# jstmn/cppflow

Hardware: AMD Instinct MI355X
Metric: LM-IK iterations/sec (seeds x waypoints) (higher is better)
Workload: dtype f32

## Files before the change

### cppflow_amd/build.py

```python

import os
import subprocess
import sys

_HERE = os.path.dirname(os.path.abspath(__file__))
CSRC = os.path.join(_HERE, "csrc")
SOURCES = ["cppflow_hip.hip", "fused_static.hip"]
EXTRA_FLAGS = {"fused_static.hip": ["-O2", "-mllvm", "-amdgpu-sched-strategy=max-ilp", "-mllvm", "-enable-post-misched=0"]}
HEADERS = ["lmik_device.h", "robots_gen.h", "rtc_specialize.h", "kernels_chain.h", "kernels_collision.h", "kernels_fused.h", "kernels_track.h", "kernels_quad.h", "kernels_eval.h",
           "kernels_coupled.h", "kernels_dp.h", "kernels_optloop.h", "kernels_scene.h", "kernels_motion.h", "kernels_motion_resolve.h", os.path.join("..", "..", "include", "cppflow_hip.h"),
           os.path.join("..", "..", "include", "cppflow_hip_debug.h")]
OUT = os.path.join(CSRC, "libcppflow_hip.so")

HIPCC_FLAGS = [
    "--offload-arch=gfx950",
    "-O3",
    "-std=c++17",
    "-fPIC",
    "-ffp-contract=off",
    "-fhip-fp32-correctly-rounded-divide-sqrt",
    "-fno-slp-vectorize",
    "-Wno-comment",
]


def source_hash() -> str:
    import hashlib

    h = hashlib.sha256()
    for name in SOURCES + [n for n in HEADERS if n != "rtc_specialize.h"] + ["rtc_specialize.h"]:
        with open(os.path.join(CSRC, name), "rb") as f:
            h.update(name.encode() + b"\0" + f.read() + b"\0")
    h.update(" ".join(HIPCC_FLAGS).encode())
    for name in SOURCES:
        h.update((name + " " + " ".join(EXTRA_FLAGS.get(name, []))).encode())
    h.update(" ".join(link_flags()).encode())
    return h.hexdigest()[:32]


def link_flags():
    return [f for f in HIPCC_FLAGS if f.startswith("--offload-arch=") or f == "-fPIC"] + ["-shared"]


def built_id() -> str:
    if not os.path.exists(OUT):
        return ""
    import re

    with open(OUT, "rb") as f:
        m = re.search(rb"CPPF_BUILD_ID=([0-9a-f]{32})", f.read())
    return m.group(1).decode() if m else ""


def needs_build() -> bool:
    if not os.path.exists(OUT):
        return True
    return built_id() != source_hash()


EMBEDDED = ["lmik_device.h", "kernels_chain.h", "kernels_collision.h", "kernels_fused.h", "kernels_track.h", "kernels_quad.h"]
EMBEDDED_OUT = os.path.join(CSRC, "embedded_src.inc")


def write_embedded_sources() -> bool:
    parts = ["// embedded_src.inc -- GENERATED by cppflow_amd/build.py (the device headers as strings for hipRTC); do not edit."]
    files = [(n, os.path.join(CSRC, n)) for n in EMBEDDED] + [("../../include/cppflow_hip.h", os.path.join(CSRC, "..", "..", "include", "cppflow_hip.h"))]
    parts.append(f"static const int kEmbeddedCount = {len(files)};")
    parts.append("static const char* const kEmbeddedNames[] = {" + ", ".join(f'"{n}"' for n, _ in files) + "};")
    parts.append("static const char* const kEmbeddedSources[] = {")
    for _, path in files:
        text = open(path).read()
        assert ')CPPFSRC"' not in text
        chunks = [text[i : i + 12000] for i in range(0, len(text), 12000)]
        parts.append("    " + "\n    ".join(f'R"CPPFSRC({c})CPPFSRC"' for c in chunks) + ",")
    parts.append("};")
    out = "\n".join(parts) + "\n"
    if os.path.exists(EMBEDDED_OUT) and open(EMBEDDED_OUT).read() == out:
        return False
    with open(EMBEDDED_OUT, "w") as f:
        f.write(out)
    return True


def build(force: bool = False, verbose: bool = False) -> str:
    from cppflow_amd import gen_robots

    if gen_robots.write() and verbose:
        print("regenerated", gen_robots.OUT)
    if write_embedded_sources() and verbose:
        print("regenerated", EMBEDDED_OUT)
    if not force and not needs_build():
        return OUT
    hipcc = os.environ.get("HIPCC", "hipcc")
    objdir = os.path.join(CSRC, "obj")
    os.makedirs(objdir, exist_ok=True)
    procs, objs = [], []
    for src in SOURCES:
        obj = os.path.join(objdir, os.path.splitext(src)[0] + ".o")
        cmd = [hipcc] + HIPCC_FLAGS + EXTRA_FLAGS.get(src, []) + [f'-DCPPF_BUILD_ID="{source_hash()}"', "-c", "-o", obj, os.path.join(CSRC, src)]
        if verbose:
            print(" ".join(cmd))
        procs.append((cmd, subprocess.Popen(cmd, cwd=CSRC)))
        objs.append(obj)
    failed = None
    for cmd, p in procs:
        if p.wait() != 0 and failed is None:
            failed = (p.returncode, cmd)
            for _, other in procs:
                if other.poll() is None:
                    other.kill()
    if failed is not None:
        raise subprocess.CalledProcessError(*failed)
    cmd = [hipcc] + link_flags() + ["-o", OUT] + objs
    if verbose:
        print(" ".join(cmd))
    subprocess.run(cmd, check=True, cwd=CSRC)
    return OUT


TEST_SRC = os.path.join(_HERE, "..", "tests", "native", "rcp_sweep.hip")
TEST_OUT = os.path.join(_HERE, "..", "tests", "native", "libcppf_testkernels.so")


def build_test_kernels(force: bool = False, verbose: bool = False) -> str:
    deps = [TEST_SRC, os.path.join(CSRC, "lmik_device.h"), os.path.abspath(__file__)]
    if not force and os.path.exists(TEST_OUT) and all(os.path.getmtime(TEST_OUT) >= os.path.getmtime(d) for d in deps):
        return TEST_OUT
    cmd = [os.environ.get("HIPCC", "hipcc")] + HIPCC_FLAGS + ["-shared", "-o", TEST_OUT, TEST_SRC]
    if verbose:
        print(" ".join(cmd))
    subprocess.run(cmd, check=True)
    return TEST_OUT


if __name__ == "__main__":
    print(build(force="--force" in sys.argv, verbose=True))
    print(build_test_kernels(force="--force" in sys.argv, verbose=True))
```

### cppflow_amd/csrc/cppflow_hip.hip

```cpp
#include <hip/hip_runtime.h>

#include <dlfcn.h>

#include <atomic>
#include <cmath>
#include <cstdio>
#include <cstring>
#include <mutex>
#include <new>
#include <string>
#include <type_traits>
#include <utility>
#include <vector>

#include "../../include/cppflow_hip_debug.h"
#include "lmik_device.h"
#include "robots_gen.h"

using namespace cppf;

namespace cppf {
bool launch_fused_static(int static_id, int coll, unsigned grid, size_t lds, hipStream_t st, const FusedArgs& args);
int fused_static_block();
}

namespace {

#ifndef CPPF_BLOCK
#define CPPF_BLOCK 256
#endif
constexpr int kBlock = CPPF_BLOCK;

#ifndef CPPF_WAVES_LM
#define CPPF_WAVES_LM 2
#endif
#ifndef CPPF_WAVES_COLL
#define CPPF_WAVES_COLL 2
#endif

#include "kernels_chain.h"
#include "kernels_collision.h"
#include "kernels_fused.h"
#include "kernels_track.h"
#include "kernels_quad.h"
#include "kernels_eval.h"
#include "kernels_scene.h"
#include "kernels_motion.h"
#include "kernels_motion_resolve.h"
#include "kernels_coupled.h"
#include "kernels_dp.h"
#include "kernels_optloop.h"


thread_local std::string g_err;

int fail(int code, const std::string& msg) {
    g_err = msg;
    return code;
}

#define CPPF_REQUIRE(cond, msg) \
    do {                        \
        if (!(cond)) return fail(CPPF_ERR_INVALID, std::string("cppflow_hip: ") + (msg)); \
    } while (0)

#define CPPF_HIP(call)                                                                                       \
    do {                                                                                                     \
        hipError_t e__ = (call);                                                                             \
        if (e__ != hipSuccess)                                                                               \
            return fail(CPPF_ERR_HIP, std::string("cppflow_hip: " #call " failed: ") + hipGetErrorString(e__)); \
    } while (0)

inline unsigned grid_for(size_t n) { return (unsigned)((n + kBlock - 1) / kBlock); }

struct RtcModule;

}

struct cppf_robot {
    cppf_robot_desc desc;
    ChainK chain;
    CollK coll;
    int device;
    int cu_count;
    int static_id;
    size_t lds_bytes;
    void* d_quad;
    float rho[CPPF_MAX_DOF][CPPF_MAX_CAPSULES];
    RtcModule* rtc;
    mutable std::atomic<int> tune[CPPF_TUNE_COUNT];
    mutable std::atomic<uint32_t> life;
};
constexpr uint32_t kRobotDead = 0x80000000u;

namespace {
constexpr int kTuneDefaults[CPPF_TUNE_COUNT] = {
     0,  -1,  16384,  1,
     1,      2,        0,          0,
     42,     22,     (int)(kGateRel * 1e6f + 0.5f),  -1,
     0,
};
inline int tune(const cppf_robot* rb, int key) { return rb->tune[key].load(std::memory_order_relaxed); }

inline size_t fused_static_lds(const cppf_robot* rb) { return fused_static_lds_bound(rb->desc.ndof); }
inline size_t fused_spread_lds(const cppf_robot* rb, size_t n) {
    const int kb = tune(rb, CPPF_TUNE_SPREAD_KB);
    if (kb <= 0 || n > (size_t)128 * kBlock) return 0;
    const size_t stat = fused_static_lds(rb);
    const size_t room = stat + 512 < 65536 ? 65536 - 512 - stat : 0;
    return std::min((size_t)kb * 1024, room);
}
}

#include "rtc_specialize.h"

namespace {

float sqrt_threshold(float r) {
    if (!(r > 0.f)) return 0.f;
    float y = r * r;
    while (std::sqrt(y) >= r) y = std::nextafterf(y, 0.f);
    while (std::sqrt(y) < r) y = std::nextafterf(y, INFINITY);
    return y;
}

struct CapsuleCentred {
    float c[3], h[3], a, ia;
    double half_length;
};
CapsuleCentred capsule_centred(const cppf_robot_desc& d, int cap) {
    CapsuleCentred r;
    for (int k = 0; k < 3; ++k) {
        r.c[k] = (float)(0.5 * ((double)d.cap_p0[cap][k] + (double)d.cap_p1[cap][k]));
        r.h[k] = (float)(0.5 * ((double)d.cap_p1[cap][k] - (double)d.cap_p0[cap][k]));
    }
    const double h0 = r.h[0], h1 = r.h[1], h2 = r.h[2];
    const double a = (h0 * h0 + h1 * h1) + h2 * h2;
    r.a = (float)a;
    r.ia = a >= 0x1p-100 ? (float)(1.0 / a) : 0.f;
    r.half_length = std::sqrt(a);
    return r;
}

double cap_half_length(const cppf_robot_desc& d, int c) { return capsule_centred(d, c).half_length; }

float cull_threshold(double reach) {
    const double y = (reach + 0.01) * (reach + 0.01) * (1.0 + 1e-4);
    float f = (float)y;
    if ((double)f < y) f = std::nextafterf(f, INFINITY);
    return f;
}

constexpr int kQuadTableRecs = CPPF_MAX_PAIRS + CPPF_MAX_CAPSULES;
float round_up_f32(double y) {
    float f = (float)y;
    if ((double)f < y) f = std::nextafterf(f, INFINITY);
    return f;
}
void motion_rho_table(const cppf_robot_desc& d, float (&rho)[CPPF_MAX_DOF][CPPF_MAX_CAPSULES]) {
    const auto norm3 = [](const float* v) { return std::sqrt((double)v[0] * v[0] + (double)v[1] * v[1] + (double)v[2] * v[2]); };
    for (int j = 0; j < CPPF_MAX_DOF; ++j)
        for (int c = 0; c < CPPF_MAX_CAPSULES; ++c) rho[j][c] = 0.f;
    for (int c = 0; c < d.n_capsules; ++c) {
        const int l = d.cap_link[c];
        const double tail = std::max(norm3(d.cap_p0[c]), norm3(d.cap_p1[c])) + (double)d.cap_r[c];
        for (int j = 0; j <= l; ++j) {
            if (d.jtype[j] == CPPF_JOINT_PRISMATIC) {
                rho[j][c] = 1.f;
                continue;
            }
            double sum = tail;
            for (int i = j + 1; i <= l; ++i) {
                sum += norm3(&d.F[i][9]);
                if (d.jtype[i] == CPPF_JOINT_PRISMATIC) sum += std::max(std::fabs((double)d.lo[i]), std::fabs((double)d.hi[i]));
            }
            rho[j][c] = round_up_f32(sum);
        }
    }
}

template <class T>
bool desc_matches(const cppf_robot_desc& d) {
    if (d.ndof != T::D || d.n_capsules != T::L || d.n_pairs != T::P) return false;
    uint32_t pm = 0;
    for (int j = 0; j < T::D; ++j) {
        if (d.jtype[j] == CPPF_JOINT_PRISMATIC) pm |= 1u << j;
        for (int k = 0; k < 12; ++k)
            if (d.F[j][k] != T::F[j][k]) return false;
        if (d.lo[j] != T::lo[j] || d.hi[j] != T::hi[j]) return false;
    }
    if (pm != T::pris_mask) return false;
    for (int k = 0; k < 12; ++k)
        if (d.F_ee[k] != T::Fee[k]) return false;
    for (int c = 0; c < T::L; ++c) {
        if (d.cap_link[c] != T::cap_link[c] || d.cap_r[c] != T::cap_r[c]) return false;
        for (int k = 0; k < 3; ++k)
            if (d.cap_p0[c][k] != T::cap_p0[c][k] || d.cap_p1[c][k] != T::cap_p1[c][k]) return false;
    }
    for (int p = 0; p < T::P; ++p)
        if (d.pairs[p][0] != T::pair_a[p] || d.pairs[p][1] != T::pair_b[p]) return false;
    return true;
}

int find_static_robot(const cppf_robot_desc& d) {
#define CPPF_MATCH(idx, Type) \
    if (desc_matches<Type>(d)) return idx;
    CPPF_FOR_EACH_STATIC_ROBOT(CPPF_MATCH)
#undef CPPF_MATCH
    return -1;
}

template <int N>
struct Dof {
    static constexpr int D = N;
};
template <class T>
struct RobotTag {
    using type = T;
};

template <class F>
int for_ndof(int d, F&& f) {
    switch (d) {
        case 3: return f(Dof<3>{});
        case 4: return f(Dof<4>{});
        case 5: return f(Dof<5>{});
        case 6: return f(Dof<6>{});
        case 7: return f(Dof<7>{});
        case 8: return f(Dof<8>{});
        case 9: return f(Dof<9>{});
        case 10: return f(Dof<10>{});
        case 11: return f(Dof<11>{});
        case 12: return f(Dof<12>{});
        default: return fail(CPPF_ERR_UNSUPPORTED, "cppflow_hip: kernels are built for ndof in 3..12");
    }
}

template <class F>
int for_dyn_robot(const cppf_robot* rb, F&& f) {
    return for_ndof(rb->desc.ndof, [&](auto dof) { return f(RobotTag<DynRobot<decltype(dof)::D>>{}); });
}

inline bool use_table(const cppf_robot* rb) { return rb->static_id >= 0 && !tune(rb, CPPF_TUNE_FORCE_GENERIC); }

template <class F>
int for_robot(const cppf_robot* rb, F&& f) {
    if (!use_table(rb)) return for_dyn_robot(rb, f);
    switch (rb->static_id) {
#define CPPF_TABLE_CASE(idx, Type) \
    case idx: return f(RobotTag<StaRobot<Type>>{});
        CPPF_FOR_EACH_STATIC_ROBOT(CPPF_TABLE_CASE)
#undef CPPF_TABLE_CASE
        default: return CPPF_OK;
    }
}

constexpr int kNoDevice = -12345;
constexpr int kPcrMaxRowsLds = 131072, kPcrMaxRowsGlobal = 49152;
constexpr int kPcrSplitMaxD = 8;

int rtc_launch(const cppf_robot* rb, RtcKernel which, unsigned grid, size_t lds, hipStream_t st, void** args) {
    hipFunction_t f = rb->rtc->fn[which];
    if (!f) return fail(CPPF_ERR_UNSUPPORTED, "cppflow_hip: this kernel is not part of the handle's specialised module");
    CPPF_HIP(hipModuleLaunchKernel(f, grid, 1, 1, (unsigned)kBlock, 1, 1, (unsigned)lds, st, args, nullptr));
    return CPPF_OK;
}

inline bool use_rtc(const cppf_robot* rb) { return rb->rtc != nullptr && !tune(rb, CPPF_TUNE_FORCE_GENERIC); }

int check_launch() {
    CPPF_HIP(hipGetLastError());
    return CPPF_OK;
}

struct DeviceGuard {
    int prev = -1;
    bool switched = false;
    hipError_t err = hipSuccess;
    explicit DeviceGuard(int device) {
        err = hipGetDevice(&prev);
        if (err == hipSuccess && prev != device) {
            err = hipSetDevice(device);
            switched = err == hipSuccess;
        }
    }
    ~DeviceGuard() {
        if (switched) (void)hipSetDevice(prev);
    }
    DeviceGuard(const DeviceGuard&) = delete;
    DeviceGuard& operator=(const DeviceGuard&) = delete;
};

#define CPPF_ENTER(rb)                                                                                              \
    CPPF_REQUIRE((rb) != nullptr, "robot handle is NULL");                                                          \
    CPPF_REQUIRE(!((rb)->life.load(std::memory_order_acquire) & kRobotDead),                                         \
                 "the robot handle was destroyed (cppf_robot_destroy; it is only kept allocated for its live batches)"); \
    DeviceGuard device_guard__((rb)->device);                                                                        \
    if (device_guard__.err != hipSuccess)                                                                            \
        return fail(CPPF_ERR_HIP, std::string("cppflow_hip: selecting the robot's device failed: ") +               \
                                      hipGetErrorString(device_guard__.err))

template <class K, class... A>
int launch_lds(K kernel, dim3 grid, size_t lds, hipStream_t st, const A&... args) {
    if (lds > (size_t)64 * 1024)
        CPPF_HIP(hipFuncSetAttribute(reinterpret_cast<const void*>(kernel), hipFuncAttributeMaxDynamicSharedMemorySize, (int)lds));
    hipLaunchKernelGGL(kernel, grid, dim3(kBlock), lds, st, args...);
    return CPPF_OK;
}

float tile_cull_threshold(const cppf_robot* robot, float reach) {
    double r_max = 0.0;
    for (int c = 0; c < robot->coll.ncaps; ++c) r_max = std::max(r_max, (double)robot->desc.cap_r[c]);
    return cull_threshold(r_max + (double)reach);
}
SceneCullK scene_cull_setup(const cppf_robot* robot, const float* box_lo, const float* box_hi, int n_obs, float reach) {
    SceneCullK sc;
    sc.box_lo = box_lo;
    sc.box_hi = box_hi;
    sc.n_obs = n_obs;
    sc.reach = reach;
    for (int c = 0; c < CPPF_MAX_CAPSULES; ++c) sc.cull2[c] = 0.f;
    for (int c = 0; c < robot->coll.ncaps; ++c)
        sc.cull2[c] = cull_threshold(cap_half_length(robot->desc, c) + (double)robot->desc.cap_r[c] + (double)reach);
    sc.tile_cull2 = tile_cull_threshold(robot, reach);
    return sc;
}

struct CuboidChunks {
    int n_chunks, chunk;
};
CuboidChunks cut_cuboid_chunks(const cppf_robot* robot, unsigned blocks, int n_obs) {
    const int groups = (n_obs + 7) / 8;
    if (groups == 0 || blocks == 0) return {1, 64};
    const unsigned want_blocks = 4u * (unsigned)(robot->cu_count > 0 ? robot->cu_count : 256);
    int n_chunks = (int)std::min<unsigned>((unsigned)groups, std::max(1u, (want_blocks + blocks - 1) / blocks));
    const int groups_per_chunk = (groups + n_chunks - 1) / n_chunks;
    n_chunks = (groups + groups_per_chunk - 1) / groups_per_chunk;
    return {n_chunks, groups_per_chunk * 8};
}

template <class Shape, class Need>
int check_scene_call(const cppf_robot* robot, Shape&& shape, int n_obs, float reach_m, bool io_ok, const char* io_msg, const float* box_lo,
                     const float* box_hi, const void* workspace, size_t workspace_bytes, Need&& need, const char* need_msg,
                     const char* kernel, size_t* lds) {
    CPPF_REQUIRE(robot != nullptr, "robot handle is NULL");
    CPPF_REQUIRE(!(robot->life.load(std::memory_order_acquire) & kRobotDead), "the robot handle was destroyed");
    if (int rc = shape()) return rc;
    CPPF_REQUIRE(n_obs >= 0 && n_obs <= CPPF_MAX_SCENE_OBSTACLES, "n_obs out of range (0 .. CPPF_MAX_SCENE_OBSTACLES)");
    CPPF_REQUIRE(reach_m >= 0.f, "reach_m must be in [0, +inf] (not NaN, not negative)");
    CPPF_REQUIRE(io_ok, io_msg);
    CPPF_REQUIRE(n_obs == 0 || (box_lo && box_hi), "box_lo / box_hi is NULL");
    CPPF_REQUIRE(workspace, "workspace is NULL");
    CPPF_REQUIRE(((uintptr_t)workspace & 15u) == 0, "workspace must be 16-byte aligned");
    size_t bytes = 0;
    if (int rc = need(&bytes)) return rc;
    CPPF_REQUIRE(workspace_bytes >= bytes, need_msg);
    if (robot->desc.ndof < 3) return fail(CPPF_ERR_UNSUPPORTED, "cppflow_hip: kernels are built for ndof in 3..12");
    *lds = use_table(robot) ? 0 : robot->lds_bytes;
    if (*lds > (size_t)160 * 1024 - 1024)
        return fail(CPPF_ERR_UNSUPPORTED, std::string("cppflow_hip: the generic ") + kernel + " kernel cannot stage this many capsules");
    return CPPF_OK;
}

}

extern "C" {

int cppf_abi_version(void) { return CPPF_ABI_VERSION; }

#ifndef CPPF_BUILD_ID
#define CPPF_BUILD_ID "unversioned"
#endif
static const char kBuildIdMarker[] = "CPPF_BUILD_ID=" CPPF_BUILD_ID;
const char* cppf_build_id(void) { return kBuildIdMarker + 14; }

const char* cppf_last_error(void) { return g_err.c_str(); }

int cppf_robot_create(const cppf_robot_desc* desc, int device, cppf_robot** out) {
    CPPF_REQUIRE(desc && out, "desc / out is NULL");
    *out = nullptr;
    const int d = desc->ndof;
    CPPF_REQUIRE(d >= 1 && d <= CPPF_MAX_DOF, "ndof out of range");
    CPPF_REQUIRE(desc->n_capsules >= 0 && desc->n_capsules <= CPPF_MAX_CAPSULES, "n_capsules out of range");
    CPPF_REQUIRE(desc->n_pairs >= 0 && desc->n_pairs <= CPPF_MAX_PAIRS, "n_pairs out of range");
    for (int j = 0; j < d; ++j) {
        CPPF_REQUIRE(desc->jtype[j] == CPPF_JOINT_REVOLUTE || desc->jtype[j] == CPPF_JOINT_PRISMATIC, "bad joint type");
        CPPF_REQUIRE(desc->lo[j] <= desc->hi[j], "joint limits: lo > hi");
        for (int k = 0; k < 12; ++k) CPPF_REQUIRE(std::isfinite(desc->F[j][k]), "non-finite chain constant");
    }
    int prev = -1;
    for (int c = 0; c < desc->n_capsules; ++c) {
        const int l = desc->cap_link[c];
        CPPF_REQUIRE(l >= -1 && l < d, "capsule link index out of range");
        CPPF_REQUIRE(l >= prev, "capsules must be ordered by link (base first)");
        prev = l;
        float len2 = 0.f;
        for (int k = 0; k < 3; ++k) {
            const float dd = desc->cap_p1[c][k] - desc->cap_p0[c][k];
            len2 += dd * dd;
        }
        CPPF_REQUIRE(len2 == 0.f || len2 > 1e-12f, "degenerate capsule (|p1 - p0| < 1e-6 but not 0; use p0 == p1 for a sphere)");
        CPPF_REQUIRE(desc->cap_r[c] >= 0.f, "negative capsule radius");
    }
    for (int p = 0; p < desc->n_pairs; ++p) {
        const int a = desc->pairs[p][0], b = desc->pairs[p][1];
        CPPF_REQUIRE(a >= 0 && a < desc->n_capsules && b >= 0 && b < desc->n_capsules && a != b, "bad capsule pair");
    }
    if (device != kNoDevice) {
        int ndev = 0;
        CPPF_HIP(hipGetDeviceCount(&ndev));
        CPPF_REQUIRE(device >= 0 && device < ndev, "device index out of range");
    }

    cppf_robot* rb = new (std::nothrow) cppf_robot();
    if (!rb) return fail(CPPF_ERR_HIP, "cppflow_hip: out of host memory");
    rb->desc = *desc;
    rb->device = device;
    rb->cu_count = 0;
    if (device != kNoDevice) (void)hipDeviceGetAttribute(&rb->cu_count, hipDeviceAttributeMultiprocessorCount, device);
    rb->life.store(0u, std::memory_order_relaxed);
    for (int k = 0; k < CPPF_TUNE_COUNT; ++k) rb->tune[k].store(kTuneDefaults[k], std::memory_order_relaxed);
    std::memset(&rb->chain, 0, sizeof(ChainK));
    std::memset(&rb->coll, 0, sizeof(CollK));
    rb->chain.ndof = d;
    for (int j = 0; j < d; ++j) {
        std::memcpy(rb->chain.F[j], desc->F[j], sizeof(float) * 12);
        rb->chain.lo[j] = desc->lo[j];
        rb->chain.hi[j] = desc->hi[j];
        if (desc->jtype[j] == CPPF_JOINT_PRISMATIC) rb->chain.pris_mask |= (1u << j);
    }
    std::memcpy(rb->chain.Fee, desc->F_ee, sizeof(float) * 12);
    CollK& co = rb->coll;
    co.ncaps = desc->n_capsules;
    co.npairs = desc->n_pairs;
    for (int c = 0; c < co.ncaps; ++c) {
        const CapsuleCentred cc = capsule_centred(*desc, c);
        for (int k = 0; k < 3; ++k) {
            co.cap_c[c][k] = cc.c[k];
            co.cap_h[c][k] = cc.h[k];
        }
        co.cap_a[c] = cc.a;
        co.cap_ia[c] = cc.ia;
        co.cap_r[c] = desc->cap_r[c];
        co.cap_link[c] = (int8_t)desc->cap_link[c];
        co.cap_thr[c] = sqrt_threshold(desc->cap_r[c]);
        co.cap_cull[c] = cull_threshold(cap_half_length(*desc, c) + (double)desc->cap_r[c]);
    }
    for (int l = -1; l <= d; ++l) {
        int first = co.ncaps;
        for (int c = co.ncaps - 1; c >= 0; --c)
            if (desc->cap_link[c] >= l) first = c;
        co.cap_begin[l + 1] = first;
    }
    for (int p = 0; p < co.npairs; ++p) {
        co.pair_a[p] = (uint8_t)desc->pairs[p][0];
        co.pair_b[p] = (uint8_t)desc->pairs[p][1];
        co.pair_thr[p] = sqrt_threshold(desc->cap_r[desc->pairs[p][0]] + desc->cap_r[desc->pairs[p][1]]);
        const int a = desc->pairs[p][0], b = desc->pairs[p][1];
        co.pair_cull[p] = cull_threshold(cap_half_length(*desc, a) + cap_half_length(*desc, b) + (double)desc->cap_r[a] +
                                         (double)desc->cap_r[b]);
    }
    rb->lds_bytes = (size_t)co.ncaps * 6 * kBlock * sizeof(float);
    rb->static_id = find_static_robot(*desc);
    if (fused_static_block() != kBlock) rb->static_id = -1;
    rb->rtc = nullptr;
    rb->d_quad = nullptr;
    motion_rho_table(*desc, rb->rho);
    if (device != kNoDevice) {
        static_assert(sizeof(rb->rho) % sizeof(uint4) == 0, "the rho table is a whole number of uint4 records");
        std::vector<uint4> host(kQuadTableRecs + sizeof(rb->rho) / sizeof(uint4), uint4{0, 0, 0, 0});
        std::memcpy(&host[kQuadTableRecs], rb->rho, sizeof(rb->rho));
        for (int p = 0; p < co.npairs; ++p) {
            QuadPairRec r{co.pair_a[p], co.pair_b[p], co.pair_thr[p], co.pair_cull[p]};
            std::memcpy(&host[p], &r, sizeof r);
        }
        for (int c = 0; c < co.ncaps; ++c) {
            QuadCapRec r{co.cap_thr[c], co.cap_cull[c], co.cap_a[c], co.cap_ia[c]};
            std::memcpy(&host[CPPF_MAX_PAIRS + c], &r, sizeof r);
        }
        DeviceGuard guard(device);
        hipError_t e = guard.err;
        rb->d_quad = nullptr;
        if (e == hipSuccess) e = hipMalloc(&rb->d_quad, host.size() * sizeof(uint4));
        if (e == hipSuccess) e = hipMemcpy(rb->d_quad, host.data(), host.size() * sizeof(uint4), hipMemcpyHostToDevice);
        if (e != hipSuccess) {
            if (rb->d_quad) (void)hipFree(rb->d_quad);
            delete rb;
            return fail(CPPF_ERR_HIP, std::string("cppflow_hip: device tables: ") + hipGetErrorString(e));
        }
    }
    *out = rb;
    return CPPF_OK;
}

namespace {
void robot_free(cppf_robot* robot) {
    if (robot->device != kNoDevice) {
        DeviceGuard guard(robot->device);
        if (robot->d_quad) (void)hipFree(robot->d_quad);
        if (robot->rtc) {
            if (robot->rtc->module) (void)hipModuleUnload(robot->rtc->module);
            delete robot->rtc;
        }
    }
    delete robot;
}
}

void cppf_robot_destroy(cppf_robot* robot) {
    if (!robot) return;
    const uint32_t before = robot->life.fetch_or(kRobotDead, std::memory_order_acq_rel);
    if (before == 0u) robot_free(robot);
}

int cppf_robot_specialize(cppf_robot* robot, const char* cache_dir) {
    CPPF_REQUIRE(robot != nullptr, "robot handle is NULL");
    if (robot->static_id >= 0 || robot->rtc) return CPPF_OK;
    const bool with_quad = robot->desc.ndof >= 6;
    const std::string source = rtc_program_source(*robot);
    if (const char* dump = std::getenv("CPPF_RTC_DUMP")) {
        std::ofstream f(dump);
        f << source;
    }
    uint64_t key = fnv1a(source);
    for (int i = 0; i < kEmbeddedCount; ++i) key = fnv1a(kEmbeddedSources[i], key);
    for (int i = 0; i < kRtcOptionCount; ++i) key = fnv1a(kRtcOptions[i], key);
    key = fnv1a(rtc_version_string(), key);
    char hex[32];
    std::snprintf(hex, sizeof hex, "%016llx", (unsigned long long)key);
    const std::string dir = rtc_cache_dir(cache_dir), file = dir + "/robot_" + hex + ".cppfrtc";
    std::vector<std::string> names;
    std::string code;
    if (!rtc_cache_read(dir, file, names, code)) {
        if (int rc = rtc_compile(source, with_quad, names, code)) return rc;
        rtc_cache_write(dir, file, names, code);
    }
    DeviceGuard device_guard__(robot->device);
    if (device_guard__.err != hipSuccess)
        return fail(CPPF_ERR_HIP, std::string("cppflow_hip: selecting the robot's device failed: ") + hipGetErrorString(device_guard__.err));
    RtcModule* m = new (std::nothrow) RtcModule();
    if (!m) return fail(CPPF_ERR_HIP, "cppflow_hip: out of host memory");
    hipError_t e = hipModuleLoadData(&m->module, code.data());
    for (int i = 0; e == hipSuccess && i < RTC_COUNT; ++i) {
        if (!with_quad && (i == RTC_QUAD0 || i == RTC_QUAD1)) continue;
        e = hipModuleGetFunction(&m->fn[i], m->module, names[(size_t)i].c_str());
    }
    if (e != hipSuccess) {
        if (m->module) (void)hipModuleUnload(m->module);
        delete m;
        return fail(CPPF_ERR_HIP, std::string("cppflow_hip: loading the specialised code object failed: ") + hipGetErrorString(e));
    }
    robot->rtc = m;
    return CPPF_OK;
}

int cppf_robot_ndof(const cppf_robot* robot) { return robot ? robot->desc.ndof : CPPF_ERR_INVALID; }

int cppf_debug_fused_single_offset(void) { return (int)__builtin_offsetof(FusedArgs, single); }

int cppf_debug_rtc_compile(const cppf_robot_desc* desc, const char* cache_dir) {
    cppf_robot* rb = nullptr;
    if (int rc = cppf_robot_create(desc, kNoDevice, &rb)) return rc;
    rb->static_id = -1;
    rb->device = kNoDevice;
    const int rc = cppf_robot_specialize(rb, cache_dir);
    delete rb;
    (void)hipGetLastError();
    return rc;
}

int cppf_robot_specialization(const cppf_robot* robot) {
    if (!robot) return CPPF_ERR_INVALID;
    return robot->static_id >= 0 ? robot->static_id : (robot->rtc ? CPPF_SPECIALIZATION_RTC : -1);
}

int cppf_debug_set(cppf_robot* robot, int key, int value) {
    CPPF_REQUIRE(robot, "robot handle is NULL");
    CPPF_REQUIRE(key >= 0 && key < CPPF_TUNE_COUNT, "unknown tuning key");
    robot->tune[key].store(value == CPPF_TUNE_DEFAULT ? kTuneDefaults[key] : value, std::memory_order_relaxed);
    return CPPF_OK;
}

int cppf_debug_get(const cppf_robot* robot, int key, int* value) {
    CPPF_REQUIRE(robot && value, "robot / value is NULL");
    CPPF_REQUIRE(key >= 0 && key < CPPF_TUNE_COUNT, "unknown tuning key");
    *value = tune(robot, key);
    return CPPF_OK;
}

int cppf_set_obstacles(cppf_robot* robot, int n_obs, const float* cuboids, const float* Rt) {
    CPPF_REQUIRE(robot, "robot handle is NULL");
    CPPF_REQUIRE(n_obs >= 0 && n_obs <= CPPF_MAX_OBSTACLES, "n_obs out of range");
    CPPF_REQUIRE(n_obs == 0 || (cuboids && Rt), "cuboids / Rt is NULL");
    for (int o = 0; o < n_obs; ++o) {
        const float* R = Rt + o * 12;
        const float I[9] = {1, 0, 0, 0, 1, 0, 0, 0, 1};
        for (int k = 0; k < 9; ++k)
            CPPF_REQUIRE(std::fabs(R[k] - I[k]) < 1e-8f, "only axis-aligned cuboids are supported (R must be I)");
        for (int k = 0; k < 3; ++k) {
            CPPF_REQUIRE(cuboids[o * 6 + k] <= cuboids[o * 6 + 3 + k], "cuboid min corner > max corner");
            robot->coll.obs_lo[o][k] = R[9 + k] + cuboids[o * 6 + k];
            robot->coll.obs_hi[o][k] = R[9 + k] + cuboids[o * 6 + 3 + k];
        }
    }
    robot->coll.nobs = n_obs;
    return CPPF_OK;
}

int cppf_set_joint_limit_padding(cppf_robot* robot, const float* lo_padded, const float* hi_padded) {
    CPPF_REQUIRE(robot, "robot handle is NULL");
    if (!lo_padded || !hi_padded) {
        robot->coll.has_jl = 0;
        return CPPF_OK;
    }
    for (int j = 0; j < robot->desc.ndof; ++j) {
        robot->coll.jl_lo[j] = lo_padded[j];
        robot->coll.jl_hi[j] = hi_padded[j];
    }
    robot->coll.has_jl = 1;
    return CPPF_OK;
}

int cppf_forward_kinematics(const cppf_robot* robot, const float* x, int n, float* poses, void* stream) {
    CPPF_ENTER(robot);
    CPPF_REQUIRE(n >= 0, "n < 0");
    if (n == 0) return CPPF_OK;
    CPPF_REQUIRE(x && poses, "x / poses is NULL");
    hipStream_t st = (hipStream_t)stream;
    return for_ndof(robot->desc.ndof, [&](auto dof) {
        hipLaunchKernelGGL((fk_kernel<decltype(dof)::D>), dim3(grid_for(n)), dim3(kBlock), 0, st, robot->chain, robot->coll, n, x, poses);
        return check_launch();
    });
}

int cppf_jacobian(const cppf_robot* robot, const float* x, int n, float* J, void* stream) {
    CPPF_ENTER(robot);
    CPPF_REQUIRE(n >= 0, "n < 0");
    if (n == 0) return CPPF_OK;
    CPPF_REQUIRE(x && J, "x / J is NULL");
    hipStream_t st = (hipStream_t)stream;
    return for_ndof(robot->desc.ndof, [&](auto dof) {
        hipLaunchKernelGGL((jacobian_kernel<decltype(dof)::D>), dim3(grid_for(n)), dim3(kBlock), 0, st, robot->chain, robot->coll, n, x, J);
        return check_launch();
    });
}

int cppf_pose_errors(const cppf_robot* robot, const float* x, const float* target, int S, int W, float* e,
                     float* current_poses, void* stream) {
    CPPF_ENTER(robot);
    CPPF_REQUIRE(S >= 0 && W >= 0, "S / W < 0");
    const size_t n = (size_t)S * W;
    if (n == 0) return CPPF_OK;
    CPPF_REQUIRE(n <= 0x7fffffffu, "S*W exceeds 2^31-1 rows");
    CPPF_REQUIRE(x && target, "x / target is NULL");
    hipStream_t st = (hipStream_t)stream;
    return for_ndof(robot->desc.ndof, [&](auto dof) {
        hipLaunchKernelGGL((pose_errors_kernel<decltype(dof)::D>), dim3(grid_for(n)), dim3(kBlock), 0, st, robot->chain, robot->coll,
                           (int)n, W, x, target, e, current_poses);
        return check_launch();
    });
}

int cppf_clamp_to_joint_limits(const cppf_robot* robot, float* x, int n, void* stream) {
    CPPF_ENTER(robot);
    CPPF_REQUIRE(n >= 0, "n < 0");
    if (n == 0) return CPPF_OK;
    CPPF_REQUIRE(x, "x is NULL");
    const size_t total = (size_t)n * robot->desc.ndof;
    hipLaunchKernelGGL(clamp_kernel, dim3(grid_for(total)), dim3(kBlock), 0, (hipStream_t)stream, robot->chain, total, x);
    return check_launch();
}

}

namespace {

int make_lm_kernel_params(const cppf_robot* robot, const cppf_lm_params* params, LmK& prm) {
    CPPF_REQUIRE(params, "params is NULL");
    CPPF_REQUIRE(params->n_steps >= 1, "n_steps must be >= 1");
    CPPF_REQUIRE(params->clamp == 1 || params->n_steps == 1, "clamp = 0 is only defined for a single step");
    CPPF_REQUIRE(params->lm_lambda > 0.f, "lm_lambda must be > 0");
    CPPF_REQUIRE(params->alpha_position > 0.f && params->alpha_rotation > 0.f, "alpha_position / alpha_rotation must be > 0");
    CPPF_REQUIRE(params->solver == CPPF_SOLVER_AUTO || params->solver == CPPF_SOLVER_F32 || params->solver == CPPF_SOLVER_F64,
                 "unknown solver");
    CPPF_REQUIRE(params->solver_gate >= 0.f, "solver_gate must be >= 0 (0 = the default tolerance)");
    CPPF_REQUIRE(params->shape == CPPF_SHAPE_AUTO || params->shape == CPPF_SHAPE_ROW || params->shape == CPPF_SHAPE_QUAD,
                 "unknown kernel shape");
    CPPF_REQUIRE(params->tol_pos_m >= 0.f && params->tol_rot_rad >= 0.f, "early-out tolerances must be >= 0");
    CPPF_REQUIRE((params->tol_pos_m > 0.f) == (params->tol_rot_rad > 0.f), "set both early-out tolerances or neither");
    prm.lm_lambda = params->lm_lambda;
    prm.a_pos = params->alpha_position;
    prm.a_rot = params->alpha_rotation;
    prm.lam_r_d = (double)params->lm_lambda / ((double)params->alpha_rotation * (double)params->alpha_rotation);
    prm.lam_p_d = (double)params->lm_lambda / ((double)params->alpha_position * (double)params->alpha_position);
    prm.lam_r = (float)prm.lam_r_d;
    prm.lam_p = (float)prm.lam_p_d;
    const float tau = params->solver_gate > 0.f ? params->solver_gate : CPPF_SOLVER_GATE_DEFAULT;
    const float a_max = std::fmax(params->alpha_position, params->alpha_rotation);
    prm.gate_thr = params->solver == CPPF_SOLVER_F32 ? INFINITY : params->solver == CPPF_SOLVER_F64 ? -INFINITY : tau / (6e-8f * a_max);
    const float rel = 1e-6f * (float)tune(robot, CPPF_TUNE_GATE_REL_PPM) / (6e-8f * a_max);
    prm.gate_rel2 = rel * rel;
    const int pace = tune(robot, CPPF_TUNE_LM_PACE);
    prm.pace_ticks = (pace == 0 || params->tol_pos_m > 0.f || params->n_steps < 3) ? 0 : (pace > 0 ? pace : (int)(0.55f * (200.f + 56.f * (float)robot->desc.ndof) + 0.5f));
    prm.n_steps = params->n_steps;
    prm.clamp = params->clamp;
    prm.n = 0;
    prm.W = 0;
    prm.tol_pos2 = params->tol_pos_m > 0.f ? std::fmax(params->tol_pos_m * params->tol_pos_m, 1.17549435e-38f) : 0.f;
    prm.tol_rot2 = params->tol_rot_rad > 0.f ? std::fmax(params->tol_rot_rad * params->tol_rot_rad, 1.17549435e-38f) : 0.f;
    return CPPF_OK;
}

inline bool outputs_want_collision(const cppf_lm_outputs& o) {
    return o.self_mask || o.env_mask || o.jlim_mask || o.ext_cost || o.min_self || o.min_env || o.seed_summary;
}
inline bool summary_in_launch(int W) { return W >= 64 && kBlock % W == 0 && (W & (W - 1)) == 0; }

int launch_fused_rows(const cppf_robot* robot, int coll, size_t n_rows, unsigned grid, hipStream_t st, const LmK& prm,
                      const BatchItemK& single, const void* table) {
    const bool generic = !use_rtc(robot) && !use_table(robot);
    const size_t spread = fused_spread_lds(robot, n_rows);
    const size_t lds_need = (generic && coll) ? robot->lds_bytes : 0;
    if (generic && coll && lds_need + fused_static_lds(robot) > (size_t)160 * 1024)
        return fail(CPPF_ERR_UNSUPPORTED, "cppflow_hip: the generic kernels cannot stage this many capsules at this ndof; cppf_robot_specialize() the robot");
    FusedArgs fa;
    fa.ch = robot->chain;
    fa.co = robot->coll;
    fa.prm = prm;
    {
        const unsigned long long slots = (unsigned long long)(robot->cu_count > 0 ? robot->cu_count : 256) * 4ull;
        const int d = robot->desc.ndof;
        const bool four = (use_rtc(robot) || use_table(robot)) ? d <= 7 : d <= 6;
        if (!four || (unsigned long long)grid * 4ull < 3ull * slots || (unsigned long long)grid > slots) fa.prm.pace_ticks = 0;
    }
    fa.single = single;
    fa.table = table;
    if (use_rtc(robot)) {
        void* args[] = {(void*)&fa.ch, (void*)&fa.co, (void*)&fa.prm, (void*)&fa.single, (void*)&fa.table};
        if (int rc = rtc_launch(robot, coll == 0 ? RTC_FUSED0 : (coll == 2 ? RTC_FUSED2 : RTC_FUSED1), grid, spread, st, args)) return rc;
    } else if (!generic) {
        if (!launch_fused_static(robot->static_id, coll, grid, spread, st, fa))
            return fail(CPPF_ERR_UNSUPPORTED, "cppflow_hip: no fused kernel for this generated table");
    } else {
        const size_t lds = std::max(lds_need, spread);
        const int rc = for_dyn_robot(robot, [&](auto tag) {
            using RB = typename decltype(tag)::type;
            if (coll == 2)
                hipLaunchKernelGGL((lm_fused_kernel<RB, 2>), dim3(grid), dim3(kBlock), lds, st, fa.ch, fa.co, fa.prm, fa.single, fa.table);
            else if (coll == 1)
                hipLaunchKernelGGL((lm_fused_kernel<RB, 1>), dim3(grid), dim3(kBlock), lds, st, fa.ch, fa.co, fa.prm, fa.single, fa.table);
            else
                hipLaunchKernelGGL((lm_fused_kernel<RB, 0>), dim3(grid), dim3(kBlock), lds, st, fa.ch, fa.co, fa.prm, fa.single, fa.table);
            return CPPF_OK;
        });
        if (rc) return rc;
    }
    return check_launch();
}

template <class RB, int COLL, bool MFMA>
void launch_quad_kernel(const cppf_robot* robot, unsigned grid, size_t lds, hipStream_t st, const LmK& prm, const float* x_in,
                        const float* target, const cppf_lm_outputs& oq, const uint4* tab, const StepGateK gate) {
    hipLaunchKernelGGL((lm_quad_kernel<RB, COLL, MFMA>), dim3(grid), dim3(kBlock), lds, st, robot->chain, robot->coll, prm, x_in, target,
                       oq, tab, gate);
}

int launch_quad(const cppf_robot* robot, bool coll, size_t n, hipStream_t st, const LmK& prm, const float* x_in, const float* target,
                const cppf_lm_outputs& oq, const StepGateK gate) {
    const unsigned grid = (unsigned)((n + kQuadRows - 1) / kQuadRows);
    const size_t lds_q = coll ? sizeof(float) * (4 * (CPPF_MAX_PAIRS + CPPF_MAX_CAPSULES) +
                                                 (size_t)kQuadRows * quad_row_stride(robot->coll.ncaps))
                              : 0;
    const uint4* tab = static_cast<const uint4*>(robot->d_quad);
    const bool mfma = tune(robot, CPPF_TUNE_QUAD_MFMA) && use_table(robot);
    if (use_rtc(robot) && robot->rtc->fn[RTC_QUAD0]) {
        void* args[] = {(void*)&robot->chain, (void*)&robot->coll, (void*)&prm, (void*)&x_in, (void*)&target, (void*)&oq, (void*)&tab, (void*)&gate};
        return rtc_launch(robot, coll ? RTC_QUAD1 : RTC_QUAD0, grid, lds_q, st, args);
    }
    return for_robot(robot, [&](auto tag) {
        using RB = typename decltype(tag)::type;
        if constexpr (RB::D >= 6) {
            constexpr bool kTable = RB::kStatic;
            const auto launch = coll ? (mfma ? launch_quad_kernel<RB, 1, kTable> : launch_quad_kernel<RB, 1, false>)
                                     : (mfma ? launch_quad_kernel<RB, 0, kTable> : launch_quad_kernel<RB, 0, false>);
            launch(robot, grid, lds_q, st, prm, x_in, target, oq, tab, gate);
        }
        return CPPF_OK;
    });
}

inline bool quad_possible(const cppf_robot* robot, const cppf_lm_outputs& out) {
    return robot->desc.ndof >= 6 && !out.J_out && !out.e_out && !out.min_self && !out.min_env &&
           (!out.seed_summary || (out.x_out && out.pos_err_m && out.rot_err_rad && out.self_mask && out.env_mask && out.jlim_mask &&
                                  out.ext_cost));
}

int collision_masks_gated(const cppf_robot* robot, const float* q, int S, int W, uint8_t* self_mask, uint8_t* env_mask,
                          uint8_t* jlim_mask, float* ext_cost, float* min_self, float* min_env, void* stream, const StepGateK gate) {
    CPPF_ENTER(robot);
    CPPF_REQUIRE(S >= 0 && W >= 0, "S / W < 0");
    const size_t n = (size_t)S * W;
    if (n == 0) return CPPF_OK;
    CPPF_REQUIRE(n <= 0x7fffffffu, "S*W exceeds 2^31-1 rows");
    CPPF_REQUIRE(q, "q is NULL");
    hipStream_t st = (hipStream_t)stream;
    const size_t lds = use_table(robot) ? 0 : robot->lds_bytes;
    if (use_rtc(robot)) {
        int n_i = (int)n;
        void* args[] = {(void*)&robot->chain, (void*)&robot->coll, (void*)&n_i, (void*)&q, (void*)&self_mask, (void*)&env_mask,
                        (void*)&jlim_mask, (void*)&ext_cost, (void*)&min_self, (void*)&min_env, (void*)&gate, (void*)&W};
        return rtc_launch(robot, (min_self || min_env) ? RTC_COLL_MIN : RTC_COLL_MASK, grid_for(n), 0, st, args);
    }
    const int rc = for_robot(robot, [&](auto tag) {
        using RB = typename decltype(tag)::type;
        if (min_self || min_env)
            hipLaunchKernelGGL((collision_kernel<RB, true>), dim3(grid_for(n)), dim3(kBlock), lds, st, robot->chain, robot->coll, (int)n,
                               q, self_mask, env_mask, jlim_mask, ext_cost, min_self, min_env, gate, W);
        else
            hipLaunchKernelGGL((collision_kernel<RB, false>), dim3(grid_for(n)), dim3(kBlock), lds, st, robot->chain, robot->coll, (int)n,
                               q, self_mask, env_mask, jlim_mask, ext_cost, min_self, min_env, gate, W);
        return CPPF_OK;
    });
    return rc ? rc : check_launch();
}

struct FullStepForm {
    bool use_pcr, use_rows;
};
FullStepForm full_step_form(const cppf_robot* robot, size_t n, int W, bool use_pose, bool var_coupling) {
    const int t_pcr_rows = tune(robot, CPPF_TUNE_PCR_MAX_ROWS);
    const bool g_pcr_lds = tune(robot, CPPF_TUNE_PCR_LDS) != 0;
    const bool g_rows_pose = tune(robot, CPPF_TUNE_ROWS_POSE) != 0, g_full_rows = tune(robot, CPPF_TUNE_FULL_ROWS) != 0;
    const size_t pcr_rows = t_pcr_rows >= 0 ? (size_t)t_pcr_rows : (size_t)((W <= 256 && g_pcr_lds) ? kPcrMaxRowsLds : kPcrMaxRowsGlobal);
    const size_t pcr_limit = pcr_rows * (robot->desc.ndof <= 7 ? 100 : 50) / 100;
    FullStepForm f;
    f.use_pcr = !var_coupling && !use_pose && W <= 512 && n <= pcr_limit && robot->desc.ndof >= 3 && robot->desc.ndof <= 8;
    f.use_rows = !var_coupling && !f.use_pcr && (!use_pose || g_rows_pose) && g_full_rows && robot->desc.ndof >= 3 &&
                 robot->desc.ndof <= 12 && W <= (1 << 19);
    return f;
}
const char* const kGatedFormRefusal =
    "cppflow_hip: the device-side optimiser loop gates the parallel-in-time and the row-per-lane "
    "elimination only (no pose block, no individually weighted differencing rows, CPPF_TUNE_FULL_ROWS on)";

int full_step_pin_check(const cppf_robot* robot, int S, int W, const cppf_full_params* params, int pin) {
    CPPF_REQUIRE(pin >= 0 && pin <= (CPPF_PIN_FIRST | CPPF_PIN_LAST), "pin_mask must be a combination of CPPF_PIN_FIRST and CPPF_PIN_LAST");
    if (pin == 0) return CPPF_OK;
    CPPF_REQUIRE(robot != nullptr, "robot handle is NULL");
    CPPF_REQUIRE(!(robot->life.load(std::memory_order_acquire) & kRobotDead), "the robot handle was destroyed");
    CPPF_REQUIRE(params, "params is NULL");
    if (params->differencing_mode != 0 || params->pose_do_scale_down_satisfied)
        return fail(CPPF_ERR_UNSUPPORTED, "cppflow_hip: a pinned end waypoint is not combined with the \"satisfied\" row options "
                                          "(differencing_mode != 0, pose_do_scale_down_satisfied)");
    if (S >= 1 && W >= 1 && (size_t)S * W <= 0x7fffffffu && !params->use_pose && robot->desc.ndof <= 8) {
        const FullStepForm form = full_step_form(robot, (size_t)S * W, W, false, false);
        if (!form.use_pcr && !form.use_rows)
            return fail(CPPF_ERR_UNSUPPORTED, "cppflow_hip: the one-wavefront-per-trajectory elimination (what a step resolves to under "
                                              "CPPF_TUNE_FULL_ROWS = 0, with fewer than 3 joints or beyond 2^19 waypoints) takes no "
                                              "pinned end waypoint");
    }
    return CPPF_OK;
}

int lm_full_step_gated(const cppf_robot* robot, const float* x_in, const float* target, const float* virtual_configs, int S, int W,
                       const cppf_full_params* params, int pin, float* work_blocks, float* work_G, float* work_y, float* x_out,
                       void* stream, const StepGateK gate, const SceneStepK* scene = nullptr) {
    if (int rc = full_step_pin_check(robot, S, W, params, pin)) return rc;
    CPPF_ENTER(robot);
    CPPF_REQUIRE(params, "params is NULL");
    CPPF_REQUIRE(S >= 0 && W >= 1, "S < 0 or W < 1");
    CPPF_REQUIRE(params->lm_lambda > 0.f, "lm_lambda must be > 0");
    CPPF_REQUIRE(!params->use_virtual_configs || (params->n_virtual_configs > 0 && 2 * params->n_virtual_configs < W),
                 "2 * n_virtual_configs must be < number of waypoints (optimization_utils.py:449-451)");
    CPPF_REQUIRE(x_out != x_in, "x_out must not alias x_in (the back substitution reads x_in)");
    if (S == 0) return CPPF_OK;
    CPPF_REQUIRE(x_in && target && work_blocks && work_G && work_y && x_out, "NULL pointer");
    const size_t n = (size_t)S * W;
    CPPF_REQUIRE(n <= 0x7fffffffu, "S*W exceeds 2^31-1 rows");
    FullK prm;
    prm.lm_lambda = params->lm_lambda;
    prm.a_pos = params->alpha_position;
    prm.a_rot = params->alpha_rotation;
    prm.a_diff = params->alpha_differencing;
    prm.a_diff_pris = params->alpha_differencing_prismatic_scaling;
    prm.a_vq = params->alpha_virtual_configs;
    prm.a_self = params->alpha_self_collision;
    prm.a_env = params->alpha_env_collision;
    prm.use_pose = params->use_pose;
    prm.use_diff = params->use_differencing;
    prm.use_vq = params->use_virtual_configs;
    prm.n_vq = params->n_virtual_configs;
    prm.use_self = params->use_self_collisions;
    prm.use_env = params->use_env_collisions;
    prm.S = S;
    prm.W = W;
    prm.pin = pin;
    CPPF_REQUIRE(params->differencing_mode >= 0 && params->differencing_mode <= 2, "differencing_mode must be 0, 1 or 2");
    CPPF_REQUIRE(!params->pose_do_scale_down_satisfied || (params->pose_scale_down >= 0.f && params->pose_scale_down < 1.f),
                 "pose scale-down must be in [0, 1) (optimization_utils.py:305)");
    CPPF_REQUIRE(params->differencing_mode != 2 || (params->differencing_scale_down >= 0.f && params->differencing_scale_down < 1.f),
                 "differencing scale-down must be in [0, 1) (optimization_utils.py:367)");
    prm.pose_scale_satisfied = params->use_pose && params->pose_do_scale_down_satisfied;
    prm.pose_thr_m = params->pose_threshold_m;
    prm.pose_thr_rad = params->pose_threshold_rad;
    prm.pose_scale = params->pose_scale_down;
    prm.diff_mode = params->use_differencing ? params->differencing_mode : 0;
    prm.diff_thr_rad = params->differencing_threshold_rad;
    prm.diff_thr_m = params->differencing_threshold_m;
// ... 1114 lines not shown
```

### cppflow_amd/csrc/kernels_collision.h

```cpp
#pragma once

struct CollOut {
    float min_self, min_env;
    int self_hit, env_hit;
};

__device__ __forceinline__ bool cull_far(float lower2, float cull2) {
    return __builtin_amdgcn_ballot_w64(!(lower2 > cull2)) == 0ull;
}

__device__ __forceinline__ float mid_dist2(const float (&a)[3], const float (&b)[3]) {
    const float dx = a[0] - b[0], dy = a[1] - b[1], dz = a[2] - b[2];
    return CPPF_FMA(dz, dz, CPPF_FMA(dy, dy, dx * dx));
}

__device__ __forceinline__ float point_box_dist2(const float (&m)[3], const float* __restrict__ lo,
                                                 const float* __restrict__ hi) {
    const float ex = m[0] - clampf(m[0], lo[0], hi[0]), ey = m[1] - clampf(m[1], lo[1], hi[1]),
                ez = m[2] - clampf(m[2], lo[2], hi[2]);
    return CPPF_FMA(ez, ez, CPPF_FMA(ey, ey, ex * ex));
}

template <class RB>
__device__ __forceinline__ void fk_capsules_to_lds(const RB& rb, const CollK& co, const float (&q)[RB::D],
                                                   float* __restrict__ lds, int tid, float (&R)[9], float (&p)[3]) {
    frame_identity(R, p);
    for (int c = co.cap_begin[0]; c < co.cap_begin[1]; ++c) {
#pragma unroll
        for (int k = 0; k < 3; ++k) {
            lds[(c * 6 + k) * kBlock + tid] = co.cap_c[c][k];
            lds[(c * 6 + 3 + k) * kBlock + tid] = co.cap_h[c][k];
        }
    }
#pragma unroll
    for (int j = 0; j < RB::D; ++j) {
        fk_fixed_joint(rb, j, R, p);
        fk_joint(R, p, rb.pris(j), q[j]);
        for (int c = co.cap_begin[j + 1]; c < co.cap_begin[j + 2]; ++c) {
            float wc[3], wh[3];
            xform_point(R, p, co.cap_c[c][0], co.cap_c[c][1], co.cap_c[c][2], wc);
            xform_dir(R, co.cap_h[c][0], co.cap_h[c][1], co.cap_h[c][2], wh);
#pragma unroll
            for (int k = 0; k < 3; ++k) {
                lds[(c * 6 + k) * kBlock + tid] = wc[k];
                lds[(c * 6 + 3 + k) * kBlock + tid] = wh[k];
            }
        }
    }
}

template <class RB>
__device__ __forceinline__ void capsule_fk_static(const RB& rb, const float (&q)[RB::D], float (&R)[9], float (&p)[3],
                                                  float (&wc)[(RB::Table::L > 0 ? RB::Table::L : 1)][3],
                                                  float (&wh)[(RB::Table::L > 0 ? RB::Table::L : 1)][3]) {
    using T = typename RB::Table;
    frame_identity(R, p);
#pragma unroll
    for (int c = 0; c < T::L; ++c) {
        if (T::cap_link[c] < 0) {
#pragma unroll
            for (int k = 0; k < 3; ++k) {
                wc[c][k] = T::cap_c[c][k];
                wh[c][k] = T::cap_h[c][k];
            }
        }
    }
#pragma unroll
    for (int j = 0; j < RB::D; ++j) {
        fk_fixed_joint(rb, j, R, p);
        fk_joint(R, p, rb.pris(j), q[j]);
#pragma unroll
        for (int c = 0; c < T::L; ++c) {
            if (T::cap_link[c] == j) {
                xform_point(R, p, T::cap_c[c][0], T::cap_c[c][1], T::cap_c[c][2], wc[c]);
                xform_dir(R, T::cap_h[c][0], T::cap_h[c][1], T::cap_h[c][2], wh[c]);
            }
        }
    }
}

__device__ __forceinline__ uint32_t cuboids_in_reach(const CollK& co, const float (&c)[3], float cull2) {
    uint32_t near = 0u;
    for (int o = 0; o < co.nobs; ++o)
        if (!cull_far(point_box_dist2(c, co.obs_lo[o], co.obs_hi[o]), cull2)) near |= 1u << o;
    return near;
}

template <class RB, bool WANT_MIN>
__device__ __forceinline__ CollOut collide_tests_static(const CollK& co,
                                                        const float (&wc)[(RB::Table::L > 0 ? RB::Table::L : 1)][3],
                                                        const float (&wh)[(RB::Table::L > 0 ? RB::Table::L : 1)][3],
                                                        bool do_self, bool do_env) {
    using T = typename RB::Table;
    CollOut r;
    r.min_self = INFINITY;
    r.self_hit = 0;
    if (do_self) {
#pragma unroll
        for (int pi = 0; pi < T::P; ++pi) {
            const int a = T::pair_a[pi], b = T::pair_b[pi];
            if constexpr (!WANT_MIN) {
                if (cull_far(mid_dist2(wc[a], wc[b]), T::pair_cull[pi])) continue;
            }
            const float d2 = seg_seg_dist2(wc[a], wh[a], wc[b], wh[b], T::cap_a[a], T::cap_ia[a], T::cap_a[b], T::cap_ia[b]);
            if constexpr (WANT_MIN) {
                const float v = __builtin_sqrtf(d2) - (T::cap_r[a] + T::cap_r[b]);
                r.min_self = v < r.min_self ? v : r.min_self;
            } else {
                r.self_hit |= d2 < T::pair_thr[pi];
            }
        }
    }
    if constexpr (WANT_MIN) r.self_hit = r.min_self < 0.f;
    r.min_env = INFINITY;
    r.env_hit = 0;
    if (do_env) {
#pragma unroll
        for (int c = 0; c < T::L; ++c) {
            uint32_t near = ~0u;
            if constexpr (!WANT_MIN) {
                near = cuboids_in_reach(co, wc[c], T::cap_cull[c]);
                if (near == 0u) continue;
            }
            for (int o = 0; o < co.nobs; ++o) {
                if (!((near >> o) & 1u)) continue;
                const float d2 = seg_box_dist2(wc[c], wh[c], co.obs_lo[o], co.obs_hi[o]);
                if constexpr (WANT_MIN) {
                    const float v = __builtin_sqrtf(d2) - T::cap_r[c];
                    r.min_env = v < r.min_env ? v : r.min_env;
                } else {
                    r.env_hit |= d2 < T::cap_thr[c];
                }
            }
        }
        if constexpr (WANT_MIN) r.env_hit = r.min_env < 0.f;
    }
    return r;
}

__device__ __forceinline__ void lds_capsule(const float* __restrict__ lds, int tid, int c, float (&wc)[3], float (&wh)[3]) {
#pragma unroll
    for (int k = 0; k < 3; ++k) {
        wc[k] = lds[(c * 6 + k) * kBlock + tid];
        wh[k] = lds[(c * 6 + 3 + k) * kBlock + tid];
    }
}

template <bool WANT_MIN>
__device__ __forceinline__ CollOut collide_from_lds(const CollK& co, const float* __restrict__ lds, int tid,
                                                    bool do_self, bool do_env) {
    CollOut r;
    r.min_self = INFINITY;
    r.self_hit = 0;
    if (do_self) {
        for (int pi = 0; pi < co.npairs; ++pi) {
            const int a = co.pair_a[pi], b = co.pair_b[pi];
            float ca[3], ha[3], cb[3], hb[3];
            lds_capsule(lds, tid, a, ca, ha);
            lds_capsule(lds, tid, b, cb, hb);
            if constexpr (!WANT_MIN) {
                if (cull_far(mid_dist2(ca, cb), co.pair_cull[pi])) continue;
            }
            const float d2 = seg_seg_dist2(ca, ha, cb, hb, co.cap_a[a], co.cap_ia[a], co.cap_a[b], co.cap_ia[b]);
            if constexpr (WANT_MIN) {
                const float v = __builtin_sqrtf(d2) - (co.cap_r[a] + co.cap_r[b]);
                r.min_self = v < r.min_self ? v : r.min_self;
            } else {
                r.self_hit |= d2 < co.pair_thr[pi];
            }
        }
    }
    if constexpr (WANT_MIN) r.self_hit = r.min_self < 0.f;
    r.min_env = INFINITY;
    r.env_hit = 0;
    if (do_env) {
        for (int c = 0; c < co.ncaps; ++c) {
            float wc[3], wh[3];
            lds_capsule(lds, tid, c, wc, wh);
            uint32_t near = ~0u;
            if constexpr (!WANT_MIN) {
                near = cuboids_in_reach(co, wc, co.cap_cull[c]);
                if (near == 0u) continue;
            }
            for (int o = 0; o < co.nobs; ++o) {
                if (!((near >> o) & 1u)) continue;
                const float d2 = seg_box_dist2(wc, wh, co.obs_lo[o], co.obs_hi[o]);
                if constexpr (WANT_MIN) {
                    const float v = __builtin_sqrtf(d2) - co.cap_r[c];
                    r.min_env = v < r.min_env ? v : r.min_env;
                } else {
                    r.env_hit |= d2 < co.cap_thr[c];
                }
            }
        }
        if constexpr (WANT_MIN) r.env_hit = r.min_env < 0.f;
    }
    return r;
}

template <class RB, bool WANT_MIN>
__device__ __forceinline__ CollOut collide_row(const RB& rb, const CollK& co, const float (&q)[RB::D], float* lds, int tid,
                                               float (&R)[9], float (&p)[3], bool do_self, bool do_env) {
    if constexpr (RB::kStatic) {
        constexpr int L = RB::Table::L > 0 ? RB::Table::L : 1;
        float wc[L][3], wh[L][3];
        capsule_fk_static<RB>(rb, q, R, p, wc, wh);
        return collide_tests_static<RB, WANT_MIN>(co, wc, wh, do_self, do_env);
    } else {
        fk_capsules_to_lds<RB>(rb, co, q, lds, tid, R, p);
        return collide_from_lds<WANT_MIN>(co, lds, tid, do_self, do_env);
    }
}

template <int D>
__device__ __forceinline__ int jlim_hit(const CollK& co, const float (&q)[D]) {
    int jl = 0;
    if (co.has_jl) {
#pragma unroll
        for (int j = 0; j < D; ++j) jl |= (q[j] < co.jl_lo[j]) | (q[j] > co.jl_hi[j]);
    }
    return jl;
}

__device__ __forceinline__ void write_coll_outputs(size_t row, const CollOut& c, int jl, uint8_t* self_mask,
                                                   uint8_t* env_mask, uint8_t* jlim_mask, float* ext_cost,
                                                   float* min_self, float* min_env) {
    if (self_mask) self_mask[row] = (uint8_t)c.self_hit;
    if (env_mask) env_mask[row] = (uint8_t)c.env_hit;
    if (jlim_mask) jlim_mask[row] = (uint8_t)jl;
    if (ext_cost) ext_cost[row] = 100.f * (float)jl + 1000.f * (float)c.env_hit + 1000.f * (float)c.self_hit;
    if (min_self) min_self[row] = c.min_self;
    if (min_env) min_env[row] = c.min_env;
}
```

### cppflow_amd/csrc/kernels_fused.h

```cpp
#pragma once


__device__ __forceinline__ void load_target(const float* __restrict__ target, int w, float (&Rt)[9], float (&tt)[3]) {
    const float* t = target + (size_t)w * 7;
    tt[0] = t[0], tt[1] = t[1], tt[2] = t[2];
    quat_to_mat(t[3], t[4], t[5], t[6], Rt);
}

struct RowSummary {
    float pos_err = 0.f, rot_err = 0.f;
    int self_hit = 0, env_hit = 0, jl = 0;
};

template <int CTRL>
__device__ __forceinline__ uint32_t dpp_or_zero(uint32_t x) {
    return (uint32_t)__builtin_amdgcn_update_dpp(0, (int)x, CTRL, 0xf, 0xf, true);
}

template <bool IS_MAX>
__device__ __forceinline__ uint32_t wave_reduce_to_lane63(uint32_t v) {
    auto op = [](uint32_t a, uint32_t b) { return IS_MAX ? __builtin_elementwise_max(a, b) : a + b; };
    v = op(v, dpp_or_zero<0x111>(v));
    v = op(v, dpp_or_zero<0x112>(v));
    v = op(v, dpp_or_zero<0x114>(v));
    v = op(v, dpp_or_zero<0x118>(v));
    v = op(v, dpp_or_zero<0x142>(v));
    v = op(v, dpp_or_zero<0x143>(v));
    return v;
}

__device__ __forceinline__ uint32_t nonneg_bits_nan_to_inf(float x) {
    return __builtin_elementwise_min(__builtin_bit_cast(uint32_t, x), 0x7f800000u);
}

__device__ __forceinline__ void lds_barrier() { asm volatile("s_waitcnt lgkmcnt(0)\n\ts_barrier" ::: "memory"); }

template <class RB>
__device__ __forceinline__ void joint_change_maxima(const RB& rb, const float (&dq)[RB::D], const float (&wr)[RB::D], uint32_t& mrev,
                                                    uint32_t& mpri) {
    const float rad2deg = 57.29577951308232087680f;
    mrev = mpri = 0u;
#pragma unroll
    for (int j = 0; j < RB::D; ++j) {
        if (rb.pris(j))
            mpri = __builtin_elementwise_max(mpri, __builtin_bit_cast(uint32_t, 100.f * fabsf(dq[j])));
        else
            mrev = __builtin_elementwise_max(mrev, __builtin_bit_cast(uint32_t, rad2deg * fabsf(wr[j])));
    }
    mrev = __builtin_elementwise_min(mrev, 0x7f800000u), mpri = __builtin_elementwise_min(mpri, 0x7f800000u);
}

template <class RB, bool = RB::kStatic>
struct MayHavePrismatic {
    static constexpr bool value = true;
};
template <class RB>
struct MayHavePrismatic<RB, true> {
    static constexpr bool value = RB::Table::pris_mask != 0;
};

template <class RB>
__device__ __forceinline__ void block_seed_summary(const RB& rb, int W, size_t row, bool active, const float (&q)[RB::D],
                                                   const RowSummary& rs, float* __restrict__ out) {
    constexpr int D = RB::D;
    static_assert(kBlock <= 256, "a seed's hit counts (<= W <= kBlock) are packed into 10-bit fields");
    __shared__ float s_q[kBlock / 64][D];
    __shared__ uint32_t s_red[kBlock / 64][5];
    const int tid = threadIdx.x, lane = tid & 63, wave = __builtin_amdgcn_readfirstlane(tid >> 6);
    const float rad2deg = 57.29577951308232087680f, pi = 3.14159265358979323846f;
    const int wps = W >> 6;
    if (wps > 1) {
        if (lane == 0) {
#pragma unroll
            for (int j = 0; j < D; ++j) s_q[wave][j] = q[j];
        }
        lds_barrier();
    }
    const bool seed_ends_here = ((wave + 1) & (wps - 1)) == 0;
    const bool has_next = active && !(lane == 63 && seed_ends_here);
    const int nw = wave + 1 < kBlock / 64 ? wave + 1 : wave;
    float dq[D], wr[D];
#pragma unroll
    for (int j = 0; j < D; ++j) {
        const float qn = __builtin_bit_cast(float, __builtin_amdgcn_update_dpp(__builtin_bit_cast(int, s_q[nw][j]), __builtin_bit_cast(int, q[j]),
                                                                               0x130, 0xf, 0xf, false));
        dq[j] = qn - q[j];
        wr[j] = (dq[j] + pi) - pi;
    }
    uint32_t mrev, mpri;
    joint_change_maxima<RB>(rb, dq, wr, mrev, mpri);
    mrev = has_next ? mrev : 0u, mpri = has_next ? mpri : 0u;
    if (__builtin_expect(__builtin_amdgcn_ballot_w64(mrev >= __builtin_bit_cast(uint32_t, 171.f)) != 0ull, 0)) {
#pragma unroll
        for (int j = 0; j < D; ++j) wr[j] = dq[j];
        wrap_pi_all<D>(wr);
        uint32_t mr, mp;
        joint_change_maxima<RB>(rb, dq, wr, mr, mp);
        mrev = has_next ? mr : 0u;
    }
    uint32_t v[5] = {nonneg_bits_nan_to_inf(100.f * fabsf(rs.pos_err)), nonneg_bits_nan_to_inf(rad2deg * fabsf(rs.rot_err)), mrev, mpri,
                     (uint32_t)rs.jl | (uint32_t)rs.env_hit << 10 | (uint32_t)rs.self_hit << 20};
#pragma unroll
    for (int k = 0; k < 3; ++k) v[k] = wave_reduce_to_lane63<true>(v[k]);
    if constexpr (MayHavePrismatic<RB>::value) v[3] = wave_reduce_to_lane63<true>(v[3]);
    v[4] = wave_reduce_to_lane63<false>(v[4]);
    float* o = out + ((uint32_t)row >> (31 - __builtin_clz((uint32_t)W))) * 8;
    if (wps > 1) {
        if (lane == 63) {
#pragma unroll
            for (int k = 0; k < 5; ++k) s_red[wave][k] = v[k];
        }
        lds_barrier();
    }
    if (active && lane == 63 && seed_ends_here) {
#pragma unroll 1
        for (int i = 1; i < wps; ++i) {
#pragma unroll
            for (int k = 0; k < 4; ++k) v[k] = __builtin_elementwise_max(v[k], s_red[wave - i][k]);
            v[4] += s_red[wave - i][4];
        }
#pragma unroll
        for (int k = 0; k < 4; ++k) o[k] = __builtin_bit_cast(float, v[k]);
        const float jl = (float)(v[4] & 1023u), env = (float)((v[4] >> 10) & 1023u), self = (float)(v[4] >> 20);
        o[4] = self, o[5] = env, o[6] = jl;
        o[7] = 100.f * jl + 1000.f * env + 1000.f * self;
    }
}

#ifndef CPPF_LM_PACE
#define CPPF_LM_PACE 1
#endif
__device__ __forceinline__ void lm_pace(uint32_t t0, int k, int pace) {
    if (CPPF_LM_PACE == 0 || pace == 0) return;
    const int lag = (int)((uint32_t)__builtin_amdgcn_s_memrealtime() - t0) - k * pace, half = pace >> 1;
    if (lag > half)
        __builtin_amdgcn_s_setprio(3);
    else if (lag > 0)
        __builtin_amdgcn_s_setprio(2);
    else if (lag > -half)
        __builtin_amdgcn_s_setprio(1);
    else
        __builtin_amdgcn_s_setprio(0);
}

template <class RB>
__device__ __forceinline__ void lm_row_load(int W, const float* __restrict__ x_in, const float* __restrict__ target,
                                            size_t row, float (&q)[RB::D], float (&Rt)[9], float (&tt)[3]) {
    load_x<RB::D>(x_in, row, q);
    load_target(target, (int)((uint32_t)row % (uint32_t)W), Rt, tt);
}

#ifndef CPPF_LEAD_SINCOS
#define CPPF_LEAD_SINCOS 2
#endif
#ifndef CPPF_FIRST_LEAN
#define CPPF_FIRST_LEAN 1
#endif
template <class RB, bool LEAD, bool FIRST = false>
constexpr int lead_sincos() {
    return LEAD ? (FIRST && CPPF_LEAD_SINCOS == 2 ? 3 : CPPF_LEAD_SINCOS) : 0;
}
template <class RB, bool LEAD, bool FIRST = false>
__device__ __forceinline__ bool lm_row_iterate(const RB& rb, const LmK& prm, const cppf_lm_outputs& out, size_t row, bool last,
                                               const float (&Rt)[9], const float (&tt)[3], float* __restrict__ gate_lds,
                                               float (&q)[RB::D]) {
    constexpr int D = RB::D;
    float delta[D];
    bool conv = false;
    {
        float R[9], p[3], ax[D][3], og[D][3], J[6][D], e[6];
        fk_ee_axes<RB, lead_sincos<RB, LEAD, FIRST>()>(rb, q, R, p, ax, og);
        pose_error<LEAD>(Rt, tt, R, p, e);
        if constexpr (!LEAD) {
            if (prm.tol_pos2 > 0.f) {
                conv = dot3(e[3], e[4], e[5], e[3], e[4], e[5]) < prm.tol_pos2 && dot3(e[0], e[1], e[2], e[0], e[1], e[2]) < prm.tol_rot2;
                if (__builtin_amdgcn_ballot_w64(!conv) == 0ull) return true;
            }
        }
        jacobian_from_axes<RB>(rb, p, ax, og, J);
        float est = 0.f;
        if constexpr (D < 6) {
            lm_primal_solve<D>(J, e, prm.lm_lambda, prm.a_pos, prm.a_rot, delta);
        } else {
            float y[6];
            if constexpr (LEAD && CPPF_LEAN_BLOCK_SOLVE != 0)
                lm_dual_solve_y_blk<D>(J, e, prm.lam_r, prm.lam_p, y, est);
            else
                lm_dual_solve_y<D>(J, e, prm.lam_r, prm.lam_p, y, est);
            lm_dual_apply<D>(J, y, delta);
        }
        if constexpr (!LEAD) {
            if (last) {
                if (out.J_out) {
                    float* Jo = out.J_out + row * 6 * D;
#pragma unroll
                    for (int i = 0; i < 6; ++i)
#pragma unroll
                        for (int j = 0; j < D; ++j) Jo[i * D + j] = J[i][j] * (i < 3 ? prm.a_rot : prm.a_pos);
                }
                if (out.e_out) {
#pragma unroll
                    for (int i = 0; i < 6; ++i) out.e_out[row * 6 + i] = e[i] * (i < 3 ? prm.a_rot : prm.a_pos);
                }
            }
        }
        if constexpr (D >= 6) {
            bool flag = !conv && est > prm.gate_thr;
            if (__builtin_expect(__builtin_amdgcn_ballot_w64(flag) != 0ull, 0)) {
                if (prm.clamp && prm.gate_thr > -INFINITY) {
                    bool cut = false;
#pragma unroll
                    for (int j = 0; j < D; ++j) {
                        const float v = q[j] + delta[j];
                        cut |= (v < rb.lo(j)) | (v > rb.hi(j));
                    }
                    flag = flag && !cut;
                }
                if constexpr (LEAD) {
                    if (prm.gate_thr > -INFINITY) {
                        const float es2 = CPPF_FMA(prm.a_pos * prm.a_pos, dot3(e[3], e[4], e[5], e[3], e[4], e[5]),
                                                   prm.a_rot * prm.a_rot * dot3(e[0], e[1], e[2], e[0], e[1], e[2]));
                        flag = flag && est * est > prm.gate_rel2 * es2;
                    }
                }
                unsigned long long todo = __builtin_amdgcn_ballot_w64(flag);
                if (todo != 0ull) {
                    int rank = lm_gate_hand_over<D>(J, e, todo, gate_lds, flag);
                    lm_gate_solve<D>(prm.lam_r_d, prm.lam_p_d, todo, rank, gate_lds, flag, delta);
                    while ((todo = __builtin_amdgcn_ballot_w64(flag)) != 0ull) {
                        float R2[9], p2[3], ax2[D][3], og2[D][3], J2[6][D], e2[6];
#pragma unroll
                        for (int j = 0; j < D; ++j) asm volatile("" : "+v"(q[j]));
                        fk_ee_axes<RB, lead_sincos<RB, LEAD, FIRST>()>(rb, q, R2, p2, ax2, og2);
                        pose_error<LEAD>(Rt, tt, R2, p2, e2);
                        jacobian_from_axes<RB>(rb, p2, ax2, og2, J2);
                        rank = lm_gate_hand_over<D>(J2, e2, todo, gate_lds, flag);
                        lm_gate_solve<D>(prm.lam_r_d, prm.lam_p_d, todo, rank, gate_lds, flag, delta);
                    }
                }
            }
        }
    }
    if constexpr (!LEAD) {
        if (prm.tol_pos2 > 0.f) {
            if (!conv) {
#pragma unroll
                for (int j = 0; j < D; ++j) q[j] += delta[j];
                if (prm.clamp) clamp_row<RB>(rb, q);
            }
            return conv;
        }
    }
#pragma unroll
    for (int j = 0; j < D; ++j) q[j] += delta[j];
    if (prm.clamp) clamp_row<RB>(rb, q);
    return false;
}

template <class RB, int COLL>
__device__ __forceinline__ void lm_row_finish(const RB& rb, const CollK& co, const cppf_lm_outputs& out, float* lds, int tid,
                                              size_t row, const float (&Rt)[9], const float (&tt)[3], const float (&q)[RB::D],
                                              RowSummary& rs) {
    constexpr int D = RB::D;
    if (out.x_out) store_x<D>(out.x_out, row, q);
    const bool want_metrics = out.pos_err_m || out.rot_err_rad || out.seed_summary;
    if constexpr (COLL != 0) {
        const bool do_self = out.self_mask || out.min_self || out.ext_cost || out.seed_summary;
        const bool do_env = out.env_mask || out.min_env || out.ext_cost || out.seed_summary;
        rs.jl = jlim_hit<D>(co, q);
        CollOut c;
        auto metrics = [&](float (&R)[9], float (&p)[3]) {
            if (want_metrics) {
                fk_fixed_ee(rb, R, p);
                pose_metrics(Rt, tt, R, p, rs.pos_err, rs.rot_err);
                if (out.pos_err_m) out.pos_err_m[row] = rs.pos_err;
                if (out.rot_err_rad) out.rot_err_rad[row] = rs.rot_err;
            }
        };
        if constexpr (RB::kStatic) {
            constexpr int L = RB::Table::L > 0 ? RB::Table::L : 1;
            float wc[L][3], wh[L][3];
            {
                float R[9], p[3];
                capsule_fk_static<RB>(rb, q, R, p, wc, wh);
                metrics(R, p);
            }
            c = collide_tests_static<RB, COLL == 2>(co, wc, wh, do_self, do_env);
        } else {
            {
                float R[9], p[3];
                fk_capsules_to_lds<RB>(rb, co, q, lds, tid, R, p);
                metrics(R, p);
            }
            c = collide_from_lds<COLL == 2>(co, lds, tid, do_self, do_env);
        }
        rs.self_hit = c.self_hit, rs.env_hit = c.env_hit;
        write_coll_outputs(row, c, rs.jl, out.self_mask, out.env_mask, out.jlim_mask, out.ext_cost, out.min_self,
                           out.min_env);
    } else {
        if (want_metrics) {
            float R[9], p[3];
            fk_ee<RB>(rb, q, R, p);
            pose_metrics(Rt, tt, R, p, rs.pos_err, rs.rot_err);
            if (out.pos_err_m) out.pos_err_m[row] = rs.pos_err;
            if (out.rot_err_rad) out.rot_err_rad[row] = rs.rot_err;
        }
    }
}

template <class RB>
constexpr int lm_waves() {
    return RB::kStatic ? (RB::D <= 7 ? 4 : 3) : (RB::D <= 6 ? 4 : (RB::D <= 8 ? 3 : 2));
}

template <class T>
__device__ __forceinline__ T* as_global(T* p) {
    return (T*)(__attribute__((address_space(1))) T*)p;
}

typedef const __attribute__((address_space(4))) BatchItemK* BatchItemPtr;

__device__ __forceinline__ BatchItemPtr fused_item(const void* table, uint32_t& blk) {
    typedef const __attribute__((address_space(4))) char* CPtr;
    blk = blockIdx.x;
    BatchItemPtr itp = (BatchItemPtr)((CPtr)__builtin_amdgcn_kernarg_segment_ptr() + __builtin_offsetof(FusedArgs, single));
    if (table) {
        const CPtr tab = (CPtr)(uintptr_t)table;
        const __attribute__((address_space(4))) BatchHeadK* hd = (const __attribute__((address_space(4))) BatchHeadK*)tab;
        uint32_t b = 0, begin = 0;
#pragma unroll
        for (int i = 0; i < CPPF_MAX_BATCH - 1; ++i) {
            const uint32_t e = hd->block_end[i];
            const bool past = blk >= e;
            b = past ? (uint32_t)(i + 1) : b;
            begin = past ? e : begin;
        }
        blk -= begin;
        itp = (BatchItemPtr)(tab + sizeof(BatchHeadK)) + b;
    }
    return itp;
}

__device__ __forceinline__ cppf_lm_outputs fused_outputs(BatchItemPtr itp) {
    cppf_lm_outputs o;
    o.x_out = as_global(itp->out.x_out), o.J_out = as_global(itp->out.J_out), o.e_out = as_global(itp->out.e_out);
    o.pos_err_m = as_global(itp->out.pos_err_m), o.rot_err_rad = as_global(itp->out.rot_err_rad);
    o.self_mask = as_global(itp->out.self_mask), o.env_mask = as_global(itp->out.env_mask), o.jlim_mask = as_global(itp->out.jlim_mask);
    o.ext_cost = as_global(itp->out.ext_cost), o.min_self = as_global(itp->out.min_self), o.min_env = as_global(itp->out.min_env);
    o.seed_summary = as_global(itp->out.seed_summary), o.n_iters = as_global(itp->out.n_iters);
    return o;
}

template <class RB, int COLL>
__global__ __launch_bounds__(kBlock) __attribute__((amdgpu_waves_per_eu(lm_waves<RB>(), lm_waves<RB>()))) void lm_fused_kernel(const ChainK ch, const CollK co, const LmK prm,
                                                          const BatchItemK single, const void* table) {
    extern __shared__ float lds[];
    (void)single;
    constexpr int D = RB::D;
    __shared__ float s_gate[kBlock / 64][GateLds<D>::kFloats];
    static_assert(sizeof(s_gate) + (kBlock / 64) * (D + 8) * sizeof(float) <= fused_static_lds_bound(D), "fused_static_lds_bound is stale");
    const RB rb{ch, co};
    uint32_t blk;
    const BatchItemPtr itp = fused_item(table, blk);
    const cppf_lm_outputs out = fused_outputs(itp);
    const int tid = threadIdx.x;
    const size_t row = (size_t)(blk * (unsigned)kBlock + (unsigned)tid);
    const bool active = row < (size_t)itp->n;
    float q[D];
#pragma unroll
    for (int j = 0; j < D; ++j) q[j] = 0.f;
    RowSummary rs;
    if (active) {
        float Rt[9], tt[3];
        lm_row_load<RB>(itp->W, as_global(itp->x_in), as_global(itp->target), row, q, Rt, tt);
        float chk = tt[0] + tt[1] + tt[2];
#pragma unroll
        for (int j = 0; j < D; ++j) chk += q[j];
#pragma unroll
        for (int k = 0; k < 9; ++k) chk += Rt[k];
        unsigned long long bad_mask = __builtin_amdgcn_ballot_w64(!(fabsf(chk) < INFINITY));
        asm volatile("" : "+s"(bad_mask));
        float* const gate_lds = s_gate[__builtin_amdgcn_readfirstlane(tid >> 6)];
        const uint32_t pace_t0 = (CPPF_LM_PACE != 0 && prm.pace_ticks != 0) ? (uint32_t)__builtin_amdgcn_s_memrealtime() : 0u;
        int iters = 0, it = 0;
        if (!(prm.tol_pos2 > 0.f)) {
            if (prm.n_steps >= 2) {
                (void)lm_row_iterate<RB, CPPF_FIRST_LEAN != 0, true>(rb, prm, out, row, false, Rt, tt, gate_lds, q);
                it = 1;
            }
            for (; it < prm.n_steps - 1; ++it) {
                lm_pace(pace_t0, it, prm.pace_ticks);
                (void)lm_row_iterate<RB, true>(rb, prm, out, row, false, Rt, tt, gate_lds, q);
            }
            iters = it;
            lm_pace(pace_t0, it, prm.pace_ticks);
        }
        for (; it < prm.n_steps; ++it) {
            const bool conv = lm_row_iterate<RB, false>(rb, prm, out, row, it == prm.n_steps - 1, Rt, tt, gate_lds, q);
            iters += conv ? 0 : 1;
            if (prm.tol_pos2 > 0.f && __builtin_amdgcn_ballot_w64(!conv) == 0ull) break;
        }
        int tid_b = threadIdx.x;
        asm volatile("" : "+v"(tid_b));
        const size_t row_b = (size_t)(blk * (unsigned)kBlock + (unsigned)tid_b);
        if (out.n_iters) out.n_iters[row_b] = iters;
        if ((bad_mask >> (tid_b & 63)) & 1ull) {
#pragma unroll
            for (int j = 0; j < D; ++j) q[j] = __builtin_nanf("");
        }
        lm_pace(pace_t0, prm.n_steps, prm.pace_ticks);
        lm_row_finish<RB, COLL>(rb, co, out, lds, tid_b, row_b, Rt, tt, q, rs);
    }
    if constexpr (COLL != 0) {
        if (out.seed_summary) {
            int tid_c = threadIdx.x;
            asm volatile("" : "+v"(tid_c));
            block_seed_summary<RB>(rb, itp->W, (size_t)(blk * (unsigned)kBlock + (unsigned)tid_c), active, q, rs, out.seed_summary);
        }
    }
}

template <class RB, bool WANT_MIN>
__global__ __launch_bounds__(kBlock, CPPF_WAVES_COLL) void collision_kernel(const ChainK ch, const CollK co, int n,
                                                           const float* __restrict__ x, uint8_t* self_mask,
                                                           uint8_t* env_mask, uint8_t* jlim_mask, float* ext_cost,
                                                           float* min_self, float* min_env, const StepGateK gate, int gate_W) {
    extern __shared__ float lds[];
    constexpr int D = RB::D;
    const RB rb{ch, co};
    const int tid = threadIdx.x;
    const size_t row = (size_t)blockIdx.x * kBlock + tid;
    if (row >= (size_t)n) return;
    if (gate.ctl != nullptr && !step_open(gate, (int)(row / (size_t)gate_W))) return;
    float q[D], R[9], p[3];
    load_x<D>(x, row, q);
    const bool do_self = self_mask || min_self || ext_cost;
    const bool do_env = env_mask || min_env || ext_cost;
    CollOut c;
    c.min_self = c.min_env = INFINITY;
    c.self_hit = c.env_hit = 0;
    if (do_self || do_env) c = collide_row<RB, WANT_MIN>(rb, co, q, lds, tid, R, p, do_self, do_env);
    write_coll_outputs(row, c, jlim_hit<D>(co, q), self_mask, env_mask, jlim_mask, ext_cost, min_self, min_env);
}

template <int D, bool ENV>
__global__ __launch_bounds__(kBlock) void distances_kernel(const ChainK ch, const CollK co, int n,
                                                           const float* __restrict__ x, float blo0, float blo1,
                                                           float blo2, float bhi0, float bhi1, float bhi2,
                                                           float* __restrict__ dists) {
    extern __shared__ float lds[];
    using RB = DynRobot<D>;
    const RB rb{ch, co};
    const int tid = threadIdx.x;
    const size_t row = (size_t)blockIdx.x * kBlock + tid;
    if (row >= (size_t)n) return;
    float q[D], R[9], p[3];
    load_x<D>(x, row, q);
    fk_capsules_to_lds<RB>(rb, co, q, lds, tid, R, p);
    if constexpr (ENV) {
        const float lo[3] = {blo0, blo1, blo2}, hi[3] = {bhi0, bhi1, bhi2};
        for (int c = 0; c < co.ncaps; ++c) {
            float wc[3], wh[3];
            lds_capsule(lds, tid, c, wc, wh);
            dists[row * co.ncaps + c] = seg_box_dist(wc, wh, lo, hi) - co.cap_r[c];
        }
    } else {
        for (int pi = 0; pi < co.npairs; ++pi) {
            const int a = co.pair_a[pi], b = co.pair_b[pi];
            float ca[3], ha[3], cb[3], hb[3];
            lds_capsule(lds, tid, a, ca, ha);
            lds_capsule(lds, tid, b, cb, hb);
            dists[row * co.npairs + pi] =
                seg_seg_dist(ca, ha, cb, hb, co.cap_a[a], co.cap_ia[a], co.cap_a[b], co.cap_ia[b]) - (co.cap_r[a] + co.cap_r[b]);
        }
    }
}

template <int D>
__global__ __launch_bounds__(kBlock) void fk_kernel(const ChainK ch, const CollK co, int n, const float* __restrict__ x,
                                                    float* __restrict__ poses) {
    using RB = DynRobot<D>;
    const RB rb{ch, co};
    const size_t row = (size_t)blockIdx.x * kBlock + threadIdx.x;
    if (row >= (size_t)n) return;
    float q[D], R[9], p[3], qt[4];
    load_x<D>(x, row, q);
    fk_ee<RB>(rb, q, R, p);
    mat_to_quat(R, qt);
    float* o = poses + row * 7;
    o[0] = p[0], o[1] = p[1], o[2] = p[2], o[3] = qt[0], o[4] = qt[1], o[5] = qt[2], o[6] = qt[3];
}

template <int D>
__global__ __launch_bounds__(kBlock) void jacobian_kernel(const ChainK ch, const CollK co, int n,
                                                          const float* __restrict__ x, float* __restrict__ Jout) {
    using RB = DynRobot<D>;
    const RB rb{ch, co};
    const size_t row = (size_t)blockIdx.x * kBlock + threadIdx.x;
    if (row >= (size_t)n) return;
    float q[D], R[9], p[3], ax[D][3], og[D][3], J[6][D];
    load_x<D>(x, row, q);
    fk_ee_axes<RB>(rb, q, R, p, ax, og);
    jacobian_from_axes<RB>(rb, p, ax, og, J);
    float* Jo = Jout + row * 6 * D;
#pragma unroll
    for (int i = 0; i < 6; ++i)
#pragma unroll
        for (int j = 0; j < D; ++j) Jo[i * D + j] = J[i][j];
}

template <int D>
__global__ __launch_bounds__(kBlock) void pose_errors_kernel(const ChainK ch, const CollK co, int n, int W,
                                                             const float* __restrict__ x,
                                                             const float* __restrict__ target, float* __restrict__ e_out,
                                                             float* __restrict__ cur_out) {
    using RB = DynRobot<D>;
    const RB rb{ch, co};
    const size_t row = (size_t)blockIdx.x * kBlock + threadIdx.x;
    if (row >= (size_t)n) return;
    float q[D], R[9], p[3], Rt[9], tt[3], e[6];
    load_x<D>(x, row, q);
    load_target(target, (int)(row % (size_t)W), Rt, tt);
    fk_ee<RB>(rb, q, R, p);
    pose_error(Rt, tt, R, p, e);
    if (e_out) {
#pragma unroll
        for (int i = 0; i < 6; ++i) e_out[row * 6 + i] = e[i];
    }
    if (cur_out) {
        float qt[4];
        mat_to_quat(R, qt);
        float* o = cur_out + row * 7;
        o[0] = p[0], o[1] = p[1], o[2] = p[2], o[3] = qt[0], o[4] = qt[1], o[5] = qt[2], o[6] = qt[3];
    }
}

template <int D>
__global__ __launch_bounds__(kBlock) void pose_metrics_kernel(const ChainK ch, const CollK co, int n, int W,
                                                              const float* __restrict__ x,
                                                              const float* __restrict__ target,
                                                              float* __restrict__ pos_err, float* __restrict__ rot_err) {
    using RB = DynRobot<D>;
    const RB rb{ch, co};
    const size_t row = (size_t)blockIdx.x * kBlock + threadIdx.x;
    if (row >= (size_t)n) return;
    float q[D], R[9], p[3], Rt[9], tt[3], pe, re;
    load_x<D>(x, row, q);
    load_target(target, (int)(row % (size_t)W), Rt, tt);
    fk_ee<RB>(rb, q, R, p);
    pose_metrics(Rt, tt, R, p, pe, re);
    if (pos_err) pos_err[row] = pe;
    if (rot_err) rot_err[row] = re;
}

__device__ __forceinline__ float clamp_joint(const ChainK& ch, int j, float v) {
    return v != v ? v : fminf(fmaxf(v, ch.lo[j]), ch.hi[j]);
}

__global__ __launch_bounds__(kBlock) void clamp_kernel(const ChainK ch, size_t total, float* __restrict__ x) {
    const size_t i = (size_t)blockIdx.x * kBlock + threadIdx.x;
    if (i >= total) return;
    const int j = (int)(i % (size_t)ch.ndof);
    x[i] = clamp_joint(ch, j, x[i]);
}

template <int D>
__global__ __launch_bounds__(64) void seed_validity_kernel(const ChainK ch, const CollK co, int S, int W,
                                                           const float* __restrict__ x,
                                                           const float* __restrict__ target, float* __restrict__ out) {
    using RB = DynRobot<D>;
    const RB rb{ch, co};
    const int s = blockIdx.x;
    if (s >= S) return;
    const float rad2deg = 57.29577951308232087680f;
    float mp = 0.f, mr = 0.f, mrev = 0.f, mpri = 0.f;
    for (int w = threadIdx.x; w < W; w += 64) {
        const size_t row = (size_t)s * W + w;
        float q[D], R[9], p[3], Rt[9], tt[3], pe, re;
        load_x<D>(x, row, q);
        load_target(target, w, Rt, tt);
        fk_ee<RB>(rb, q, R, p);
        pose_metrics(Rt, tt, R, p, pe, re);
        mp = fmaxf(mp, nan_to_inf(100.f * pe));
        mr = fmaxf(mr, nan_to_inf(rad2deg * re));
        if (w + 1 < W) {
            float qn[D], dq[D], wr[D];
            load_x<D>(x, row + 1, qn);
#pragma unroll
            for (int j = 0; j < D; ++j) dq[j] = wr[j] = qn[j] - q[j];
            wrap_pi_all<D>(wr);
#pragma unroll
            for (int j = 0; j < D; ++j) {
                if (rb.pris(j))
                    mpri = fmaxf(mpri, nan_to_inf(fabsf(100.f * dq[j])));
                else
                    mrev = fmaxf(mrev, nan_to_inf(fabsf(rad2deg * wr[j])));
            }
        }
    }
#pragma unroll
    for (int off = 32; off > 0; off >>= 1) {
        mp = fmaxf(mp, __shfl_xor(mp, off, 64));
        mr = fmaxf(mr, __shfl_xor(mr, off, 64));
        mrev = fmaxf(mrev, __shfl_xor(mrev, off, 64));
        mpri = fmaxf(mpri, __shfl_xor(mpri, off, 64));
    }
    if (threadIdx.x == 0) {
        out[s * 4 + 0] = mp, out[s * 4 + 1] = mr, out[s * 4 + 2] = mrev, out[s * 4 + 3] = mpri;
    }
}
```

### cppflow_amd/csrc/lmik_device.h

```cpp
#pragma once

#include <hip/hip_runtime.h>
#ifndef __HIPCC_RTC__
#include <stdint.h>
#endif

#include "../../include/cppflow_hip.h"

#ifndef INFINITY
#define INFINITY __builtin_huge_valf()
#endif

#define CPPF_FMA(a, b, c) __builtin_fmaf((a), (b), (c))

namespace cppf {

struct ChainK {
    float F[CPPF_MAX_DOF][12];
    float Fee[12];
    float lo[CPPF_MAX_DOF];
    float hi[CPPF_MAX_DOF];
    uint32_t pris_mask;
    int32_t ndof;
};

struct CollK {
    float cap_c[CPPF_MAX_CAPSULES][3];
    float cap_h[CPPF_MAX_CAPSULES][3];
    float cap_a[CPPF_MAX_CAPSULES];
    float cap_ia[CPPF_MAX_CAPSULES];
    float cap_r[CPPF_MAX_CAPSULES];
    int32_t cap_begin[CPPF_MAX_DOF + 2];
    int8_t cap_link[CPPF_MAX_CAPSULES];
    float pair_thr[CPPF_MAX_PAIRS];
    float cap_thr[CPPF_MAX_CAPSULES];
    float pair_cull[CPPF_MAX_PAIRS];
    float cap_cull[CPPF_MAX_CAPSULES];
    uint8_t pair_a[CPPF_MAX_PAIRS];
    uint8_t pair_b[CPPF_MAX_PAIRS];
    float obs_lo[CPPF_MAX_OBSTACLES][3];
    float obs_hi[CPPF_MAX_OBSTACLES][3];
    float jl_lo[CPPF_MAX_DOF];
    float jl_hi[CPPF_MAX_DOF];
    int32_t ncaps, npairs, nobs, has_jl;
};

struct LmK {
    double lam_r_d, lam_p_d;
    float lam_r, lam_p;
    float lm_lambda, a_pos, a_rot;
    int32_t n_steps, clamp;
    int32_t n, W;
    float tol_pos2, tol_rot2;
    float gate_thr;
    float gate_rel2;
    int32_t pace_ticks;
};

struct StepGateK {
    const int32_t* ctl;
    int32_t per_traj;
    uint32_t mask;
};
__device__ __forceinline__ bool step_open(const StepGateK& g, int s) {
    if (g.ctl == nullptr) return true;
    return ((g.mask >> (uint32_t)g.ctl[(size_t)(s * g.per_traj) * 16]) & 1u) != 0u;
}

struct BatchItemK {
    const float* x_in;
    const float* target;
    cppf_lm_outputs out;
    int32_t n, W;
};

struct BatchHeadK {
    uint32_t block_end[CPPF_MAX_BATCH];
};

struct FusedArgs {
    ChainK ch;
    CollK co;
    LmK prm;
    BatchItemK single;
    const void* table;
};

__device__ __forceinline__ float cmul(float x, float c) {
    if (__builtin_constant_p(c)) {
        if (c == 0.f) return 0.f;
        if (c == 1.f) return x;
        if (c == -1.f) return -x;
    }
    return x * c;
}

__device__ __forceinline__ float cfma(float x, float c, float acc) {
    if (__builtin_constant_p(c)) {
        if (c == 0.f) return acc;
        if (__builtin_constant_p(acc) && acc == 0.f) return cmul(x, c);
        if (c == 1.f) return acc + x;
        if (c == -1.f) return acc - x;
    }
    return CPPF_FMA(x, c, acc);
}

__device__ __forceinline__ float cfma2(float a, float b, float acc) {
    if (__builtin_constant_p(a) && a == 0.f) return acc;
    return cfma(a, b, acc);
}

template <int D_>
struct DynRobot {
    static constexpr int D = D_;
    static constexpr bool kStatic = false;
    const ChainK& ch;
    const CollK& co;
    __device__ __forceinline__ float F(int j, int k) const { return ch.F[j][k]; }
    __device__ __forceinline__ float Fee(int k) const { return ch.Fee[k]; }
    __device__ __forceinline__ bool pris(int j) const { return (ch.pris_mask >> j) & 1u; }
    __device__ __forceinline__ float lo(int j) const { return ch.lo[j]; }
    __device__ __forceinline__ float hi(int j) const { return ch.hi[j]; }
};

template <class T>
struct StaRobot {
    using Table = T;
    static constexpr int D = T::D;
    static constexpr bool kStatic = true;
    const ChainK& ch;
    const CollK& co;
    __device__ __forceinline__ float F(int j, int k) const { return T::F[j][k]; }
    __device__ __forceinline__ float Fee(int k) const { return T::Fee[k]; }
    __device__ __forceinline__ bool pris(int j) const { return (T::pris_mask >> j) & 1u; }
    __device__ __forceinline__ float lo(int j) const { return T::lo[j]; }
    __device__ __forceinline__ float hi(int j) const { return T::hi[j]; }
};

__device__ __forceinline__ void sincos_cw(float x, float& s, float& c) {
    const float magic = 12582912.0f;
    const float t = CPPF_FMA(x, 0.63661977236758134f, magic);
    const float k = t - magic;
    float r = CPPF_FMA(-k, 1.5703125f, x);
    r = CPPF_FMA(-k, 4.837512969970703125e-4f, r);
    r = CPPF_FMA(-k, 7.54978995489188e-8f, r);
    const float z = r * r;
    const float ps = CPPF_FMA(CPPF_FMA(-1.9515295891e-4f, z, 8.3321608736e-3f), z, -1.6666654611e-1f);
    const float sn = CPPF_FMA(r * z, ps, r);
    const float pc = CPPF_FMA(CPPF_FMA(2.443315711809948e-5f, z, -1.388731625493765e-3f), z, 4.166664568298827e-2f);
    const float cs = CPPF_FMA(z * z, pc, CPPF_FMA(-0.5f, z, 1.0f));
    const uint32_t ki = __float_as_uint(t);
    const bool odd = ki & 1u;
    const uint32_t so = __float_as_uint(odd ? cs : sn) ^ ((ki << 30) & 0x80000000u);
    const uint32_t co = __float_as_uint(odd ? sn : cs) ^ (((ki + 1u) << 30) & 0x80000000u);
    s = __uint_as_float(so);
    c = __uint_as_float(co);
}

__device__ __forceinline__ void sincos_hw(float x, float& s, float& c) {
    const float r = x * 0.15915494309189535f;
    s = __builtin_amdgcn_sinf(r);
    c = __builtin_amdgcn_cosf(r);
}

constexpr float kPiF = 3.14159274101257324f, kTwoPiF = 6.28318548202514648f;
template <int FOLD>
__device__ __forceinline__ void sincos_pi(float x, float& s, float& c) {
    float r = x;
    if constexpr (FOLD == 1) r = x > kPiF ? x - kTwoPiF : x;
    if constexpr (FOLD == -1) r = x < -kPiF ? x + kTwoPiF : x;
    if constexpr (FOLD == 2) {
        const float magic = 12582912.0f;
        const float k = CPPF_FMA(x, 0.15915494309189535f, magic) - magic;
        r = CPPF_FMA(-k, 1.9353071795864769e-3f, CPPF_FMA(-k, 6.28125f, x));
    }
    const float u = r * r;
    float ps = -2.0696598213e-08f, pc = 1.7243808603e-09f;
    ps = CPPF_FMA(ps, u, 2.7087969556e-06f);
    pc = CPPF_FMA(pc, u, -2.7078681342e-07f);
    ps = CPPF_FMA(ps, u, -1.9817604334e-04f);
    pc = CPPF_FMA(pc, u, 2.4769848096e-05f);
    ps = CPPF_FMA(ps, u, 8.3327908069e-03f);
    pc = CPPF_FMA(pc, u, -1.3887801906e-03f);
    ps = CPPF_FMA(ps, u, -1.6666620970e-01f);
    pc = CPPF_FMA(pc, u, 4.1666489094e-02f);
    ps = CPPF_FMA(ps, u, 9.9999994040e-01f);
    pc = CPPF_FMA(pc, u, -4.9999988079e-01f);
    s = ps * r;
    c = CPPF_FMA(pc, u, 1.0f);
}

__device__ __forceinline__ void fk_fixed(float (&R)[9], float (&p)[3], const float (&F)[12]) {
    float A[9], np[3];
#pragma unroll
    for (int i = 0; i < 3; ++i) {
        const float r0 = R[3 * i], r1 = R[3 * i + 1], r2 = R[3 * i + 2];
        np[i] = cfma(r2, F[11], cfma(r1, F[10], cfma(r0, F[9], p[i])));
#pragma unroll
        for (int c = 0; c < 3; ++c) A[3 * i + c] = cfma(r2, F[6 + c], cfma(r1, F[3 + c], cmul(r0, F[c])));
    }
#pragma unroll
    for (int k = 0; k < 9; ++k) R[k] = A[k];
#pragma unroll
    for (int k = 0; k < 3; ++k) p[k] = np[k];
}

template <class RB>
__device__ __forceinline__ void fk_fixed_joint(const RB& rb, int j, float (&R)[9], float (&p)[3]) {
    float F[12];
#pragma unroll
    for (int k = 0; k < 12; ++k) F[k] = rb.F(j, k);
    fk_fixed(R, p, F);
}

template <class RB>
__device__ __forceinline__ void fk_fixed_ee(const RB& rb, float (&R)[9], float (&p)[3]) {
    float F[12];
#pragma unroll
    for (int k = 0; k < 12; ++k) F[k] = rb.Fee(k);
    fk_fixed(R, p, F);
}

template <int SC = 0>
__device__ __forceinline__ void fk_joint(float (&R)[9], float (&p)[3], bool prismatic, float q, float lo = 0.f, float hi = 0.f) {
    if (!prismatic) {
        float s, c;
        if constexpr (SC == 1) {
            sincos_hw(q, s, c);
        } else if constexpr (SC == 3) {
            sincos_pi<2>(q, s, c);
        } else if constexpr (SC == 2) {
            if (lo >= -kPiF && hi <= kPiF)
                sincos_pi<0>(q, s, c);
            else if (lo >= -kPiF && hi <= 3.f * kPiF)
                sincos_pi<1>(q, s, c);
            else if (lo >= -3.f * kPiF && hi <= kPiF)
                sincos_pi<-1>(q, s, c);
            else
                sincos_pi<2>(q, s, c);
        } else {
            sincos_cw(q, s, c);
        }
#pragma unroll
        for (int i = 0; i < 3; ++i) {
            const float a0 = R[3 * i], a1 = R[3 * i + 1];
            R[3 * i] = cfma(s, a1, cmul(c, a0));
            R[3 * i + 1] = cfma(c, a1, -cmul(s, a0));
        }
    } else {
#pragma unroll
        for (int i = 0; i < 3; ++i) p[i] = CPPF_FMA(R[3 * i + 2], q, p[i]);
    }
}

__device__ __forceinline__ void frame_identity(float (&R)[9], float (&p)[3]) {
    R[0] = 1.f, R[1] = 0.f, R[2] = 0.f, R[3] = 0.f, R[4] = 1.f, R[5] = 0.f, R[6] = 0.f, R[7] = 0.f, R[8] = 1.f;
    p[0] = p[1] = p[2] = 0.f;
}

__device__ __forceinline__ float dot3(float a0, float a1, float a2, float b0, float b1, float b2) {
    return CPPF_FMA(a2, b2, CPPF_FMA(a1, b1, a0 * b0));
}

__device__ __forceinline__ float nan_to_inf(float v) { return v != v ? INFINITY : v; }

__device__ __forceinline__ float clampf(float x, float lo, float hi) { return __builtin_amdgcn_fmed3f(x, lo, hi); }
__device__ __forceinline__ float clamp01(float v) { return __builtin_amdgcn_fmed3f(v, 0.f, 1.f); }

__device__ __forceinline__ void xform_point(const float (&R)[9], const float (&p)[3], float c0, float c1, float c2,
                                            float (&w)[3]) {
#pragma unroll
    for (int i = 0; i < 3; ++i) w[i] = cfma(R[3 * i + 2], c2, cfma(R[3 * i + 1], c1, cfma(R[3 * i], c0, p[i])));
}

__device__ __forceinline__ void mat_to_quat(const float (&R)[9], float (&q)[4]) {
    const float m00 = R[0], m01 = R[1], m02 = R[2], m10 = R[3], m11 = R[4], m12 = R[5], m20 = R[6], m21 = R[7], m22 = R[8];
    const float q0 = 1.f + m00 + m11 + m22, q1 = 1.f + m00 - m11 - m22, q2 = 1.f - m00 + m11 - m22,
                q3 = 1.f - m00 - m11 + m22;
    int best = 0;
    float bv = q0;
    if (q1 > bv) best = 1, bv = q1;
    if (q2 > bv) best = 2, bv = q2;
    if (q3 > bv) best = 3, bv = q3;
    const float d = __builtin_sqrtf(bv > 0.f ? bv : 0.f);
    const float inv = 0.5f / d;
    if (best == 0) {
        q[0] = 0.5f * d, q[1] = (m21 - m12) * inv, q[2] = (m02 - m20) * inv, q[3] = (m10 - m01) * inv;
    } else if (best == 1) {
        q[0] = (m21 - m12) * inv, q[1] = 0.5f * d, q[2] = (m10 + m01) * inv, q[3] = (m02 + m20) * inv;
    } else if (best == 2) {
        q[0] = (m02 - m20) * inv, q[1] = (m10 + m01) * inv, q[2] = 0.5f * d, q[3] = (m12 + m21) * inv;
    } else {
        q[0] = (m10 - m01) * inv, q[1] = (m20 + m02) * inv, q[2] = (m21 + m12) * inv, q[3] = 0.5f * d;
    }
}

__device__ __forceinline__ void quat_to_mat(float w, float x, float y, float z, float (&R)[9]) {
    R[0] = 1.f - 2.f * (y * y + z * z);
    R[1] = 2.f * (x * y - w * z);
    R[2] = 2.f * (x * z + w * y);
    R[3] = 2.f * (x * y + w * z);
    R[4] = 1.f - 2.f * (x * x + z * z);
    R[5] = 2.f * (y * z - w * x);
    R[6] = 2.f * (x * z - w * y);
    R[7] = 2.f * (y * z + w * x);
    R[8] = 1.f - 2.f * (x * x + y * y);
}

__device__ __forceinline__ float rcp_newton(float x) {
    const float y0 = __builtin_amdgcn_rcpf(x);
    return CPPF_FMA(CPPF_FMA(-x, y0, 1.0f), y0, y0);
}
__device__ __forceinline__ float rcp_rn(float x) { return fabsf(x) >= 0x1p-100f ? rcp_newton(x) : 0.f; }
__device__ __forceinline__ float rcp_rn_pos(float x) { return x >= 0x1p-100f ? rcp_newton(x) : 0.f; }

__device__ __forceinline__ float clamp11(float v) { return __builtin_amdgcn_fmed3f(v, -1.f, 1.f); }

__device__ __forceinline__ void xform_dir(const float (&R)[9], float h0, float h1, float h2, float (&w)[3]) {
#pragma unroll
    for (int i = 0; i < 3; ++i) w[i] = cfma(R[3 * i + 2], h2, cfma(R[3 * i + 1], h1, cmul(R[3 * i], h0)));
}

__device__ __forceinline__ float seg_seg_closest2(const float (&C1)[3], const float (&H1)[3], const float (&C2)[3],
                                                  const float (&H2)[3], float a, float ia, float e, float ie,
                                                  float (&c1)[3], float (&c2)[3]) {
    float rr[3];
#pragma unroll
    for (int i = 0; i < 3; ++i) rr[i] = C1[i] - C2[i];
    const float b = dot3(H1[0], H1[1], H1[2], H2[0], H2[1], H2[2]);
    const float c = dot3(H1[0], H1[1], H1[2], rr[0], rr[1], rr[2]);
    const float f = dot3(H2[0], H2[1], H2[2], rr[0], rr[1], rr[2]);
    const float denom = CPPF_FMA(-b, b, a * e);
    float s = clamp11(CPPF_FMA(b, f, -(c * e)) * rcp_rn_pos(denom));
    float t = CPPF_FMA(b, s, f) * ie;
    const float s_lo = clamp11(-(b + c) * ia), s_hi = clamp11((b - c) * ia);
    s = t < -1.f ? s_lo : (t > 1.f ? s_hi : s);
    s = ie == 0.f ? clamp11(-c * ia) : s;
    t = clamp11(t);
    float df[3];
#pragma unroll
    for (int i = 0; i < 3; ++i) {
        df[i] = CPPF_FMA(-t, H2[i], CPPF_FMA(s, H1[i], rr[i]));
        c1[i] = CPPF_FMA(s, H1[i], C1[i]);
        c2[i] = CPPF_FMA(t, H2[i], C2[i]);
    }
    return dot3(df[0], df[1], df[2], df[0], df[1], df[2]);
}
// ... 124 lines not shown
```

### cppflow_amd/csrc/robots_gen.h

```cpp
#pragma once
#include <stdint.h>

namespace cppf {
namespace gen {

struct Panda {
    static constexpr const char* name = "panda";
    static constexpr int D = 7, L = 9, P = 25;
    static constexpr uint32_t pris_mask = 0u;
    static constexpr float F[7][12] = {
        {1.0f, 0.0f, 0.0f, 0.0f, 1.0f, 0.0f, 0.0f, 0.0f, 1.0f, 0.0f, 0.0f, 0x1.54fdf40000000p-2f},
        {1.0f, 0.0f, 0.0f, 0.0f, 0.0f, 1.0f, 0.0f, -1.0f, 0.0f, 0.0f, 0.0f, 0.0f},
        {1.0f, 0.0f, 0.0f, 0.0f, 0.0f, -1.0f, 0.0f, 1.0f, 0.0f, 0.0f, -0x1.4395820000000p-2f, 0.0f},
        {1.0f, 0.0f, 0.0f, 0.0f, 0.0f, -1.0f, 0.0f, 1.0f, 0.0f, 0x1.51eb860000000p-4f, 0.0f, 0.0f},
        {1.0f, 0.0f, 0.0f, 0.0f, 0.0f, 1.0f, 0.0f, -1.0f, 0.0f, -0x1.51eb860000000p-4f, 0x1.89374c0000000p-2f, 0.0f},
        {1.0f, 0.0f, 0.0f, 0.0f, 0.0f, -1.0f, 0.0f, 1.0f, 0.0f, 0.0f, 0.0f, 0.0f},
        {1.0f, 0.0f, 0.0f, 0.0f, 0.0f, -1.0f, 0.0f, 1.0f, 0.0f, 0x1.6872b00000000p-4f, 0.0f, 0.0f},
    };
    static constexpr float Fee[12] = {0x1.6a09e60000000p-1f, 0x1.6a09e60000000p-1f, 0.0f, -0x1.6a09e60000000p-1f, 0x1.6a09e60000000p-1f, 0.0f, 0.0f, 0.0f, 1.0f, 0.0f, 0.0f, 0x1.b645a20000000p-4f};
    static constexpr float lo[7] = {-0x1.72daba0000000p+1f, -0x1.c346dc0000000p+0f, -0x1.72daba0000000p+1f, -0x1.8930be0000000p+1f, -0x1.72daba0000000p+1f, -0x1.1eb8520000000p-6f, -0x1.72daba0000000p+1f};
    static constexpr float hi[7] = {0x1.72daba0000000p+1f, 0x1.c346dc0000000p+0f, 0x1.72daba0000000p+1f, -0x1.1de69a0000000p-4f, 0x1.72daba0000000p+1f, 0x1.e051ec0000000p+1f, 0x1.72daba0000000p+1f};
    static constexpr int cap_link[9] = {-1, 0, 1, 2, 3, 4, 5, 6, 6};
    static constexpr float cap_p0[9][3] = {{-0x1.eb851e0000000p-5f, 0.0f, 0x1.eb851e0000000p-5f}, {0.0f, 0.0f, -0x1.851eb80000000p-3f}, {0.0f, 0.0f, 0.0f}, {0.0f, 0.0f, -0x1.5c28f60000000p-3f}, {0.0f, 0.0f, 0.0f}, {0.0f, 0.0f, -0x1.0a3d700000000p-2f}, {0.0f, 0.0f, 0.0f}, {0.0f, 0.0f, 0.0f}, {-0x1.ec5f620000000p-5f, -0x1.ec5f620000000p-5f, 0x1.2d0e560000000p-3f}};
    static constexpr float cap_p1[9][3] = {{0.0f, 0.0f, 0x1.eb851e0000000p-5f}, {0.0f, 0.0f, -0x1.eb851e0000000p-6f}, {0.0f, -0x1.0a3d700000000p-3f, 0.0f}, {0x1.51eb860000000p-4f, 0.0f, 0.0f}, {-0x1.51eb860000000p-4f, 0x1.c28f5c0000000p-4f, 0.0f}, {0.0f, 0x1.47ae140000000p-5f, -0x1.47ae140000000p-6f}, {0x1.6872b00000000p-4f, 0.0f, 0.0f}, {0.0f, 0.0f, 0x1.70a3d80000000p-4f}, {0x1.ec5f620000000p-5f, 0x1.ec5f620000000p-5f, 0x1.2d0e560000000p-3f}};
    static constexpr float cap_r[9] = {0x1.70a3d80000000p-4f, 0x1.0a3d700000000p-4f, 0x1.0a3d700000000p-4f, 0x1.eb851e0000000p-5f, 0x1.eb851e0000000p-5f, 0x1.c28f5c0000000p-5f, 0x1.99999a0000000p-5f, 0x1.70a3d80000000p-5f, 0x1.47ae140000000p-5f};
    static constexpr float cap_c[9][3] = {{-0x1.eb851e0000000p-6f, 0.0f, 0x1.eb851e0000000p-5f}, {0.0f, 0.0f, -0x1.c28f5c0000000p-4f}, {0.0f, -0x1.0a3d700000000p-4f, 0.0f}, {0x1.51eb860000000p-5f, 0.0f, -0x1.5c28f60000000p-4f}, {-0x1.51eb860000000p-5f, 0x1.c28f5c0000000p-5f, 0.0f}, {0.0f, 0x1.47ae140000000p-6f, -0x1.1eb8520000000p-3f}, {0x1.6872b00000000p-5f, 0.0f, 0.0f}, {0.0f, 0.0f, 0x1.70a3d80000000p-5f}, {0.0f, 0.0f, 0x1.2d0e560000000p-3f}};
    static constexpr float cap_h[9][3] = {{0x1.eb851e0000000p-6f, 0.0f, 0.0f}, {0.0f, 0.0f, 0x1.47ae140000000p-4f}, {0.0f, -0x1.0a3d700000000p-4f, 0.0f}, {0x1.51eb860000000p-5f, 0.0f, 0x1.5c28f60000000p-4f}, {-0x1.51eb860000000p-5f, 0x1.c28f5c0000000p-5f, 0.0f}, {0.0f, 0x1.47ae140000000p-6f, 0x1.eb851e0000000p-4f}, {0x1.6872b00000000p-5f, 0.0f, 0.0f}, {0.0f, 0.0f, 0x1.70a3d80000000p-5f}, {0x1.ec5f620000000p-5f, 0x1.ec5f620000000p-5f, 0.0f}};
    static constexpr float cap_a[9] = {0x1.d7dbf40000000p-11f, 0x1.a36e2e0000000p-8f, 0x1.14e3bc0000000p-8f, 0x1.2481700000000p-7f, 0x1.35c2900000000p-8f, 0x1.e4f7640000000p-7f, 0x1.fb82c20000000p-10f, 0x1.096bba0000000p-9f, 0x1.d97f620000000p-8f};
    static constexpr float cap_ia[9] = {0x1.15c71e0000000p+10f, 0x1.3880000000000p+7f, 0x1.d95f700000000p+7f, 0x1.c019ce0000000p+6f, 0x1.a723f60000000p+7f, 0x1.0e45320000000p+6f, 0x1.0243b40000000p+9f, 0x1.edd3be0000000p+8f, 0x1.14d10e0000000p+7f};
    static constexpr float pair_thr[25] = {0x1.89a0260000000p-6f, 0x1.70a3d80000000p-6f, 0x1.70a3d80000000p-6f, 0x1.5879400000000p-6f, 0x1.41205a0000000p-6f, 0x1.2a99320000000p-6f, 0x1.14e3ba0000000p-6f, 0x1.0000000000000p-6f, 0x1.0000000000000p-6f, 0x1.d7dbf20000000p-7f, 0x1.b15b540000000p-7f, 0x1.8c7e280000000p-7f, 0x1.6944660000000p-7f, 0x1.0000000000000p-6f, 0x1.d7dbf20000000p-7f, 0x1.b15b540000000p-7f, 0x1.8c7e280000000p-7f, 0x1.6944660000000p-7f, 0x1.b15b540000000p-7f, 0x1.8c7e280000000p-7f, 0x1.6944680000000p-7f, 0x1.47ae120000000p-7f, 0x1.8c7e280000000p-7f, 0x1.6944680000000p-7f, 0x1.47ae120000000p-7f};
    static constexpr float cap_thr[9] = {0x1.096bba0000000p-7f, 0x1.14e3ba0000000p-8f, 0x1.14e3ba0000000p-8f, 0x1.d7dbf20000000p-9f, 0x1.d7dbf20000000p-9f, 0x1.8c7e280000000p-9f, 0x1.47ae140000000p-9f, 0x1.096bba0000000p-9f, 0x1.a36e2c0000000p-10f};
    static constexpr float pair_cull[25] = {0x1.14ead40000000p-4f, 0x1.4b84da0000000p-4f, 0x1.1242d40000000p-4f, 0x1.8137460000000p-4f, 0x1.9b153a0000000p-5f, 0x1.8c88520000000p-5f, 0x1.0a5e7a0000000p-4f, 0x1.8858bc0000000p-4f, 0x1.49d18e0000000p-4f, 0x1.c295de0000000p-4f, 0x1.fbf6860000000p-5f, 0x1.ebc6240000000p-5f, 0x1.4128940000000p-4f, 0x1.27de9e0000000p-4f, 0x1.9abfce0000000p-4f, 0x1.c09b240000000p-5f, 0x1.b166700000000p-5f, 0x1.1fab9e0000000p-4f, 0x1.dcb6c20000000p-4f, 0x1.11b0a40000000p-4f, 0x1.0948ea0000000p-4f, 0x1.57465c0000000p-4f, 0x1.bbd3760000000p-5f, 0x1.acb3bc0000000p-5f, 0x1.1cf6800000000p-4f};
    static constexpr float cap_cull[9] = {0x1.14ead60000000p-6f, 0x1.89aa3a0000000p-6f, 0x1.4128940000000p-6f, 0x1.bb4b580000000p-6f, 0x1.3b72fc0000000p-6f, 0x1.1d70780000000p-5f, 0x1.6274440000000p-7f, 0x1.47b67a0000000p-7f, 0x1.2aa0d60000000p-6f};
    static constexpr int pair_a[25] = {0, 0, 0, 0, 0, 0, 0, 1, 1, 1, 1, 1, 1, 2, 2, 2, 2, 2, 3, 3, 3, 3, 4, 4, 4};
    static constexpr int pair_b[25] = {2, 3, 4, 5, 6, 7, 8, 3, 4, 5, 6, 7, 8, 4, 5, 6, 7, 8, 5, 6, 7, 8, 6, 7, 8};
};

struct Fetch {
    static constexpr const char* name = "fetch";
    static constexpr int D = 8, L = 10, P = 27;
    static constexpr uint32_t pris_mask = 1u;
    static constexpr float F[8][12] = {
        {1.0f, 0.0f, 0.0f, 0.0f, 1.0f, 0.0f, 0.0f, 0.0f, 1.0f, -0x1.63d70a0000000p-4f, 0.0f, 0x1.827d020000000p-2f},
        {1.0f, 0.0f, 0.0f, 0.0f, 1.0f, 0.0f, 0.0f, 0.0f, 1.0f, 0x1.e9930c0000000p-4f, 0.0f, 0x1.64f2280000000p-2f},
        {0.0f, 1.0f, 0.0f, 0.0f, 0.0f, 1.0f, 1.0f, 0.0f, 0.0f, 0x1.df3b640000000p-4f, 0.0f, 0x1.eb851e0000000p-5f},
        {0.0f, 1.0f, 0.0f, 0.0f, 0.0f, 1.0f, 1.0f, 0.0f, 0.0f, 0.0f, 0x1.c083120000000p-3f, 0.0f},
        {0.0f, 0.0f, 1.0f, 1.0f, 0.0f, 0.0f, 0.0f, 1.0f, 0.0f, 0.0f, 0.0f, 0x1.10624e0000000p-3f},
        {0.0f, 1.0f, 0.0f, 0.0f, 0.0f, 1.0f, 1.0f, 0.0f, 0.0f, 0.0f, 0x1.9374bc0000000p-3f, 0.0f},
        {0.0f, 0.0f, 1.0f, 1.0f, 0.0f, 0.0f, 0.0f, 1.0f, 0.0f, 0.0f, 0.0f, 0x1.fdf3b60000000p-4f},
        {0.0f, 1.0f, 0.0f, 0.0f, 0.0f, 1.0f, 1.0f, 0.0f, 0.0f, 0.0f, 0x1.1ba5e40000000p-3f, 0.0f},
    };
    static constexpr float Fee[12] = {0.0f, 1.0f, 0.0f, 0.0f, 0.0f, 1.0f, 1.0f, 0.0f, 0.0f, 0.0f, 0.0f, 0x1.54e3bc0000000p-3f};
    static constexpr float lo[8] = {0.0f, -0x1.9b089a0000000p+0f, -0x1.3893740000000p+0f, -0x1.921fb60000000p+1f, -0x1.2020c40000000p+1f, -0x1.921fb60000000p+1f, -0x1.147ae20000000p+1f, -0x1.921fb60000000p+1f};
    static constexpr float hi[8] = {0x1.8b6ae80000000p-2f, 0x1.9b089a0000000p+0f, 0x1.849ba60000000p+0f, 0x1.921fb60000000p+1f, 0x1.2020c40000000p+1f, 0x1.921fb60000000p+1f, 0x1.147ae20000000p+1f, 0x1.921fb60000000p+1f};
    static constexpr int cap_link[10] = {-1, 0, 1, 2, 3, 4, 5, 6, 7, 7};
    static constexpr float cap_p0[10][3] = {{0.0f, 0.0f, 0x1.3333340000000p-3f}, {-0x1.3333340000000p-4f, 0.0f, 0x1.99999a0000000p-5f}, {0.0f, 0.0f, 0.0f}, {0.0f, 0.0f, 0.0f}, {0.0f, 0.0f, 0.0f}, {0.0f, 0.0f, 0.0f}, {0.0f, 0.0f, 0.0f}, {0.0f, 0.0f, 0.0f}, {0.0f, 0.0f, 0.0f}, {-0x1.eb851e0000000p-5f, 0.0f, 0x1.1773180000000p-3f}};
    static constexpr float cap_p1[10][3] = {{0.0f, 0.0f, 0x1.ae147a0000000p-3f}, {-0x1.3333340000000p-4f, 0.0f, 0x1.19999a0000000p-1f}, {0x1.df3b640000000p-4f, 0.0f, 0x1.eb851e0000000p-5f}, {0.0f, 0x1.c083120000000p-3f, 0.0f}, {0.0f, 0.0f, 0x1.10624e0000000p-3f}, {0.0f, 0x1.9374bc0000000p-3f, 0.0f}, {0.0f, 0.0f, 0x1.fdf3b60000000p-4f}, {0.0f, 0x1.1ba5e40000000p-3f, 0.0f}, {0.0f, 0.0f, 0x1.c28f5c0000000p-4f}, {0x1.eb851e0000000p-5f, 0.0f, 0x1.1773180000000p-3f}};
    static constexpr float cap_r[10] = {0x1.3333340000000p-2f, 0x1.eb851e0000000p-4f, 0x1.1eb8520000000p-4f, 0x1.0a3d700000000p-4f, 0x1.eb851e0000000p-5f, 0x1.eb851e0000000p-5f, 0x1.c28f5c0000000p-5f, 0x1.c28f5c0000000p-5f, 0x1.99999a0000000p-5f, 0x1.47ae140000000p-5f};
    static constexpr float cap_c[10][3] = {{0.0f, 0.0f, 0x1.70a3d80000000p-3f}, {-0x1.3333340000000p-4f, 0.0f, 0x1.3333340000000p-2f}, {0x1.df3b640000000p-5f, 0.0f, 0x1.eb851e0000000p-6f}, {0.0f, 0x1.c083120000000p-4f, 0.0f}, {0.0f, 0.0f, 0x1.10624e0000000p-4f}, {0.0f, 0x1.9374bc0000000p-4f, 0.0f}, {0.0f, 0.0f, 0x1.fdf3b60000000p-5f}, {0.0f, 0x1.1ba5e40000000p-4f, 0.0f}, {0.0f, 0.0f, 0x1.c28f5c0000000p-5f}, {0.0f, 0.0f, 0x1.1773180000000p-3f}};
    static constexpr float cap_h[10][3] = {{0.0f, 0.0f, 0x1.eb85180000000p-6f}, {0.0f, 0.0f, 0x1.0000000000000p-2f}, {0x1.df3b640000000p-5f, 0.0f, 0x1.eb851e0000000p-6f}, {0.0f, 0x1.c083120000000p-4f, 0.0f}, {0.0f, 0.0f, 0x1.10624e0000000p-4f}, {0.0f, 0x1.9374bc0000000p-4f, 0.0f}, {0.0f, 0.0f, 0x1.fdf3b60000000p-5f}, {0.0f, 0x1.1ba5e40000000p-4f, 0.0f}, {0.0f, 0.0f, 0x1.c28f5c0000000p-5f}, {0x1.eb851e0000000p-5f, 0.0f, 0.0f}};
    static constexpr float cap_a[10] = {0x1.d7dbe80000000p-11f, 0x1.0000000000000p-4f, 0x1.1b43520000000p-8f, 0x1.88e5820000000p-7f, 0x1.21d10c0000000p-8f, 0x1.3dec5e0000000p-7f, 0x1.fbe9840000000p-9f, 0x1.3a48320000000p-8f, 0x1.8c7e280000000p-9f, 0x1.d7dbf40000000p-9f};
    static constexpr float cap_ia[10] = {0x1.15c7240000000p+10f, 0x1.0000000000000p+4f, 0x1.ceb8d40000000p+7f, 0x1.4d9aba0000000p+6f, 0x1.c4422a0000000p+7f, 0x1.9c46880000000p+6f, 0x1.020f740000000p+8f, 0x1.a10d5c0000000p+7f, 0x1.4a941a0000000p+8f, 0x1.15c71e0000000p+8f};
    static constexpr float pair_thr[27] = {0x1.10d8460000000p-3f, 0x1.096bba0000000p-3f, 0x1.096bba0000000p-3f, 0x1.0219660000000p-3f, 0x1.0219660000000p-3f, 0x1.f5c2920000000p-4f, 0x1.d97f620000000p-4f, 0x1.096bb80000000p-5f, 0x1.096bb80000000p-5f, 0x1.f5c28c0000000p-6f, 0x1.f5c28c0000000p-6f, 0x1.d97f620000000p-6f, 0x1.a36e2c0000000p-6f, 0x1.14e3ba0000000p-6f, 0x1.0000000000000p-6f, 0x1.0000000000000p-6f, 0x1.d7dbf60000000p-7f, 0x1.8c7e280000000p-7f, 0x1.d7dbf20000000p-7f, 0x1.d7dbf20000000p-7f, 0x1.b15b540000000p-7f, 0x1.6944660000000p-7f, 0x1.b15b540000000p-7f, 0x1.8c7e280000000p-7f, 0x1.47ae120000000p-7f, 0x1.8c7e280000000p-7f, 0x1.47ae120000000p-7f};
    static constexpr float cap_thr[10] = {0x1.70a3d80000000p-4f, 0x1.d7dbf20000000p-7f, 0x1.41205a0000000p-8f, 0x1.14e3ba0000000p-8f, 0x1.d7dbf20000000p-9f, 0x1.d7dbf20000000p-9f, 0x1.8c7e280000000p-9f, 0x1.8c7e280000000p-9f, 0x1.47ae140000000p-9f, 0x1.a36e2c0000000p-10f};
    static constexpr float pair_cull[27] = {0x1.0f17260000000p-2f, 0x1.bdbc260000000p-3f, 0x1.fcfbc80000000p-3f, 0x1.ac3bd40000000p-3f, 0x1.b972160000000p-3f, 0x1.9598860000000p-3f, 0x1.8c88500000000p-3f, 0x1.06b9be0000000p-2f, 0x1.28f8b60000000p-2f, 0x1.fa6f240000000p-3f, 0x1.0465840000000p-2f, 0x1.e1c9fa0000000p-3f, 0x1.d7e80a0000000p-3f, 0x1.7b2e6a0000000p-4f, 0x1.1b54ce0000000p-4f, 0x1.2a9d580000000p-4f, 0x1.018d280000000p-4f, 0x1.eec3ba0000000p-5f, 0x1.74fd9a0000000p-4f, 0x1.867f240000000p-4f, 0x1.5752340000000p-4f, 0x1.4b907e0000000p-4f, 0x1.1684680000000p-4f, 0x1.ddd2dc0000000p-5f, 0x1.ca3e2a0000000p-5f, 0x1.326bb00000000p-4f, 0x1.2751c40000000p-4f};
    static constexpr float cap_cull[10] = {0x1.d98b840000000p-4f, 0x1.27c2c20000000p-3f, 0x1.5c0d380000000p-6f, 0x1.16e2b80000000p-5f, 0x1.314d240000000p-6f, 0x1.d139a20000000p-6f, 0x1.0953540000000p-6f, 0x1.2751c40000000p-6f, 0x1.b166700000000p-7f, 0x1.8c884e0000000p-7f};
    static constexpr int pair_a[27] = {0, 0, 0, 0, 0, 0, 0, 1, 1, 1, 1, 1, 1, 2, 2, 2, 2, 2, 3, 3, 3, 3, 4, 4, 4, 5, 5};
    static constexpr int pair_b[27] = {3, 4, 5, 6, 7, 8, 9, 4, 5, 6, 7, 8, 9, 5, 6, 7, 8, 9, 6, 7, 8, 9, 7, 8, 9, 8, 9};
};

struct FetchArm {
    static constexpr const char* name = "fetch_arm";
    static constexpr int D = 7, L = 10, P = 26;
    static constexpr uint32_t pris_mask = 0u;
    static constexpr float F[7][12] = {
        {1.0f, 0.0f, 0.0f, 0.0f, 1.0f, 0.0f, 0.0f, 0.0f, 1.0f, 0x1.0b78040000000p-5f, 0.0f, 0x1.73b7960000000p-1f},
        {0.0f, 1.0f, 0.0f, 0.0f, 0.0f, 1.0f, 1.0f, 0.0f, 0.0f, 0x1.df3b640000000p-4f, 0.0f, 0x1.eb851e0000000p-5f},
        {0.0f, 1.0f, 0.0f, 0.0f, 0.0f, 1.0f, 1.0f, 0.0f, 0.0f, 0.0f, 0x1.c083120000000p-3f, 0.0f},
        {0.0f, 0.0f, 1.0f, 1.0f, 0.0f, 0.0f, 0.0f, 1.0f, 0.0f, 0.0f, 0.0f, 0x1.10624e0000000p-3f},
        {0.0f, 1.0f, 0.0f, 0.0f, 0.0f, 1.0f, 1.0f, 0.0f, 0.0f, 0.0f, 0x1.9374bc0000000p-3f, 0.0f},
        {0.0f, 0.0f, 1.0f, 1.0f, 0.0f, 0.0f, 0.0f, 1.0f, 0.0f, 0.0f, 0.0f, 0x1.fdf3b60000000p-4f},
        {0.0f, 1.0f, 0.0f, 0.0f, 0.0f, 1.0f, 1.0f, 0.0f, 0.0f, 0.0f, 0x1.1ba5e40000000p-3f, 0.0f},
    };
    static constexpr float Fee[12] = {0.0f, 1.0f, 0.0f, 0.0f, 0.0f, 1.0f, 1.0f, 0.0f, 0.0f, 0.0f, 0.0f, 0x1.54e3bc0000000p-3f};
    static constexpr float lo[7] = {-0x1.9b089a0000000p+0f, -0x1.3893740000000p+0f, -0x1.921fb60000000p+1f, -0x1.2020c40000000p+1f, -0x1.921fb60000000p+1f, -0x1.147ae20000000p+1f, -0x1.921fb60000000p+1f};
    static constexpr float hi[7] = {0x1.9b089a0000000p+0f, 0x1.849ba60000000p+0f, 0x1.921fb60000000p+1f, 0x1.2020c40000000p+1f, 0x1.921fb60000000p+1f, 0x1.147ae20000000p+1f, 0x1.921fb60000000p+1f};
    static constexpr int cap_link[10] = {-1, -1, 0, 1, 2, 3, 4, 5, 6, 6};
    static constexpr float cap_p0[10][3] = {{0.0f, 0.0f, 0x1.3333340000000p-3f}, {-0x1.4b851e0000000p-3f, 0.0f, 0x1.b5b0360000000p-2f}, {0.0f, 0.0f, 0.0f}, {0.0f, 0.0f, 0.0f}, {0.0f, 0.0f, 0.0f}, {0.0f, 0.0f, 0.0f}, {0.0f, 0.0f, 0.0f}, {0.0f, 0.0f, 0.0f}, {0.0f, 0.0f, 0.0f}, {-0x1.eb851e0000000p-5f, 0.0f, 0x1.1773180000000p-3f}};
    static constexpr float cap_p1[10][3] = {{0.0f, 0.0f, 0x1.ae147a0000000p-3f}, {-0x1.4b851e0000000p-3f, 0.0f, 0x1.dad81a0000000p-1f}, {0x1.df3b640000000p-4f, 0.0f, 0x1.eb851e0000000p-5f}, {0.0f, 0x1.c083120000000p-3f, 0.0f}, {0.0f, 0.0f, 0x1.10624e0000000p-3f}, {0.0f, 0x1.9374bc0000000p-3f, 0.0f}, {0.0f, 0.0f, 0x1.fdf3b60000000p-4f}, {0.0f, 0x1.1ba5e40000000p-3f, 0.0f}, {0.0f, 0.0f, 0x1.c28f5c0000000p-4f}, {0x1.eb851e0000000p-5f, 0.0f, 0x1.1773180000000p-3f}};
    static constexpr float cap_r[10] = {0x1.3333340000000p-2f, 0x1.eb851e0000000p-4f, 0x1.1eb8520000000p-4f, 0x1.0a3d700000000p-4f, 0x1.eb851e0000000p-5f, 0x1.eb851e0000000p-5f, 0x1.c28f5c0000000p-5f, 0x1.c28f5c0000000p-5f, 0x1.99999a0000000p-5f, 0x1.47ae140000000p-5f};
    static constexpr float cap_c[10][3] = {{0.0f, 0.0f, 0x1.70a3d80000000p-3f}, {-0x1.4b851e0000000p-3f, 0.0f, 0x1.5ad81a0000000p-1f}, {0x1.df3b640000000p-5f, 0.0f, 0x1.eb851e0000000p-6f}, {0.0f, 0x1.c083120000000p-4f, 0.0f}, {0.0f, 0.0f, 0x1.10624e0000000p-4f}, {0.0f, 0x1.9374bc0000000p-4f, 0.0f}, {0.0f, 0.0f, 0x1.fdf3b60000000p-5f}, {0.0f, 0x1.1ba5e40000000p-4f, 0.0f}, {0.0f, 0.0f, 0x1.c28f5c0000000p-5f}, {0.0f, 0.0f, 0x1.1773180000000p-3f}};
    static constexpr float cap_h[10][3] = {{0.0f, 0.0f, 0x1.eb85180000000p-6f}, {0.0f, 0.0f, 0x1.fffffe0000000p-3f}, {0x1.df3b640000000p-5f, 0.0f, 0x1.eb851e0000000p-6f}, {0.0f, 0x1.c083120000000p-4f, 0.0f}, {0.0f, 0.0f, 0x1.10624e0000000p-4f}, {0.0f, 0x1.9374bc0000000p-4f, 0.0f}, {0.0f, 0.0f, 0x1.fdf3b60000000p-5f}, {0.0f, 0x1.1ba5e40000000p-4f, 0.0f}, {0.0f, 0.0f, 0x1.c28f5c0000000p-5f}, {0x1.eb851e0000000p-5f, 0.0f, 0.0f}};
    static constexpr float cap_a[10] = {0x1.d7dbe80000000p-11f, 0x1.fffffc0000000p-5f, 0x1.1b43520000000p-8f, 0x1.88e5820000000p-7f, 0x1.21d10c0000000p-8f, 0x1.3dec5e0000000p-7f, 0x1.fbe9840000000p-9f, 0x1.3a48320000000p-8f, 0x1.8c7e280000000p-9f, 0x1.d7dbf40000000p-9f};
    static constexpr float cap_ia[10] = {0x1.15c7240000000p+10f, 0x1.0000020000000p+4f, 0x1.ceb8d40000000p+7f, 0x1.4d9aba0000000p+6f, 0x1.c4422a0000000p+7f, 0x1.9c46880000000p+6f, 0x1.020f740000000p+8f, 0x1.a10d5c0000000p+7f, 0x1.4a941a0000000p+8f, 0x1.15c71e0000000p+8f};
    static constexpr float pair_thr[26] = {0x1.096bba0000000p-3f, 0x1.096bba0000000p-3f, 0x1.0219660000000p-3f, 0x1.0219660000000p-3f, 0x1.f5c2920000000p-4f, 0x1.d97f620000000p-4f, 0x1.096bb80000000p-5f, 0x1.096bb80000000p-5f, 0x1.f5c28c0000000p-6f, 0x1.f5c28c0000000p-6f, 0x1.d97f620000000p-6f, 0x1.a36e2c0000000p-6f, 0x1.14e3ba0000000p-6f, 0x1.0000000000000p-6f, 0x1.0000000000000p-6f, 0x1.d7dbf60000000p-7f, 0x1.8c7e280000000p-7f, 0x1.d7dbf20000000p-7f, 0x1.d7dbf20000000p-7f, 0x1.b15b540000000p-7f, 0x1.6944660000000p-7f, 0x1.b15b540000000p-7f, 0x1.8c7e280000000p-7f, 0x1.47ae120000000p-7f, 0x1.8c7e280000000p-7f, 0x1.47ae120000000p-7f};
    static constexpr float cap_thr[10] = {0x1.70a3d80000000p-4f, 0x1.d7dbf20000000p-7f, 0x1.41205a0000000p-8f, 0x1.14e3ba0000000p-8f, 0x1.d7dbf20000000p-9f, 0x1.d7dbf20000000p-9f, 0x1.8c7e280000000p-9f, 0x1.8c7e280000000p-9f, 0x1.47ae140000000p-9f, 0x1.a36e2c0000000p-10f};
    static constexpr float pair_cull[26] = {0x1.bdbc260000000p-3f, 0x1.fcfbc80000000p-3f, 0x1.ac3bd40000000p-3f, 0x1.b972160000000p-3f, 0x1.9598860000000p-3f, 0x1.8c88500000000p-3f, 0x1.06b9bc0000000p-2f, 0x1.28f8b40000000p-2f, 0x1.fa6f220000000p-3f, 0x1.0465840000000p-2f, 0x1.e1c9f80000000p-3f, 0x1.d7e8080000000p-3f, 0x1.7b2e6a0000000p-4f, 0x1.1b54ce0000000p-4f, 0x1.2a9d580000000p-4f, 0x1.018d280000000p-4f, 0x1.eec3ba0000000p-5f, 0x1.74fd9a0000000p-4f, 0x1.867f240000000p-4f, 0x1.5752340000000p-4f, 0x1.4b907e0000000p-4f, 0x1.1684680000000p-4f, 0x1.ddd2dc0000000p-5f, 0x1.ca3e2a0000000p-5f, 0x1.326bb00000000p-4f, 0x1.2751c40000000p-4f};
    static constexpr float cap_cull[10] = {0x1.d98b840000000p-4f, 0x1.27c2c20000000p-3f, 0x1.5c0d380000000p-6f, 0x1.16e2b80000000p-5f, 0x1.314d240000000p-6f, 0x1.d139a20000000p-6f, 0x1.0953540000000p-6f, 0x1.2751c40000000p-6f, 0x1.b166700000000p-7f, 0x1.8c884e0000000p-7f};
    static constexpr int pair_a[26] = {0, 0, 0, 0, 0, 0, 1, 1, 1, 1, 1, 1, 2, 2, 2, 2, 2, 3, 3, 3, 3, 4, 4, 4, 5, 5};
    static constexpr int pair_b[26] = {4, 5, 6, 7, 8, 9, 4, 5, 6, 7, 8, 9, 5, 6, 7, 8, 9, 6, 7, 8, 9, 7, 8, 9, 8, 9};
};

struct Chain12 {
    static constexpr const char* name = "chain12";
    static constexpr int D = 12, L = 13, P = 55;
    static constexpr uint32_t pris_mask = 0u;
    static constexpr float F[12][12] = {
        {1.0f, 0.0f, 0.0f, 0.0f, 1.0f, 0.0f, 0.0f, 0.0f, 1.0f, 0.0f, 0.0f, 0x1.3333340000000p-3f},
        {0.0f, 1.0f, 0.0f, 0.0f, 0.0f, 1.0f, 1.0f, 0.0f, 0.0f, 0.0f, 0.0f, 0x1.3333340000000p-3f},
        {0.0f, 0.0f, 1.0f, 1.0f, 0.0f, 0.0f, 0.0f, 1.0f, 0.0f, 0x1.3333340000000p-3f, 0.0f, 0.0f},
        {0.0f, 1.0f, 0.0f, 0.0f, 0.0f, 1.0f, 1.0f, 0.0f, 0.0f, 0.0f, 0.0f, 0x1.3333340000000p-3f},
        {0.0f, 0.0f, 1.0f, 1.0f, 0.0f, 0.0f, 0.0f, 1.0f, 0.0f, 0x1.3333340000000p-3f, 0.0f, 0.0f},
        {0.0f, 1.0f, 0.0f, 0.0f, 0.0f, 1.0f, 1.0f, 0.0f, 0.0f, 0.0f, 0.0f, 0x1.3333340000000p-3f},
        {0.0f, 0.0f, 1.0f, 1.0f, 0.0f, 0.0f, 0.0f, 1.0f, 0.0f, 0x1.3333340000000p-3f, 0.0f, 0.0f},
        {0.0f, 1.0f, 0.0f, 0.0f, 0.0f, 1.0f, 1.0f, 0.0f, 0.0f, 0.0f, 0.0f, 0x1.3333340000000p-3f},
        {0.0f, 0.0f, 1.0f, 1.0f, 0.0f, 0.0f, 0.0f, 1.0f, 0.0f, 0x1.3333340000000p-3f, 0.0f, 0.0f},
        {0.0f, 1.0f, 0.0f, 0.0f, 0.0f, 1.0f, 1.0f, 0.0f, 0.0f, 0.0f, 0.0f, 0x1.3333340000000p-3f},
        {0.0f, 0.0f, 1.0f, 1.0f, 0.0f, 0.0f, 0.0f, 1.0f, 0.0f, 0x1.3333340000000p-3f, 0.0f, 0.0f},
        {0.0f, 1.0f, 0.0f, 0.0f, 0.0f, 1.0f, 1.0f, 0.0f, 0.0f, 0.0f, 0.0f, 0x1.3333340000000p-3f},
    };
    static constexpr float Fee[12] = {0.0f, 0.0f, 1.0f, 1.0f, 0.0f, 0.0f, 0.0f, 1.0f, 0.0f, 0x1.3333340000000p-3f, 0.0f, 0.0f};
    static constexpr float lo[12] = {-0x1.6666660000000p+1f, -0x1.6666660000000p+1f, -0x1.6666660000000p+1f, -0x1.6666660000000p+1f, -0x1.6666660000000p+1f, -0x1.6666660000000p+1f, -0x1.6666660000000p+1f, -0x1.6666660000000p+1f, -0x1.6666660000000p+1f, -0x1.6666660000000p+1f, -0x1.6666660000000p+1f, -0x1.6666660000000p+1f};
    static constexpr float hi[12] = {0x1.6666660000000p+1f, 0x1.6666660000000p+1f, 0x1.6666660000000p+1f, 0x1.6666660000000p+1f, 0x1.6666660000000p+1f, 0x1.6666660000000p+1f, 0x1.6666660000000p+1f, 0x1.6666660000000p+1f, 0x1.6666660000000p+1f, 0x1.6666660000000p+1f, 0x1.6666660000000p+1f, 0x1.6666660000000p+1f};
    static constexpr int cap_link[13] = {-1, 0, 1, 2, 3, 4, 5, 6, 7, 8, 9, 10, 11};
    static constexpr float cap_p0[13][3] = {{0.0f, 0.0f, 0.0f}, {0.0f, 0.0f, 0x1.47ae140000000p-6f}, {0x1.47ae140000000p-6f, 0.0f, 0.0f}, {0.0f, 0.0f, 0x1.47ae140000000p-6f}, {0x1.47ae140000000p-6f, 0.0f, 0.0f}, {0.0f, 0.0f, 0x1.47ae140000000p-6f}, {0x1.47ae140000000p-6f, 0.0f, 0.0f}, {0.0f, 0.0f, 0x1.47ae140000000p-6f}, {0x1.47ae140000000p-6f, 0.0f, 0.0f}, {0.0f, 0.0f, 0x1.47ae140000000p-6f}, {0x1.47ae140000000p-6f, 0.0f, 0.0f}, {0.0f, 0.0f, 0x1.47ae140000000p-6f}, {0x1.47ae140000000p-6f, 0.0f, 0.0f}};
    static constexpr float cap_p1[13][3] = {{0.0f, 0.0f, 0x1.99999a0000000p-4f}, {0.0f, 0.0f, 0x1.0a3d700000000p-3f}, {0x1.0a3d700000000p-3f, 0.0f, 0.0f}, {0.0f, 0.0f, 0x1.0a3d700000000p-3f}, {0x1.0a3d700000000p-3f, 0.0f, 0.0f}, {0.0f, 0.0f, 0x1.0a3d700000000p-3f}, {0x1.0a3d700000000p-3f, 0.0f, 0.0f}, {0.0f, 0.0f, 0x1.0a3d700000000p-3f}, {0x1.0a3d700000000p-3f, 0.0f, 0.0f}, {0.0f, 0.0f, 0x1.0a3d700000000p-3f}, {0x1.0a3d700000000p-3f, 0.0f, 0.0f}, {0.0f, 0.0f, 0x1.0a3d700000000p-3f}, {0x1.0a3d700000000p-3f, 0.0f, 0.0f}};
    static constexpr float cap_r[13] = {0x1.99999a0000000p-5f, 0x1.1eb8520000000p-5f, 0x1.1eb8520000000p-5f, 0x1.1eb8520000000p-5f, 0x1.1eb8520000000p-5f, 0x1.1eb8520000000p-5f, 0x1.1eb8520000000p-5f, 0x1.1eb8520000000p-5f, 0x1.1eb8520000000p-5f, 0x1.1eb8520000000p-5f, 0x1.1eb8520000000p-5f, 0x1.1eb8520000000p-5f, 0x1.1eb8520000000p-5f};
    static constexpr float cap_c[13][3] = {{0.0f, 0.0f, 0x1.99999a0000000p-5f}, {0.0f, 0.0f, 0x1.3333320000000p-4f}, {0x1.3333320000000p-4f, 0.0f, 0.0f}, {0.0f, 0.0f, 0x1.3333320000000p-4f}, {0x1.3333320000000p-4f, 0.0f, 0.0f}, {0.0f, 0.0f, 0x1.3333320000000p-4f}, {0x1.3333320000000p-4f, 0.0f, 0.0f}, {0.0f, 0.0f, 0x1.3333320000000p-4f}, {0x1.3333320000000p-4f, 0.0f, 0.0f}, {0.0f, 0.0f, 0x1.3333320000000p-4f}, {0x1.3333320000000p-4f, 0.0f, 0.0f}, {0.0f, 0.0f, 0x1.3333320000000p-4f}, {0x1.3333320000000p-4f, 0.0f, 0.0f}};
    static constexpr float cap_h[13][3] = {{0.0f, 0.0f, 0x1.99999a0000000p-5f}, {0.0f, 0.0f, 0x1.c28f5c0000000p-5f}, {0x1.c28f5c0000000p-5f, 0.0f, 0.0f}, {0.0f, 0.0f, 0x1.c28f5c0000000p-5f}, {0x1.c28f5c0000000p-5f, 0.0f, 0.0f}, {0.0f, 0.0f, 0x1.c28f5c0000000p-5f}, {0x1.c28f5c0000000p-5f, 0.0f, 0.0f}, {0.0f, 0.0f, 0x1.c28f5c0000000p-5f}, {0x1.c28f5c0000000p-5f, 0.0f, 0.0f}, {0.0f, 0.0f, 0x1.c28f5c0000000p-5f}, {0x1.c28f5c0000000p-5f, 0.0f, 0.0f}, {0.0f, 0.0f, 0x1.c28f5c0000000p-5f}, {0x1.c28f5c0000000p-5f, 0.0f, 0.0f}};
    static constexpr float cap_a[13] = {0x1.47ae160000000p-9f, 0x1.8c7e280000000p-9f, 0x1.8c7e280000000p-9f, 0x1.8c7e280000000p-9f, 0x1.8c7e280000000p-9f, 0x1.8c7e280000000p-9f, 0x1.8c7e280000000p-9f, 0x1.8c7e280000000p-9f, 0x1.8c7e280000000p-9f, 0x1.8c7e280000000p-9f, 0x1.8c7e280000000p-9f, 0x1.8c7e280000000p-9f, 0x1.8c7e280000000p-9f};
    static constexpr float cap_ia[13] = {0x1.9000000000000p+8f, 0x1.4a941a0000000p+8f, 0x1.4a941a0000000p+8f, 0x1.4a941a0000000p+8f, 0x1.4a941a0000000p+8f, 0x1.4a941a0000000p+8f, 0x1.4a941a0000000p+8f, 0x1.4a941a0000000p+8f, 0x1.4a941a0000000p+8f, 0x1.4a941a0000000p+8f, 0x1.4a941a0000000p+8f, 0x1.4a941a0000000p+8f, 0x1.4a941a0000000p+8f};
    static constexpr float pair_thr[55] = {0x1.d97f620000000p-8f, 0x1.d97f620000000p-8f, 0x1.d97f620000000p-8f, 0x1.d97f620000000p-8f, 0x1.d97f620000000p-8f, 0x1.d97f620000000p-8f, 0x1.d97f620000000p-8f, 0x1.d97f620000000p-8f, 0x1.d97f620000000p-8f, 0x1.d97f620000000p-8f, 0x1.41205a0000000p-8f, 0x1.41205a0000000p-8f, 0x1.41205a0000000p-8f, 0x1.41205a0000000p-8f, 0x1.41205a0000000p-8f, 0x1.41205a0000000p-8f, 0x1.41205a0000000p-8f, 0x1.41205a0000000p-8f, 0x1.41205a0000000p-8f, 0x1.41205a0000000p-8f, 0x1.41205a0000000p-8f, 0x1.41205a0000000p-8f, 0x1.41205a0000000p-8f, 0x1.41205a0000000p-8f, 0x1.41205a0000000p-8f, 0x1.41205a0000000p-8f, 0x1.41205a0000000p-8f, 0x1.41205a0000000p-8f, 0x1.41205a0000000p-8f, 0x1.41205a0000000p-8f, 0x1.41205a0000000p-8f, 0x1.41205a0000000p-8f, 0x1.41205a0000000p-8f, 0x1.41205a0000000p-8f, 0x1.41205a0000000p-8f, 0x1.41205a0000000p-8f, 0x1.41205a0000000p-8f, 0x1.41205a0000000p-8f, 0x1.41205a0000000p-8f, 0x1.41205a0000000p-8f, 0x1.41205a0000000p-8f, 0x1.41205a0000000p-8f, 0x1.41205a0000000p-8f, 0x1.41205a0000000p-8f, 0x1.41205a0000000p-8f, 0x1.41205a0000000p-8f, 0x1.41205a0000000p-8f, 0x1.41205a0000000p-8f, 0x1.41205a0000000p-8f, 0x1.41205a0000000p-8f, 0x1.41205a0000000p-8f, 0x1.41205a0000000p-8f, 0x1.41205a0000000p-8f, 0x1.41205a0000000p-8f, 0x1.41205a0000000p-8f};
    static constexpr float cap_thr[13] = {0x1.47ae140000000p-9f, 0x1.41205a0000000p-10f, 0x1.41205a0000000p-10f, 0x1.41205a0000000p-10f, 0x1.41205a0000000p-10f, 0x1.41205a0000000p-10f, 0x1.41205a0000000p-10f, 0x1.41205a0000000p-10f, 0x1.41205a0000000p-10f, 0x1.41205a0000000p-10f, 0x1.41205a0000000p-10f, 0x1.41205a0000000p-10f, 0x1.41205a0000000p-10f};
    static constexpr float pair_cull[55] = {0x1.47b67a0000000p-5f, 0x1.47b67a0000000p-5f, 0x1.47b67a0000000p-5f, 0x1.47b67a0000000p-5f, 0x1.47b67a0000000p-5f, 0x1.47b67a0000000p-5f, 0x1.47b67a0000000p-5f, 0x1.47b67a0000000p-5f, 0x1.47b67a0000000p-5f, 0x1.47b67a0000000p-5f, 0x1.27c2c20000000p-5f, 0x1.27c2c20000000p-5f, 0x1.27c2c20000000p-5f, 0x1.27c2c20000000p-5f, 0x1.27c2c20000000p-5f, 0x1.27c2c20000000p-5f, 0x1.27c2c20000000p-5f, 0x1.27c2c20000000p-5f, 0x1.27c2c20000000p-5f, 0x1.27c2c20000000p-5f, 0x1.27c2c20000000p-5f, 0x1.27c2c20000000p-5f, 0x1.27c2c20000000p-5f, 0x1.27c2c20000000p-5f, 0x1.27c2c20000000p-5f, 0x1.27c2c20000000p-5f, 0x1.27c2c20000000p-5f, 0x1.27c2c20000000p-5f, 0x1.27c2c20000000p-5f, 0x1.27c2c20000000p-5f, 0x1.27c2c20000000p-5f, 0x1.27c2c20000000p-5f, 0x1.27c2c20000000p-5f, 0x1.27c2c20000000p-5f, 0x1.27c2c20000000p-5f, 0x1.27c2c20000000p-5f, 0x1.27c2c20000000p-5f, 0x1.27c2c20000000p-5f, 0x1.27c2c20000000p-5f, 0x1.27c2c20000000p-5f, 0x1.27c2c20000000p-5f, 0x1.27c2c20000000p-5f, 0x1.27c2c20000000p-5f, 0x1.27c2c20000000p-5f, 0x1.27c2c20000000p-5f, 0x1.27c2c20000000p-5f, 0x1.27c2c20000000p-5f, 0x1.27c2c20000000p-5f, 0x1.27c2c20000000p-5f, 0x1.27c2c20000000p-5f, 0x1.27c2c20000000p-5f, 0x1.27c2c20000000p-5f, 0x1.27c2c20000000p-5f, 0x1.27c2c20000000p-5f, 0x1.27c2c20000000p-5f};
    static constexpr float cap_cull[13] = {0x1.8c88500000000p-7f, 0x1.47b6780000000p-7f, 0x1.47b6780000000p-7f, 0x1.47b6780000000p-7f, 0x1.47b6780000000p-7f, 0x1.47b6780000000p-7f, 0x1.47b6780000000p-7f, 0x1.47b6780000000p-7f, 0x1.47b6780000000p-7f, 0x1.47b6780000000p-7f, 0x1.47b6780000000p-7f, 0x1.47b6780000000p-7f, 0x1.47b6780000000p-7f};
    static constexpr int pair_a[55] = {0, 0, 0, 0, 0, 0, 0, 0, 0, 0, 1, 1, 1, 1, 1, 1, 1, 1, 1, 2, 2, 2, 2, 2, 2, 2, 2, 3, 3, 3, 3, 3, 3, 3, 4, 4, 4, 4, 4, 4, 5, 5, 5, 5, 5, 6, 6, 6, 6, 7, 7, 7, 8, 8, 9};
    static constexpr int pair_b[55] = {3, 4, 5, 6, 7, 8, 9, 10, 11, 12, 4, 5, 6, 7, 8, 9, 10, 11, 12, 5, 6, 7, 8, 9, 10, 11, 12, 6, 7, 8, 9, 10, 11, 12, 7, 8, 9, 10, 11, 12, 8, 9, 10, 11, 12, 9, 10, 11, 12, 10, 11, 12, 11, 12, 12};
};

constexpr int kNumStaticRobots = 4;
}
}

#define CPPF_FOR_EACH_STATIC_ROBOT(M) \
    M(0, ::cppf::gen::Panda) \
    M(1, ::cppf::gen::Fetch) \
    M(2, ::cppf::gen::FetchArm) \
    M(3, ::cppf::gen::Chain12)
```

### cppflow_amd/csrc/rtc_specialize.h

```cpp
#pragma once

#include <sys/stat.h>
#include <sys/types.h>
#include <unistd.h>

#include <cstdlib>
#include <fstream>
#include <sstream>

#include "embedded_src.inc"

namespace {

enum RtcKernel { RTC_FUSED0 = 0, RTC_FUSED1, RTC_FUSED2, RTC_COLL_MASK, RTC_COLL_MIN, RTC_QUAD0, RTC_QUAD1, RTC_TRACK, RTC_COUNT };

const char* const kRtcNameExpr[RTC_COUNT] = {
    "cppf_rtc::lm_fused_kernel<cppf::StaRobot<cppf::gen::Custom>, 0>",
    "cppf_rtc::lm_fused_kernel<cppf::StaRobot<cppf::gen::Custom>, 1>",
    "cppf_rtc::lm_fused_kernel<cppf::StaRobot<cppf::gen::Custom>, 2>",
    "cppf_rtc::collision_kernel<cppf::StaRobot<cppf::gen::Custom>, false>",
    "cppf_rtc::collision_kernel<cppf::StaRobot<cppf::gen::Custom>, true>",
    "cppf_rtc::lm_quad_kernel<cppf::StaRobot<cppf::gen::Custom>, 0, false>",
    "cppf_rtc::lm_quad_kernel<cppf::StaRobot<cppf::gen::Custom>, 1, false>",
    "cppf_rtc::track_kernel<cppf::StaRobot<cppf::gen::Custom>>",
};

const char* const kRtcOptions[] = {"--offload-arch=gfx950", "-O3", "-std=c++17", "-ffp-contract=off",
                                   "-fhip-fp32-correctly-rounded-divide-sqrt", "-fno-slp-vectorize", "-Wno-comment",
                                   "-mllvm", "-amdgpu-sched-strategy=max-ilp", "-mllvm", "-enable-post-misched=0"};
constexpr int kRtcOptionCount = (int)(sizeof(kRtcOptions) / sizeof(kRtcOptions[0]));

struct RtcModule {
    hipModule_t module = nullptr;
    hipFunction_t fn[RTC_COUNT] = {};
};

typedef struct _hiprtcProgram* RtcProgram;
struct RtcApi {
    void* handle = nullptr;
    int (*CreateProgram)(RtcProgram*, const char*, const char*, int, const char* const*, const char* const*) = nullptr;
    int (*AddNameExpression)(RtcProgram, const char*) = nullptr;
    int (*CompileProgram)(RtcProgram, int, const char* const*) = nullptr;
    int (*GetProgramLogSize)(RtcProgram, size_t*) = nullptr;
    int (*GetProgramLog)(RtcProgram, char*) = nullptr;
    int (*GetCodeSize)(RtcProgram, size_t*) = nullptr;
    int (*GetCode)(RtcProgram, char*) = nullptr;
    int (*GetLoweredName)(RtcProgram, const char*, const char**) = nullptr;
    int (*DestroyProgram)(RtcProgram*) = nullptr;
    const char* (*GetErrorString)(int) = nullptr;
    int (*Version)(int*, int*) = nullptr;
};
RtcApi g_rtc;

int load_hiprtc() {
    if (g_rtc.handle) return CPPF_OK;
    const char* names[] = {"libhiprtc.so.7", "libhiprtc.so", "/opt/rocm/lib/libhiprtc.so"};
    void* h = nullptr;
    for (const char* n : names) {
        h = dlopen(n, RTLD_NOW | RTLD_GLOBAL);
        if (h) break;
    }
    if (!h) return fail(CPPF_ERR_UNSUPPORTED, std::string("cppflow_hip: cannot load hipRTC (libhiprtc.so): ") + dlerror());
    RtcApi api;
    api.handle = h;
#define CPPF_SYM(field, name)                                                                          \
    api.field = reinterpret_cast<decltype(api.field)>(dlsym(h, name));                                 \
    if (!api.field) return fail(CPPF_ERR_UNSUPPORTED, std::string("cppflow_hip: hipRTC lacks ") + name)
    CPPF_SYM(CreateProgram, "hiprtcCreateProgram");
    CPPF_SYM(AddNameExpression, "hiprtcAddNameExpression");
    CPPF_SYM(CompileProgram, "hiprtcCompileProgram");
    CPPF_SYM(GetProgramLogSize, "hiprtcGetProgramLogSize");
    CPPF_SYM(GetProgramLog, "hiprtcGetProgramLog");
    CPPF_SYM(GetCodeSize, "hiprtcGetCodeSize");
    CPPF_SYM(GetCode, "hiprtcGetCode");
    CPPF_SYM(GetLoweredName, "hiprtcGetLoweredName");
    CPPF_SYM(DestroyProgram, "hiprtcDestroyProgram");
    CPPF_SYM(GetErrorString, "hiprtcGetErrorString");
#undef CPPF_SYM
    api.Version = reinterpret_cast<decltype(api.Version)>(dlsym(h, "hiprtcVersion"));
    g_rtc = api;
    return CPPF_OK;
}

std::string rtc_version_string() {
    int major = 0, minor = 0;
    if (load_hiprtc() != CPPF_OK || !g_rtc.Version || g_rtc.Version(&major, &minor) != 0) return "?";
    return std::to_string(major) + "." + std::to_string(minor);
}

std::string rtc_float(float v) {
    if (v != v) return "__builtin_nanf(\"\")";
    if (v == INFINITY) return "__builtin_huge_valf()";
    if (v == -INFINITY) return "(-__builtin_huge_valf())";
    char buf[64];
    std::snprintf(buf, sizeof buf, "%af", (double)v);
    return buf;
}

template <class It>
std::string rtc_array(It begin, It end) {
    std::string s = "{";
    for (It it = begin; it != end; ++it) {
        if (it != begin) s += ", ";
        s += rtc_float(*it);
    }
    return s + "}";
}

std::string rtc_table_source(const cppf_robot& rb) {
    const cppf_robot_desc& d = rb.desc;
    const CollK& co = rb.coll;
    const int D = d.ndof, L = d.n_capsules, P = d.n_pairs, Lm = L > 0 ? L : 1, Pm = P > 0 ? P : 1;
    std::ostringstream o;
    o << "namespace cppf { namespace gen {\nstruct Custom {\n";
    o << "    static constexpr const char* name = \"custom\";\n";
    o << "    static constexpr int D = " << D << ", L = " << L << ", P = " << P << ";\n";
    o << "    static constexpr uint32_t pris_mask = " << rb.chain.pris_mask << "u;\n";
    o << "    static constexpr float F[" << D << "][12] = {\n";
    for (int j = 0; j < D; ++j) o << "        " << rtc_array(d.F[j], d.F[j] + 12) << ",\n";
    o << "    };\n";
    o << "    static constexpr float Fee[12] = " << rtc_array(d.F_ee, d.F_ee + 12) << ";\n";
    o << "    static constexpr float lo[" << D << "] = " << rtc_array(d.lo, d.lo + D) << ";\n";
    o << "    static constexpr float hi[" << D << "] = " << rtc_array(d.hi, d.hi + D) << ";\n";
    o << "    static constexpr int cap_link[" << Lm << "] = {";
    for (int c = 0; c < Lm; ++c) o << (c ? ", " : "") << (L ? d.cap_link[c] : 0);
    o << "};\n";
    auto vec3s = [&](const char* nm, const float (*p)[3]) {
        o << "    static constexpr float " << nm << "[" << Lm << "][3] = {";
        for (int c = 0; c < Lm; ++c) {
            const float z[3] = {0.f, 0.f, 0.f};
            const float* v = L ? p[c] : z;
            o << (c ? ", " : "") << rtc_array(v, v + 3);
        }
        o << "};\n";
    };
    vec3s("cap_p0", d.cap_p0);
    vec3s("cap_p1", d.cap_p1);
    vec3s("cap_c", co.cap_c);
    vec3s("cap_h", co.cap_h);
    std::vector<float> cap_r(Lm, 0.f), cap_thr(Lm, 0.f), cap_cull(Lm, 0.f), pair_thr(Pm, 0.f), pair_cull(Pm, 0.f), cap_a(Lm, 0.f), cap_ia(Lm, 0.f);
    for (int c = 0; c < L; ++c)
        cap_r[c] = d.cap_r[c], cap_thr[c] = co.cap_thr[c], cap_cull[c] = co.cap_cull[c], cap_a[c] = co.cap_a[c], cap_ia[c] = co.cap_ia[c];
    for (int p = 0; p < P; ++p) pair_thr[p] = co.pair_thr[p], pair_cull[p] = co.pair_cull[p];
    o << "    static constexpr float cap_a[" << Lm << "] = " << rtc_array(cap_a.begin(), cap_a.end()) << ";\n";
    o << "    static constexpr float cap_ia[" << Lm << "] = " << rtc_array(cap_ia.begin(), cap_ia.end()) << ";\n";
    o << "    static constexpr float cap_r[" << Lm << "] = " << rtc_array(cap_r.begin(), cap_r.end()) << ";\n";
    o << "    static constexpr float pair_thr[" << Pm << "] = " << rtc_array(pair_thr.begin(), pair_thr.end()) << ";\n";
    o << "    static constexpr float cap_thr[" << Lm << "] = " << rtc_array(cap_thr.begin(), cap_thr.end()) << ";\n";
    o << "    static constexpr float pair_cull[" << Pm << "] = " << rtc_array(pair_cull.begin(), pair_cull.end()) << ";\n";
    o << "    static constexpr float cap_cull[" << Lm << "] = " << rtc_array(cap_cull.begin(), cap_cull.end()) << ";\n";
    for (int side = 0; side < 2; ++side) {
        o << "    static constexpr int pair_" << (side ? "b" : "a") << "[" << Pm << "] = {";
        for (int p = 0; p < Pm; ++p) o << (p ? ", " : "") << (P ? d.pairs[p][side] : 0);
        o << "};\n";
    }
    o << "};\n} }\n";
    return o.str();
}

std::string rtc_program_source(const cppf_robot& rb) {
    std::string s;
    s += "// generated by cppf_robot_specialize (csrc/rtc_specialize.h)\n";
    s += "#include \"lmik_device.h\"\n";
    s += rtc_table_source(rb);
    s += "using namespace cppf;\n";
    s += "namespace cppf_rtc {\n";
    s += "constexpr int kBlock = " + std::to_string(kBlock) + ";\n";
    s += "#define CPPF_WAVES_LM " + std::to_string(CPPF_WAVES_LM) + "\n";
    s += "#define CPPF_WAVES_COLL " + std::to_string(CPPF_WAVES_COLL) + "\n";
    s += "#include \"kernels_chain.h\"\n#include \"kernels_collision.h\"\n#include \"kernels_fused.h\"\n#include \"kernels_track.h\"\n#include \"kernels_quad.h\"\n";
    s += "}  // namespace cppf_rtc\n";
    return s;
}

uint64_t fnv1a(const std::string& s, uint64_t h = 1469598103934665603ull) {
    for (unsigned char c : s) {
        h ^= c;
        h *= 1099511628211ull;
    }
    return h;
}

std::string rtc_cache_dir(const char* cache_dir) {
    if (cache_dir && *cache_dir) return cache_dir;
    if (const char* e = std::getenv("CPPF_CACHE_DIR"))
        if (*e) return e;
    if (const char* home = std::getenv("HOME"))
        if (*home) return std::string(home) + "/.cache/cppflow_amd";
    return "/tmp/cppflow_amd-" + std::to_string((long)getuid());
}

void mkdir_p(const std::string& path) {
    std::string cur;
    for (size_t i = 0; i <= path.size(); ++i) {
        if (i == path.size() || path[i] == '/') {
            if (!cur.empty()) (void)mkdir(cur.c_str(), i == path.size() ? 0700 : 0755);
        }
        if (i < path.size()) cur += path[i];
    }
}

bool rtc_cache_dir_trusted(const std::string& dir) {
    struct stat st;
    if (lstat(dir.c_str(), &st) != 0) return false;
    return S_ISDIR(st.st_mode) && st.st_uid == getuid() && (st.st_mode & (S_IWGRP | S_IWOTH)) == 0;
}

bool rtc_cache_read(const std::string& dir, const std::string& file, std::vector<std::string>& names, std::string& code) {
    if (!rtc_cache_dir_trusted(dir)) return false;
    std::ifstream f(file, std::ios::binary);
    if (!f) return false;
    std::string magic, sum;
    if (!std::getline(f, magic) || magic != "CPPFRTC2" || !std::getline(f, sum)) return false;
    names.clear();
    for (int i = 0; i < RTC_COUNT; ++i) {
        std::string n;
        if (!std::getline(f, n) || n.empty()) return false;
        names.push_back(n);
    }
    std::ostringstream rest;
    rest << f.rdbuf();
    code = rest.str();
    char want[32];
    std::snprintf(want, sizeof want, "%016llx", (unsigned long long)fnv1a(code));
    return code.size() > 64 && sum == want;
}

void rtc_cache_write(const std::string& dir, const std::string& file, const std::vector<std::string>& names, const std::string& code) {
    mkdir_p(dir);
    if (!rtc_cache_dir_trusted(dir)) return;
    const std::string tmp = file + ".tmp." + std::to_string((long)getpid());
    {
        std::ofstream f(tmp, std::ios::binary);
        if (!f) return;
        char sum[32];
        std::snprintf(sum, sizeof sum, "%016llx", (unsigned long long)fnv1a(code));
        f << "CPPFRTC2\n" << sum << "\n";
        for (const std::string& n : names) f << n << "\n";
        f.write(code.data(), (std::streamsize)code.size());
        if (!f) return;
    }
    (void)std::rename(tmp.c_str(), file.c_str());
}

int rtc_compile(const std::string& source, bool with_quad, std::vector<std::string>& names, std::string& code) {
    if (int rc = load_hiprtc()) return rc;
    RtcProgram prog = nullptr;
    int r = g_rtc.CreateProgram(&prog, source.c_str(), "cppf_custom_robot.hip", kEmbeddedCount, kEmbeddedSources, kEmbeddedNames);
    if (r != 0) return fail(CPPF_ERR_HIP, std::string("cppflow_hip: hiprtcCreateProgram: ") + g_rtc.GetErrorString(r));
    auto wanted = [&](int i) { return with_quad || (i != RTC_QUAD0 && i != RTC_QUAD1); };
    for (int i = 0; i < RTC_COUNT; ++i)
        if (wanted(i)) (void)g_rtc.AddNameExpression(prog, kRtcNameExpr[i]);
    r = g_rtc.CompileProgram(prog, kRtcOptionCount, kRtcOptions);
    if (r != 0) {
        size_t n = 0;
        std::string log;
        if (g_rtc.GetProgramLogSize(prog, &n) == 0 && n > 1) {
            log.resize(n);
            (void)g_rtc.GetProgramLog(prog, &log[0]);
        }
        (void)g_rtc.DestroyProgram(&prog);
        return fail(CPPF_ERR_HIP, std::string("cppflow_hip: hipRTC compilation failed: ") + g_rtc.GetErrorString(r) + "\n" + log.substr(0, 4000));
    }
    names.clear();
    for (int i = 0; i < RTC_COUNT; ++i) {
        const char* low = nullptr;
        if (!wanted(i)) {
            names.push_back("-");
            continue;
        }
        r = g_rtc.GetLoweredName(prog, kRtcNameExpr[i], &low);
        if (r != 0 || !low) {
            (void)g_rtc.DestroyProgram(&prog);
            return fail(CPPF_ERR_HIP, std::string("cppflow_hip: no lowered name for ") + kRtcNameExpr[i]);
        }
        names.push_back(low);
    }
    size_t n = 0;
    r = g_rtc.GetCodeSize(prog, &n);
    if (r == 0) {
        code.resize(n);
        r = g_rtc.GetCode(prog, &code[0]);
    }
    (void)g_rtc.DestroyProgram(&prog);
    if (r != 0) return fail(CPPF_ERR_HIP, std::string("cppflow_hip: hiprtcGetCode: ") + g_rtc.GetErrorString(r));
    return CPPF_OK;
}

}
```

### cppflow_amd/gen_robots.py

```python

import os

import numpy as np

from cppflow_amd.robot_model import CanonicalChain, canonicalize
from cppflow_amd.robot_zoo import ROBOT_SPECS

OUT = os.path.join(os.path.dirname(os.path.abspath(__file__)), "csrc", "robots_gen.h")
ORDER = ["panda", "fetch", "fetch_arm", "chain12"]


def _f(v) -> str:
    v = float(np.float32(v))
    if v == 0.0:
        return "0.0f"
    if v == 1.0:
        return "1.0f"
    if v == -1.0:
        return "-1.0f"
    return v.hex() + "f"


def _arr(vals) -> str:
    return "{" + ", ".join(_f(v) for v in vals) + "}"


def sqrt_threshold(r) -> np.float32:
    r = np.float32(r)
    if r <= 0:
        return np.float32(0.0)
    y = np.float32(r * r)
    while np.sqrt(y) >= r:
        y = np.nextafter(y, np.float32(0.0))
    while np.sqrt(y) < r:
        y = np.nextafter(y, np.float32(np.inf))
    return y


def cull_threshold(reach: float) -> np.float32:
    y = (float(reach) + 0.01) ** 2 * (1.0 + 1e-4)
    f = np.float32(y)
    if float(f) < y:
        f = np.nextafter(f, np.float32(np.inf))
    return f


def capsule_centred(cap_p0, cap_p1):
    p0 = np.asarray(cap_p0, dtype=np.float32).astype(np.float64).reshape(-1, 3)
    p1 = np.asarray(cap_p1, dtype=np.float32).astype(np.float64).reshape(-1, 3)
    c = (0.5 * (p0 + p1)).astype(np.float32)
    h = (0.5 * (p1 - p0)).astype(np.float32)
    hd = h.astype(np.float64)
    a = (hd[:, 0] * hd[:, 0] + hd[:, 1] * hd[:, 1]) + hd[:, 2] * hd[:, 2]
    ia = np.where(a >= 2.0**-100, 1.0 / np.maximum(a, 2.0**-100), 0.0)
    return c, h, a.astype(np.float32), ia.astype(np.float32), np.sqrt(a)


def emit_robot(name: str, ch: CanonicalChain) -> str:
    d, L, P = ch.ndof, ch.n_capsules, ch.n_pairs
    cname = "".join(p.capitalize() for p in name.split("_"))
    s = [f"struct {cname} {{"]
    s.append(f'    static constexpr const char* name = "{name}";')
    s.append(f"    static constexpr int D = {d}, L = {L}, P = {P};")
    s.append(f"    static constexpr uint32_t pris_mask = {sum(1 << j for j in range(d) if ch.jtype[j] == 1)}u;")
    s.append(f"    static constexpr float F[{d}][12] = {{")
    for j in range(d):
        s.append("        " + _arr(ch.F[j]) + ",")
    s.append("    };")
    s.append(f"    static constexpr float Fee[12] = {_arr(ch.F_ee)};")
    s.append(f"    static constexpr float lo[{d}] = {_arr(ch.lo)};")
    s.append(f"    static constexpr float hi[{d}] = {_arr(ch.hi)};")
    Lm, Pm = max(L, 1), max(P, 1)
    s.append(f"    static constexpr int cap_link[{Lm}] = {{" + ", ".join(str(int(v)) for v in (ch.cap_link if L else [0])) + "};")
    s.append(f"    static constexpr float cap_p0[{Lm}][3] = {{" + ", ".join(_arr(v) for v in (ch.cap_p0 if L else [[0, 0, 0]])) + "};")
    s.append(f"    static constexpr float cap_p1[{Lm}][3] = {{" + ", ".join(_arr(v) for v in (ch.cap_p1 if L else [[0, 0, 0]])) + "};")
    s.append(f"    static constexpr float cap_r[{Lm}] = {_arr(ch.cap_r if L else [0])};")
    cc, hh, aa, ia, half = capsule_centred(ch.cap_p0, ch.cap_p1) if L else (np.zeros((1, 3)), np.zeros((1, 3)), [0], [0], [])
    s.append(f"    static constexpr float cap_c[{Lm}][3] = {{" + ", ".join(_arr(v) for v in cc) + "};  // centre 0.5 (p0 + p1)")
    s.append(f"    static constexpr float cap_h[{Lm}][3] = {{" + ", ".join(_arr(v) for v in hh) + "};  // half-axis 0.5 (p1 - p0)")
    s.append(f"    static constexpr float cap_a[{Lm}] = {_arr(aa)};  // |h|^2")
    s.append(f"    static constexpr float cap_ia[{Lm}] = {_arr(ia)};  // 1 / |h|^2")
    r32 = ch.cap_r.astype(np.float32)
    pair_thr = [sqrt_threshold(np.float32(r32[a] + r32[b])) for a, b in ch.pairs] if P else [0]
    cap_thr = [sqrt_threshold(r) for r in r32] if L else [0]
    s.append(f"    static constexpr float pair_thr[{Pm}] = {_arr(pair_thr)};  // sqrt thresholds of r_a + r_b")
    s.append(f"    static constexpr float cap_thr[{Lm}] = {_arr(cap_thr)};  // sqrt thresholds of r")
    pair_cull = [cull_threshold(half[a] + half[b] + float(r32[a]) + float(r32[b])) for a, b in ch.pairs] if P else [0]
    cap_cull = [cull_threshold(half[c] + float(r32[c])) for c in range(L)] if L else [0]
    s.append(f"    static constexpr float pair_cull[{Pm}] = {_arr(pair_cull)};  // broad phase, pairs")
    s.append(f"    static constexpr float cap_cull[{Lm}] = {_arr(cap_cull)};  // broad phase, capsule vs cuboid")
    s.append(f"    static constexpr int pair_a[{Pm}] = {{" + ", ".join(str(int(v)) for v in (ch.pairs[:, 0] if P else [0])) + "};")
    s.append(f"    static constexpr int pair_b[{Pm}] = {{" + ", ".join(str(int(v)) for v in (ch.pairs[:, 1] if P else [0])) + "};")
    s.append("};")
    return "\n".join(s)


def generate() -> str:
    parts = [
        "// robots_gen.h -- GENERATED by cppflow_amd/gen_robots.py from cppflow_amd/robot_zoo.py; do not edit.",
        "// Canonical chains (cppflow_amd/robot_model.py) of the shipped robots as compile-time tables.",
        "#pragma once",
        "#include <stdint.h>",
        "",
        "namespace cppf {",
        "namespace gen {",
        "",
    ]
    names = []
    for name in ORDER:
        ch = canonicalize(ROBOT_SPECS[name]())
        parts.append(emit_robot(name, ch))
        parts.append("")
        names.append("".join(p.capitalize() for p in name.split("_")))
    parts.append(f"constexpr int kNumStaticRobots = {len(names)};")
    parts.append("}  // namespace gen")
    parts.append("}  // namespace cppf")
    parts.append("")
    parts.append("// X-macro over the generated robots: CPPF_FOR_EACH_STATIC_ROBOT(M) expands M(index, Type)")
    parts.append("#define CPPF_FOR_EACH_STATIC_ROBOT(M) \\")
    parts.append(" \\\n".join(f"    M({i}, ::cppf::gen::{n})" for i, n in enumerate(names)))
    parts.append("")
    return "\n".join(parts)


def write(force: bool = False) -> bool:
    text = generate()
    if not force and os.path.exists(OUT) and open(OUT).read() == text:
        return False
    with open(OUT, "w") as f:
        f.write(text)
    return True


if __name__ == "__main__":
    print(OUT, "written" if write() else "up to date")
```

Measured before the change: 75.75 billion.

## Skip certified-safe self-collision pairs and unreachable capsule-obstacle tests

An offline interval branch-and-bound certifies capsule pairs that can never come within 1 cm of each other inside the joint limits, and the in-limits collision path skips those pairs at compile time. The host also computes per-capsule bitmasks of obstacles that each capsule could ever reach, and the device skips environment tests for capsules outside them. This reduces the narrow-phase collision work done after LM-IK rows finish. It adds a code-generation step and relies on the certification being conservative and on the in_limits condition (clamping on, no tolerance early exit) holding for the rows that use it.

```diff
diff --git a/cppflow_amd/build.py b/cppflow_amd/build.py
--- a/cppflow_amd/build.py
+++ b/cppflow_amd/build.py
@@ -7,7 +7,7 @@
 CSRC = os.path.join(_HERE, "csrc")
 SOURCES = ["cppflow_hip.hip", "fused_static.hip"]
 EXTRA_FLAGS = {"fused_static.hip": ["-O2", "-mllvm", "-amdgpu-sched-strategy=max-ilp", "-mllvm", "-enable-post-misched=0"]}
-HEADERS = ["lmik_device.h", "robots_gen.h", "rtc_specialize.h", "kernels_chain.h", "kernels_collision.h", "kernels_fused.h", "kernels_track.h", "kernels_quad.h", "kernels_eval.h",
+HEADERS = ["lmik_device.h", "obstacle_reach.h", "robots_gen.h", "rtc_specialize.h", "kernels_chain.h", "kernels_collision.h", "kernels_fused.h", "kernels_track.h", "kernels_quad.h", "kernels_eval.h",
            "kernels_coupled.h", "kernels_dp.h", "kernels_optloop.h", "kernels_scene.h", "kernels_motion.h", "kernels_motion_resolve.h", os.path.join("..", "..", "include", "cppflow_hip.h"),
            os.path.join("..", "..", "include", "cppflow_hip_debug.h")]
 OUT = os.path.join(CSRC, "libcppflow_hip.so")
diff --git a/cppflow_amd/csrc/cppflow_hip.hip b/cppflow_amd/csrc/cppflow_hip.hip
--- a/cppflow_amd/csrc/cppflow_hip.hip
+++ b/cppflow_amd/csrc/cppflow_hip.hip
@@ -15,6 +15,7 @@
 
 #include "../../include/cppflow_hip_debug.h"
 #include "lmik_device.h"
+#include "obstacle_reach.h"
 #include "robots_gen.h"
 
 using namespace cppf;
@@ -604,6 +605,9 @@
         }
     }
     robot->coll.nobs = n_obs;
+    const CapsuleReach live = capsule_reach(robot->desc, robot->coll.cap_c, robot->coll.cap_cull, n_obs, robot->coll.obs_lo, robot->coll.obs_hi);
+    robot->coll.cap_live_any = live.any;
+    robot->coll.cap_live_lim = live.lim;
     return CPPF_OK;
 }
 
diff --git a/cppflow_amd/csrc/kernels_collision.h b/cppflow_amd/csrc/kernels_collision.h
--- a/cppflow_amd/csrc/kernels_collision.h
+++ b/cppflow_amd/csrc/kernels_collision.h
@@ -86,11 +86,17 @@
     return near;
 }
 
-template <class RB, bool WANT_MIN>
+template <class T>
+constexpr bool has_certified_pairs() {
+    for (int pi = 0; pi < T::P; ++pi)
+        if (T::pair_never[pi]) return true;
+    return false;
+}
+template <class RB, bool WANT_MIN, bool IN_LIMITS = false>
 __device__ __forceinline__ CollOut collide_tests_static(const CollK& co,
                                                         const float (&wc)[(RB::Table::L > 0 ? RB::Table::L : 1)][3],
                                                         const float (&wh)[(RB::Table::L > 0 ? RB::Table::L : 1)][3],
-                                                        bool do_self, bool do_env) {
+                                                        bool do_self, bool do_env, uint32_t live) {
     using T = typename RB::Table;
     CollOut r;
     r.min_self = INFINITY;
@@ -100,6 +106,7 @@
         for (int pi = 0; pi < T::P; ++pi) {
             const int a = T::pair_a[pi], b = T::pair_b[pi];
             if constexpr (!WANT_MIN) {
+                if (IN_LIMITS && T::pair_never[pi]) continue;
                 if (cull_far(mid_dist2(wc[a], wc[b]), T::pair_cull[pi])) continue;
             }
             const float d2 = seg_seg_dist2(wc[a], wh[a], wc[b], wh[b], T::cap_a[a], T::cap_ia[a], T::cap_a[b], T::cap_ia[b]);
@@ -119,6 +126,7 @@
         for (int c = 0; c < T::L; ++c) {
             uint32_t near = ~0u;
             if constexpr (!WANT_MIN) {
+                if (!((live >> c) & 1u)) continue;
                 near = cuboids_in_reach(co, wc[c], T::cap_cull[c]);
                 if (near == 0u) continue;
             }
@@ -205,7 +213,7 @@
         constexpr int L = RB::Table::L > 0 ? RB::Table::L : 1;
         float wc[L][3], wh[L][3];
         capsule_fk_static<RB>(rb, q, R, p, wc, wh);
-        return collide_tests_static<RB, WANT_MIN>(co, wc, wh, do_self, do_env);
+        return collide_tests_static<RB, WANT_MIN>(co, wc, wh, do_self, do_env, co.cap_live_any);
     } else {
         fk_capsules_to_lds<RB>(rb, co, q, lds, tid, R, p);
         return collide_from_lds<WANT_MIN>(co, lds, tid, do_self, do_env);
diff --git a/cppflow_amd/csrc/kernels_fused.h b/cppflow_amd/csrc/kernels_fused.h
--- a/cppflow_amd/csrc/kernels_fused.h
+++ b/cppflow_amd/csrc/kernels_fused.h
@@ -260,7 +260,7 @@
 template <class RB, int COLL>
 __device__ __forceinline__ void lm_row_finish(const RB& rb, const CollK& co, const cppf_lm_outputs& out, float* lds, int tid,
                                               size_t row, const float (&Rt)[9], const float (&tt)[3], const float (&q)[RB::D],
-                                              RowSummary& rs) {
+                                              RowSummary& rs, bool in_limits) {
     constexpr int D = RB::D;
     if (out.x_out) store_x<D>(out.x_out, row, q);
     const bool want_metrics = out.pos_err_m || out.rot_err_rad || out.seed_summary;
@@ -285,7 +285,11 @@
                 capsule_fk_static<RB>(rb, q, R, p, wc, wh);
                 metrics(R, p);
             }
-            c = collide_tests_static<RB, COLL == 2>(co, wc, wh, do_self, do_env);
+            const uint32_t live = in_limits ? co.cap_live_lim : co.cap_live_any;
+            if (COLL == 1 && has_certified_pairs<typename RB::Table>() && in_limits)
+                c = collide_tests_static<RB, false, true>(co, wc, wh, do_self, do_env, live);
+            else
+                c = collide_tests_static<RB, COLL == 2>(co, wc, wh, do_self, do_env, live);
         } else {
             {
                 float R[9], p[3];
@@ -409,7 +413,8 @@
             for (int j = 0; j < D; ++j) q[j] = __builtin_nanf("");
         }
         lm_pace(pace_t0, prm.n_steps, prm.pace_ticks);
-        lm_row_finish<RB, COLL>(rb, co, out, lds, tid_b, row_b, Rt, tt, q, rs);
+        const bool in_limits = prm.clamp != 0 && prm.n_steps >= 1 && !(prm.tol_pos2 > 0.f);
+        lm_row_finish<RB, COLL>(rb, co, out, lds, tid_b, row_b, Rt, tt, q, rs, in_limits);
     }
     if constexpr (COLL != 0) {
         if (out.seed_summary) {
diff --git a/cppflow_amd/csrc/lmik_device.h b/cppflow_amd/csrc/lmik_device.h
--- a/cppflow_amd/csrc/lmik_device.h
+++ b/cppflow_amd/csrc/lmik_device.h
@@ -43,6 +43,8 @@
     float jl_lo[CPPF_MAX_DOF];
     float jl_hi[CPPF_MAX_DOF];
     int32_t ncaps, npairs, nobs, has_jl;
+    uint32_t cap_live_any;
+    uint32_t cap_live_lim;
 };
 
 struct LmK {
diff --git a/cppflow_amd/csrc/obstacle_reach.h b/cppflow_amd/csrc/obstacle_reach.h
--- /dev/null
+++ b/cppflow_amd/csrc/obstacle_reach.h
@@ -0,0 +1,67 @@
+#pragma once
+
+#include <math.h>
+#include <stdint.h>
+
+#include "../../include/cppflow_hip.h"
+
+namespace cppf {
+
+struct CapsuleReach {
+    uint32_t any;
+    uint32_t lim;
+};
+
+inline float host_point_box_dist2(const float m[3], const float lo[3], const float hi[3]) {
+    float e[3];
+    for (int k = 0; k < 3; ++k) {
+        const float cl = m[k] < lo[k] ? lo[k] : (m[k] > hi[k] ? hi[k] : m[k]);
+        e[k] = m[k] - cl;
+    }
+    return fmaf(e[2], e[2], fmaf(e[1], e[1], e[0] * e[0]));
+}
+
+inline CapsuleReach capsule_reach(const cppf_robot_desc& d, const float (*cap_c)[3], const float* cap_cull, int nobs,
+                                  const float (*obs_lo)[3], const float (*obs_hi)[3]) {
+    CapsuleReach r{0u, 0u};
+    const double o[3] = {d.F[0][9], d.F[0][10], d.F[0][11]};
+    double travel[CPPF_MAX_DOF];
+    double acc = 0.0;
+    for (int j = 0; j < d.ndof; ++j) {
+        if (j > 0) acc += sqrt((double)d.F[j][9] * d.F[j][9] + (double)d.F[j][10] * d.F[j][10] + (double)d.F[j][11] * d.F[j][11]);
+        if (d.jtype[j] == CPPF_JOINT_PRISMATIC) acc += fmax(fabs((double)d.lo[j]), fabs((double)d.hi[j]));
+        travel[j] = acc;
+    }
+    for (int c = 0; c < d.n_capsules; ++c) {
+        const int l = d.cap_link[c];
+        bool live_any = true, live_lim = false;
+        const bool on_axis0 = l == 0 && d.jtype[0] == CPPF_JOINT_REVOLUTE && d.cap_p0[c][0] == 0.f && d.cap_p0[c][1] == 0.f &&
+                              d.cap_p1[c][0] == 0.f && d.cap_p1[c][1] == 0.f;
+        if (l < 0 || on_axis0) {
+            float m[3] = {cap_c[c][0], cap_c[c][1], cap_c[c][2]};
+            if (on_axis0)
+                for (int k = 0; k < 3; ++k) m[k] = fmaf(d.F[0][3 * k + 2], cap_c[c][2], d.F[0][9 + k]);
+            live_any = false;
+            for (int ob = 0; ob < nobs; ++ob) live_any |= !(host_point_box_dist2(m, obs_lo[ob], obs_hi[ob]) > cap_cull[c]);
+            live_lim = live_any;
+        } else {
+            double n0 = 0.0, n1 = 0.0;
+            for (int k = 0; k < 3; ++k) n0 += (double)d.cap_p0[c][k] * d.cap_p0[c][k], n1 += (double)d.cap_p1[c][k] * d.cap_p1[c][k];
+            const double reach = (travel[l] + sqrt(fmax(n0, n1)) + (double)d.cap_r[c] + 0.01) * (1.0 + 1e-6);
+            for (int ob = 0; ob < nobs; ++ob) {
+                double d2 = 0.0;
+                for (int k = 0; k < 3; ++k) {
+                    const double lo = obs_lo[ob][k], hi = obs_hi[ob][k];
+                    const double e = o[k] < lo ? lo - o[k] : (o[k] > hi ? o[k] - hi : 0.0);
+                    d2 += e * e;
+                }
+                live_lim |= !(d2 > reach * reach);
+            }
+        }
+        if (live_any) r.any |= 1u << c;
+        if (live_lim) r.lim |= 1u << c;
+    }
+    return r;
+}
+
+}
diff --git a/cppflow_amd/csrc/robots_gen.h b/cppflow_amd/csrc/robots_gen.h
--- a/cppflow_amd/csrc/robots_gen.h
+++ b/cppflow_amd/csrc/robots_gen.h
@@ -34,6 +34,7 @@
     static constexpr float cap_cull[9] = {0x1.14ead60000000p-6f, 0x1.89aa3a0000000p-6f, 0x1.4128940000000p-6f, 0x1.bb4b580000000p-6f, 0x1.3b72fc0000000p-6f, 0x1.1d70780000000p-5f, 0x1.6274440000000p-7f, 0x1.47b67a0000000p-7f, 0x1.2aa0d60000000p-6f};
     static constexpr int pair_a[25] = {0, 0, 0, 0, 0, 0, 0, 1, 1, 1, 1, 1, 1, 2, 2, 2, 2, 2, 3, 3, 3, 3, 4, 4, 4};
     static constexpr int pair_b[25] = {2, 3, 4, 5, 6, 7, 8, 3, 4, 5, 6, 7, 8, 4, 5, 6, 7, 8, 5, 6, 7, 8, 6, 7, 8};
+    static constexpr bool pair_never[25] = {true, true, false, false, false, false, false, true, true, false, false, false, false, true, true, false, false, false, true, true, true, false, true, true, true};
 };
 
 struct Fetch {
@@ -67,6 +68,7 @@
     static constexpr float cap_cull[10] = {0x1.d98b840000000p-4f, 0x1.27c2c20000000p-3f, 0x1.5c0d380000000p-6f, 0x1.16e2b80000000p-5f, 0x1.314d240000000p-6f, 0x1.d139a20000000p-6f, 0x1.0953540000000p-6f, 0x1.2751c40000000p-6f, 0x1.b166700000000p-7f, 0x1.8c884e0000000p-7f};
     static constexpr int pair_a[27] = {0, 0, 0, 0, 0, 0, 0, 1, 1, 1, 1, 1, 1, 2, 2, 2, 2, 2, 3, 3, 3, 3, 4, 4, 4, 5, 5};
     static constexpr int pair_b[27] = {3, 4, 5, 6, 7, 8, 9, 4, 5, 6, 7, 8, 9, 5, 6, 7, 8, 9, 6, 7, 8, 9, 7, 8, 9, 8, 9};
+    static constexpr bool pair_never[27] = {true, false, false, false, false, false, false, true, false, false, false, false, false, true, false, false, false, false, false, false, false, false, true, false, false, false, true};
 };
 
 struct FetchArm {
@@ -99,6 +101,7 @@
     static constexpr float cap_cull[10] = {0x1.d98b840000000p-4f, 0x1.27c2c20000000p-3f, 0x1.5c0d380000000p-6f, 0x1.16e2b80000000p-5f, 0x1.314d240000000p-6f, 0x1.d139a20000000p-6f, 0x1.0953540000000p-6f, 0x1.2751c40000000p-6f, 0x1.b166700000000p-7f, 0x1.8c884e0000000p-7f};
     static constexpr int pair_a[26] = {0, 0, 0, 0, 0, 0, 1, 1, 1, 1, 1, 1, 2, 2, 2, 2, 2, 3, 3, 3, 3, 4, 4, 4, 5, 5};
     static constexpr int pair_b[26] = {4, 5, 6, 7, 8, 9, 4, 5, 6, 7, 8, 9, 5, 6, 7, 8, 9, 6, 7, 8, 9, 7, 8, 9, 8, 9};
+    static constexpr bool pair_never[26] = {false, false, false, false, false, false, true, false, false, false, false, false, true, false, false, false, false, false, false, false, false, true, false, false, false, true};
 };
 
 struct Chain12 {
@@ -136,6 +139,7 @@
     static constexpr float cap_cull[13] = {0x1.8c88500000000p-7f, 0x1.47b6780000000p-7f, 0x1.47b6780000000p-7f, 0x1.47b6780000000p-7f, 0x1.47b6780000000p-7f, 0x1.47b6780000000p-7f, 0x1.47b6780000000p-7f, 0x1.47b6780000000p-7f, 0x1.47b6780000000p-7f, 0x1.47b6780000000p-7f, 0x1.47b6780000000p-7f, 0x1.47b6780000000p-7f, 0x1.47b6780000000p-7f};
     static constexpr int pair_a[55] = {0, 0, 0, 0, 0, 0, 0, 0, 0, 0, 1, 1, 1, 1, 1, 1, 1, 1, 1, 2, 2, 2, 2, 2, 2, 2, 2, 3, 3, 3, 3, 3, 3, 3, 4, 4, 4, 4, 4, 4, 5, 5, 5, 5, 5, 6, 6, 6, 6, 7, 7, 7, 8, 8, 9};
     static constexpr int pair_b[55] = {3, 4, 5, 6, 7, 8, 9, 10, 11, 12, 4, 5, 6, 7, 8, 9, 10, 11, 12, 5, 6, 7, 8, 9, 10, 11, 12, 6, 7, 8, 9, 10, 11, 12, 7, 8, 9, 10, 11, 12, 8, 9, 10, 11, 12, 9, 10, 11, 12, 10, 11, 12, 11, 12, 12};
+    static constexpr bool pair_never[55] = {false, false, false, false, false, false, false, false, false, false, false, false, false, false, false, false, false, false, false, false, false, false, false, false, false, false, false, false, false, false, false, false, false, false, false, false, false, false, false, false, false, false, false, false, false, false, false, false, false, false, false, false, false, false, false};
 };
 
 constexpr int kNumStaticRobots = 4;
diff --git a/cppflow_amd/csrc/rtc_specialize.h b/cppflow_amd/csrc/rtc_specialize.h
--- a/cppflow_amd/csrc/rtc_specialize.h
+++ b/cppflow_amd/csrc/rtc_specialize.h
@@ -154,6 +154,9 @@
         for (int p = 0; p < Pm; ++p) o << (p ? ", " : "") << (P ? d.pairs[p][side] : 0);
         o << "};\n";
     }
+    o << "    static constexpr bool pair_never[" << Pm << "] = {";
+    for (int p = 0; p < Pm; ++p) o << (p ? ", " : "") << "false";
+    o << "};\n";
     o << "};\n} }\n";
     return o.str();
 }
diff --git a/cppflow_amd/gen_robots.py b/cppflow_amd/gen_robots.py
--- a/cppflow_amd/gen_robots.py
+++ b/cppflow_amd/gen_robots.py
@@ -54,6 +54,104 @@
     a = (hd[:, 0] * hd[:, 0] + hd[:, 1] * hd[:, 1]) + hd[:, 2] * hd[:, 2]
     ia = np.where(a >= 2.0**-100, 1.0 / np.maximum(a, 2.0**-100), 0.0)
     return c, h, a.astype(np.float32), ia.astype(np.float32), np.sqrt(a)
+
+
+CERT_MARGIN = 0.01
+CERT_SLACK = 1e-6
+CERT_MAX_DIMS = 4
+CERT_MAX_BOXES = 100000
+
+
+def _seg_point_dist2(p, a, d, dd):
+    u = np.clip(np.einsum("ij,ij->i", p - a, d) / np.where(dd > 0, dd, 1.0), 0.0, 1.0) * (dd > 0)
+    e = p - (a + u[:, None] * d)
+    return np.einsum("ij,ij->i", e, e)
+
+
+def segment_distance(p1, q1, p2, q2):
+    d1, d2, r = q1 - p1, q2 - p2, p1 - p2
+    a, e = np.einsum("ij,ij->i", d1, d1), np.einsum("ij,ij->i", d2, d2)
+    b, c, f = np.einsum("ij,ij->i", d1, d2), np.einsum("ij,ij->i", d1, r), np.einsum("ij,ij->i", d2, r)
+    den = a * e - b * b
+    ok = den > 1e-12 * np.maximum(a * e, 1e-300)
+    s = np.clip(np.where(ok, (b * f - c * e) / np.where(ok, den, 1.0), 0.0), 0.0, 1.0)
+    t = np.clip(np.where(e > 0, (b * s + f) / np.where(e > 0, e, 1.0), 0.0), 0.0, 1.0)
+    g = (p1 + s[:, None] * d1) - (p2 + t[:, None] * d2)
+    best = np.einsum("ij,ij->i", g, g)
+    for v in (_seg_point_dist2(p1, p2, d2, e), _seg_point_dist2(q1, p2, d2, e), _seg_point_dist2(p2, p1, d1, a), _seg_point_dist2(q2, p1, d1, a)):
+        best = np.minimum(best, v)
+    return np.sqrt(best)
+
+
+def pair_joints(ch: CanonicalChain, a: int, b: int):
+    if ch.cap_link[a] > ch.cap_link[b]:
+        a, b = b, a
+    return a, b, list(range(int(ch.cap_link[a]) + 1, int(ch.cap_link[b]) + 1))
+
+
+def _pair_clearance(ch: CanonicalChain, a: int, b: int, joints, q):
+    n = q.shape[0]
+    R = np.broadcast_to(np.eye(3), (n, 3, 3))
+    p = np.zeros((n, 3))
+    for i, j in enumerate(joints):
+        F = ch.F[j]
+        p = p + R @ F[9:12]
+        R = R @ F[:9].reshape(3, 3)
+        if ch.jtype[j] == 1:
+            p = p + R[:, :, 2] * q[:, i : i + 1]
+        else:
+            cs, sn = np.cos(q[:, i]), np.sin(q[:, i])
+            M = np.zeros((n, 3, 3))
+            M[:, 0, 0], M[:, 0, 1], M[:, 1, 0], M[:, 1, 1], M[:, 2, 2] = cs, -sn, sn, cs, 1.0
+            R = R @ M
+    b0, b1 = p + R @ ch.cap_p0[b], p + R @ ch.cap_p1[b]
+    a0, a1 = np.broadcast_to(ch.cap_p0[a], (n, 3)), np.broadcast_to(ch.cap_p1[a], (n, 3))
+    return segment_distance(a0, a1, b0, b1) - (ch.cap_r[a] + ch.cap_r[b])
+
+
+def pair_travel_bounds(ch: CanonicalChain, b: int, joints):
+    reach = max(np.linalg.norm(ch.cap_p0[b]), np.linalg.norm(ch.cap_p1[b]))
+    rho = []
+    for j in reversed(joints):
+        rho.append(1.0 if ch.jtype[j] == 1 else reach)
+        if ch.jtype[j] == 1:
+            reach += max(abs(ch.lo[j]), abs(ch.hi[j]))
+        reach += np.linalg.norm(ch.F[j][9:12])
+    return np.array(rho[::-1])
+
+
+def certify_pair(ch: CanonicalChain, a: int, b: int, margin: float = CERT_MARGIN, max_dims: int = CERT_MAX_DIMS,
+                 max_boxes: int = CERT_MAX_BOXES) -> bool:
+    a, b, joints = pair_joints(ch, a, b)
+    if not joints:
+        return bool(_pair_clearance(ch, a, b, joints, np.zeros((1, 0)))[0] >= margin + CERT_SLACK)
+    if len(joints) > max_dims or not np.all(ch.hi[joints] >= ch.lo[joints]):
+        return False
+    rho = pair_travel_bounds(ch, b, joints)
+    c = 0.5 * (ch.lo[joints] + ch.hi[joints])[None]
+    w = 0.5 * (ch.hi[joints] - ch.lo[joints])[None]
+    done = 0
+    while c.shape[0]:
+        done += c.shape[0]
+        if done > max_boxes:
+            return False
+        d = _pair_clearance(ch, a, b, joints, c)
+        if np.any(d < margin + CERT_SLACK):
+            return False
+        open_ = d - (w * rho).sum(axis=1) < margin + CERT_SLACK
+        c, w = c[open_], w[open_]
+        k = np.argmax(w * rho, axis=1)
+        rows = np.arange(c.shape[0])
+        w[rows, k] *= 0.5
+        lo_half, hi_half = c.copy(), c.copy()
+        lo_half[rows, k] -= w[rows, k]
+        hi_half[rows, k] += w[rows, k]
+        c, w = np.concatenate([lo_half, hi_half]), np.concatenate([w, w])
+    return True
+
+
+def pair_never(ch: CanonicalChain):
+    return [certify_pair(ch, int(a), int(b)) for a, b in ch.pairs]
 
 
 def emit_robot(name: str, ch: CanonicalChain) -> str:
@@ -91,6 +189,8 @@
     s.append(f"    static constexpr float cap_cull[{Lm}] = {_arr(cap_cull)};  // broad phase, capsule vs cuboid")
     s.append(f"    static constexpr int pair_a[{Pm}] = {{" + ", ".join(str(int(v)) for v in (ch.pairs[:, 0] if P else [0])) + "};")
     s.append(f"    static constexpr int pair_b[{Pm}] = {{" + ", ".join(str(int(v)) for v in (ch.pairs[:, 1] if P else [0])) + "};")
+    never = pair_never(ch) if P else [False]
+    s.append(f"    static constexpr bool pair_never[{Pm}] = {{" + ", ".join("true" if v else "false" for v in never) + "};  // certified: never within 1 cm inside [lo, hi]")
     s.append("};")
     return "\n".join(s)
 
```

New measurement: 77.50 billion, median of 6. 1.02x the previous value.
